# eduardburlacu/DiTSep

Measured on AMD Instinct MI355X. Metric: separated utterances/sec @ N=30, 2-spk 4 s mixtures, higher is better.
Workload: dtype fp16 (fp16 MFMA operands, fp32 accumulate)

## Files before the change

ditsep_amd/csrc/engine.hip:

```cpp
#include <math.h>
#include <stdarg.h>
#include <stdio.h>
#include <stdlib.h>
#include <string.h>

#include <algorithm>
#include <map>
#include <numeric>
#include <set>
#include <stdexcept>
#include <string>
#include <vector>

#include "../../include/ditsep_hip.h"
#include "igemm.h"
#include "kernels.h"

namespace {

struct Err : std::runtime_error {
  int code;
  Err(int c, const std::string& m) : std::runtime_error(m), code(c) {}
};

[[noreturn]] void fail(int code, const char* fmt, ...) {
  char buf[512];
  va_list ap;
  va_start(ap, fmt);
  vsnprintf(buf, sizeof buf, fmt, ap);
  va_end(ap);
  throw Err(code, buf);
}

#define HIPCHK(expr)                                                                       \
  do {                                                                                     \
    hipError_t e_ = (expr);                                                                \
    if (e_ != hipSuccess) fail(DSN_EHIP, "%s -> %s (%s:%d)", #expr, hipGetErrorString(e_), \
                               __FILE__, __LINE__);                                        \
  } while (0)

struct DevTensor {
  float* p = nullptr;
  std::vector<long> shape;
  long numel = 0;
};

struct Packed {
  op16_t* w = nullptr;
  long ps = 0;
  int N = 0, K = 0, Cin = 0, taps = 0;
  float* bias = nullptr;
  int bias_mod = 1;
};

struct ActP {
  int kind = DSN_ACT_NONE;
  float* a = nullptr;
  float* ib = nullptr;
  int mod = 1;
};

struct Packed8 {
  unsigned char* w = nullptr;
  unsigned char* s = nullptr;
  int N = 0, K = 0;
  float* bias = nullptr;
};

struct DitLayer {
  float *g1 = nullptr, *be1 = nullptr, *g2 = nullptr, *be2 = nullptr;
  Packed qkv, out, ff1, ff2;
  Packed8 qkv8, out8, ff1_8, ff2_8;
  Packed ff1f;
  float* ff1_colsum = nullptr;
  Packed8 ff1f8;
  float* ff1_colsum8 = nullptr;
};

struct ResUnit {
  ActP act0, act2;
  Packed conv7, conv1;
  int dil = 1;
};

struct VaeBlock {
  ActP act;
  Packed conv;
  ResUnit ru[3];
  int cin = 0, cout = 0, stride = 1;
};

struct Graph {
  hipGraphExec_t exec = nullptr;
  uint64_t epoch = ~0ull;
  bool warmed = false;
};

struct ProfRec {
  hipEvent_t a, b;
  double flops;
  double hbm_bytes = 0;
  const char* tag = "";
  bool gemm = true;
  bool hbm_bound = false;
};

struct ProfRow {
  std::string name;
  double ms = 0, flops = 0, bytes = 0;
  int64_t launches = 0;
};

}

struct dsn_ctx {
  dsn_config cfg;
  std::string err;
  int P = 2;
  int PL = 2;
  bool fp8 = false;
  bool fold_ln8 = false;
  bool fold_ln = false;
  bool finalized = false;
  bool use_graphs = false;
  int* fin_err_host = nullptr;
  int* fin_err_dev = nullptr;
  std::map<int, std::pair<unsigned*, long>> gnf_sync;
  unsigned* gnf_counters(int nper, long count, hipStream_t st) {
    if (!fin_err_host) {
      HIPCHK(hipHostMalloc((void**)&fin_err_host, sizeof(int), hipHostMallocMapped));
      *fin_err_host = 0;
      HIPCHK(hipHostGetDevicePointer((void**)&fin_err_dev, fin_err_host, 0));
    }
    auto& c = gnf_sync[nper];
    if (!c.first || c.second < count) {
      if (c.first) {
        HIPCHK(hipDeviceSynchronize());
        HIPCHK(hipFree(c.first));
      }
      c.second = std::max(count, 1024L);
      HIPCHK(hipMalloc((void**)&c.first, c.second * sizeof(unsigned)));
      HIPCHK(hipMemsetAsync(c.first, 0, c.second * sizeof(unsigned), st));
      ++ws_epoch;
    }
    return c.first;
  }
  double hbm_ms = 0, hbm_bytes = 0;
  int64_t hbm_launches = 0;
  std::map<std::string, DevTensor> raw;
  std::vector<void*> allocs;
  std::map<std::string, std::pair<void*, size_t>> ws;
  uint64_t ws_epoch = 0;
  struct StoiFilter {
    double* taps = nullptr;
    int ntaps = 0, up = 1, down = 1, n_pre_pad = 0, n_pre_remove = 0;
  };
  std::map<int, StoiFilter> stoi_filters;
  OdeCtl* ode_host = nullptr;

  float* tf_w = nullptr;
  Packed t1, t2, pin, pout;
  std::vector<DitLayer> layers;
  Packed dec_in;
  std::vector<VaeBlock> dec_blocks;
  ActP dec_final_act;
  float* dec_out_w = nullptr;
  int dec_out_taps = 7;
  float *enc_in_w = nullptr, *enc_in_b = nullptr;
  std::vector<VaeBlock> enc_blocks;
  ActP enc_final_act;
  Packed enc_out;

  std::map<std::string, Graph> graphs;
  hipStream_t own[2] = {nullptr, nullptr};
  hipEvent_t ev_in[2] = {nullptr, nullptr}, ev_out[2] = {nullptr, nullptr};
  bool profiling = false;
  std::vector<ProfRec> prof;
  std::vector<ProfRow> prof_rows;
  const char* cur_tag = "";
  struct Tag {
    dsn_ctx* c;
    const char* prev;
    Tag(dsn_ctx* ctx, const char* t) : c(ctx), prev(ctx->cur_tag) { c->cur_tag = t; }
    ~Tag() { c->cur_tag = prev; }
  };
  template <class F>
  void prof_launch(const char* tag, double bytes, hipStream_t st, F&& f) {
    if (!profiling) {
      f();
      return;
    }
    ProfRec pr;
    HIPCHK(hipEventCreate(&pr.a));
    HIPCHK(hipEventCreate(&pr.b));
    pr.flops = 0;
    pr.hbm_bytes = bytes;
    pr.tag = tag;
    pr.gemm = false;
    HIPCHK(hipEventRecord(pr.a, st));
    f();
    HIPCHK(hipEventRecord(pr.b, st));
    prof.push_back(pr);
  }
  std::vector<float> tv_host;
  int tv_B = -1;

  template <class F>
  void run_graphed(const std::string& key, hipStream_t st, F&& body) {
    if (!use_graphs || profiling) {
      body(st);
      return;
    }
    Graph& g = graphs[key];
    if (g.exec && g.epoch == ws_epoch) {
      HIPCHK(hipGraphLaunch(g.exec, st));
      return;
    }
    if (g.exec) {
      (void)hipGraphExecDestroy(g.exec);
      g.exec = nullptr;
    }
    if (!g.warmed || g.epoch != ws_epoch) {
      body(st);
      g.warmed = true;
      g.epoch = ws_epoch;
      return;
    }
    hipGraph_t graph = nullptr;
// ... 260 lines not shown
      raw.erase(name);
    }
  }

  void finalize(hipStream_t st, bool strict = true) {
    used.clear();
    if (!allocs.empty()) {
      HIPCHK(hipDeviceSynchronize());
      for (void* q : allocs) (void)hipFree(q);
      allocs.clear();
      ++ws_epoch;
    }
    const int D = cfg.dit_embed_dim;
    fold_ln = P == 1 && !fp8 && D % 64 == 0 && getenv("DSN_NO_LN_FOLD") == nullptr;
    fold_ln8 = fp8 && D % 128 == 0 && getenv("DSN_NO_LN_FOLD") == nullptr;
    if (cfg.score_kind == DSN_SCORE_DIT) {
      const std::string sp = "score_model.";
      if (D % 64 != 0 || cfg.dit_heads <= 0 || D / cfg.dit_heads != 64 || D % cfg.dit_heads != 0)
        fail(DSN_EINVAL, "DiT: embed_dim must be heads x 64 (got %d / %d heads)", D, cfg.dit_heads);
      tf_w = get(sp + "timestep_features.weight").p;
      t1 = pack_linear(sp + "to_timestep_embed.0.weight", sp + "to_timestep_embed.0.bias", false, st);
      t2 = pack_linear(sp + "to_timestep_embed.2.weight", sp + "to_timestep_embed.2.bias", false, st);
      fold_dit_io(sp);
      pin = pack_linear(sp + "__project_in_folded", "", false, st);
      pout = pack_linear(sp + "__project_out_folded", "", false, st);
      layers.resize(cfg.dit_depth);
      for (int i = 0; i < cfg.dit_depth; ++i) {
        const std::string lp = sp + "transformer.layers." + std::to_string(i) + ".";
        DitLayer& L = layers[i];
        L.g1 = get(lp + "pre_norm.gamma").p;
        L.be1 = maybe(lp + "pre_norm.beta");
        L.g2 = get(lp + "ff_norm.gamma").p;
        L.be2 = maybe(lp + "ff_norm.beta");
        if (fp8) {
          L.qkv8 = pack_linear_fp8(lp + "self_attn.to_qkv.weight", "", false, st);
          L.qkv = pack_linear(lp + "self_attn.to_qkv.weight", "", false, st);
          L.out8 = pack_linear_fp8(lp + "self_attn.to_out.weight", "", false, st);
          L.ff1_8 = pack_linear_fp8(lp + "ff.ff.0.proj.weight", lp + "ff.ff.0.proj.bias", true, st);
          L.ff2_8 = pack_linear_fp8(lp + "ff.ff.2.weight", lp + "ff.ff.2.bias", false, st);
          if (fold_ln8) {
            const DevTensor& w = get(lp + "ff.ff.0.proj.weight");
            Packed8& p = L.ff1f8;
            p.N = L.ff1_8.N;
            p.K = L.ff1_8.K;
            p.w = (unsigned char*)dmalloc((size_t)p.N * p.K);
            p.s = (unsigned char*)dmalloc((size_t)p.N * (p.K / 32));
            launch_pack_weight_fp8(w.p, p.w, p.s, p.N, p.K, 1, st, L.g2);
            L.ff1_colsum8 = (float*)dmalloc(sizeof(float) * p.N);
            launch_fp8_row_sum(p.w, p.s, p.N, p.K, L.ff1_colsum8, st);
            p.bias = L.ff1_8.bias;
            if (L.be2) {
              float* tmp = (float*)dmalloc(sizeof(float) * p.N);
              launch_bias_plus_wbeta(w.p, L.be2, maybe(lp + "ff.ff.0.proj.bias"), p.N, p.K, tmp, st);
              p.bias = (float*)dmalloc(sizeof(float) * p.N);
              launch_pack_bias_swiglu(tmp, p.bias, p.N, st);
            }
          }
          continue;
        }
        L.qkv = pack_linear(lp + "self_attn.to_qkv.weight", "", false, st);
        L.out = pack_linear(lp + "self_attn.to_out.weight", "", false, st);
        L.ff1 = pack_linear(lp + "ff.ff.0.proj.weight", lp + "ff.ff.0.proj.bias", true, st);
        L.ff2 = pack_linear(lp + "ff.ff.2.weight", lp + "ff.ff.2.bias", false, st);
        if (fold_ln) {
          const DevTensor& w = get(lp + "ff.ff.0.proj.weight");
          Packed& p = L.ff1f;
          p.N = (int)w.shape[0];
          p.K = p.Cin = (int)(w.numel / w.shape[0]);
          p.taps = 1;
          p.ps = (long)p.N * p.K;
          p.w = (op16_t*)dmalloc(sizeof(op16_t) * p.ps * P);
          launch_pack_weight(w.p, nullptr, p.w, p.ps, PL, PACK_LINEAR_SWIGLU, p.N, p.K, p.K, p.N, 1, 1, st, L.g2);
          L.ff1_colsum = (float*)dmalloc(sizeof(float) * p.N);
          launch_packed_row_sum(p.w, p.ps, PL, p.N, p.K, L.ff1_colsum, st);
          const float* b1 = maybe(lp + "ff.ff.0.proj.bias");
          p.bias = L.ff1.bias;
          if (L.be2) {
            float* tmp = (float*)dmalloc(sizeof(float) * p.N);
            launch_bias_plus_wbeta(w.p, L.be2, b1, p.N, p.K, tmp, st);
            p.bias = (float*)dmalloc(sizeof(float) * p.N);
            launch_pack_bias_swiglu(tmp, p.bias, p.N, st);
          }
          p.bias_mod = p.N;
        }
      }
    }
    if (cfg.score_kind == DSN_SCORE_NCSNPP) finalize_ncsnpp(st);
    const int nb = cfg.vae_n_blocks;
    const int ch = cfg.vae_channels;
    std::vector<int> mult(nb + 1, 1);
    for (int i = 0; i < nb; ++i) mult[i + 1] = cfg.vae_c_mults[i];
    if (cfg.vae_has_decoder) {
      const std::string dp = "vae.decoder.";
      dec_in = pack_conv(dp + "layers.0.", st);
      dec_blocks.resize(nb);
      int li = 1;
      for (int i = nb; i >= 1; --i, ++li) {
        VaeBlock& b = dec_blocks[li - 1];
        const std::string bp = dp + "layers." + std::to_string(li) + ".";
        b.cin = mult[i] * ch;
        b.cout = mult[i - 1] * ch;
        b.stride = cfg.vae_strides[i - 1];
        b.act = make_act(bp + "layers.0.", b.cin, st);
        b.conv = pack_convT(bp + "layers.1.", b.stride, st);
        const int dils[3] = {1, 3, 9};
        for (int j = 0; j < 3; ++j)
          b.ru[j] = make_ru(bp + "layers." + std::to_string(2 + j) + ".", b.cout, dils[j], st);
      }
      dec_final_act = make_act(dp + "layers." + std::to_string(li) + ".", mult[0] * ch, st);
      {
        const std::string fp = dp + "layers." + std::to_string(li + 1) + ".";
        const bool wn = has(fp + "weight_v");
        const DevTensor& v = get(fp + (wn ? "weight_v" : "weight"));
        if (v.shape[0] != 1) fail(DSN_EINVAL, "decoder io_channels must be 1 (got %ld)", v.shape[0]);
        const int C = (int)v.shape[1], kw = (int)v.shape[2];
        dec_out_taps = kw;
        std::vector<float> hv(v.numel), hg(1, 1.f);
        HIPCHK(hipStreamSynchronize(st));
        HIPCHK(hipMemcpy(hv.data(), v.p, sizeof(float) * v.numel, hipMemcpyDeviceToHost));
        double nrm = 1.0, g = 1.0;
        if (wn) {
          HIPCHK(hipMemcpy(hg.data(), get(fp + "weight_g").p, sizeof(float), hipMemcpyDeviceToHost));
          double ss = 0;
          for (float x : hv) ss += (double)x * x;
          nrm = sqrt(ss);
          g = hg[0];
        }
        std::vector<float> w(kw * C);
        for (int c = 0; c < C; ++c)
          for (int k = 0; k < kw; ++k) w[k * C + c] = (float)(hv[c * kw + k] * ((float)g / (float)nrm));
        dec_out_w = (float*)dmalloc(sizeof(float) * w.size());
        HIPCHK(hipMemcpy(dec_out_w, w.data(), sizeof(float) * w.size(), hipMemcpyHostToDevice));
      }
    }
    if (cfg.vae_has_encoder) {
      const std::string ep = "vae.encoder.";
      {
        const std::string fp = ep + "layers.0.";
        const bool wn = has(fp + "weight_v");
        const DevTensor& v = get(fp + (wn ? "weight_v" : "weight"));
        if (v.shape[1] != 1) fail(DSN_EINVAL, "encoder in_channels must be 1");
        const int Cout = (int)v.shape[0], kw = (int)v.shape[2];
        std::vector<float> hv(v.numel), hg(Cout, 1.f);
        HIPCHK(hipStreamSynchronize(st));
        HIPCHK(hipMemcpy(hv.data(), v.p, sizeof(float) * v.numel, hipMemcpyDeviceToHost));
        if (wn) HIPCHK(hipMemcpy(hg.data(), get(fp + "weight_g").p, sizeof(float) * Cout, hipMemcpyDeviceToHost));
        for (int co = 0; co < Cout; ++co) {
          float s = 1.f;
          if (wn) {
            float ss = 0;
            for (int k = 0; k < kw; ++k) ss += hv[co * kw + k] * hv[co * kw + k];
            s = hg[co] / sqrtf(ss);
          }
          for (int k = 0; k < kw; ++k) hv[co * kw + k] *= s;
        }
        enc_in_w = (float*)dmalloc(sizeof(float) * hv.size());
        HIPCHK(hipMemcpy(enc_in_w, hv.data(), sizeof(float) * hv.size(), hipMemcpyHostToDevice));
        enc_in_b = maybe(fp + "bias");
      }
      enc_blocks.resize(nb);
      int li = 1;
      for (int i = 0; i < nb; ++i, ++li) {
        VaeBlock& b = enc_blocks[i];
        const std::string bp = ep + "layers." + std::to_string(li) + ".";
        b.cin = mult[i] * ch;
        b.cout = mult[i + 1] * ch;
// ... 31 lines not shown
    d.in_row_elems = w.Cin;
    d.out_bstride = (long)rows_per_b * w.N;
    d.out_row_elems = w.N;
    d.out_off = 0;
    d.out_limit = d.out_bstride;
    d.resid_bstride = d.out_bstride;
    d.resid_row_elems = d.out_row_elems;
    d.resid_off = d.out_off;
    d.bias = w.bias;
    d.bias_mod = w.bias_mod;
    d.out_scale = 1.f;
    d.act_mod = 1;
    return d;
  }
  void set_act(GemmDesc& d, const ActP& a) {
    d.act = a.kind;
    d.act_a = a.a;
    d.act_b = a.ib;
    d.act_mod = a.mod;
  }
  int pick_ksplit(const GemmDesc& d) const {
    const int nkt = d.taps * (d.Cin / 32);
    const int tiles = cdiv(d.M, 128) * cdiv(d.N, 128);
    int k = (400 + tiles / 2) / tiles;
    k = std::min(k, std::min(8, nkt / 8));
    return std::max(k, 1);
  }
  void audit_span(const char* what, const void* p, long lo_bytes, long hi_bytes, const GemmDesc& d) const {
    if (!p || hi_bytes <= lo_bytes) return;
    hipDeviceptr_t base = nullptr;
    size_t size = 0;
    if (hipMemGetAddressRange(&base, &size, (hipDeviceptr_t)p) != hipSuccess)
      fail(DSN_EINVAL, "audit: %s = %p is not inside a device allocation (M=%d N=%d Cin=%d taps=%d)", what, p, d.M, d.N,
           d.Cin, d.taps);
    const char* b0 = (const char*)base;
    const char* q = (const char*)p;
    if (q + lo_bytes < b0 || q + hi_bytes > b0 + size)
      fail(DSN_EINVAL, "audit: %s spans [%ld, %ld) bytes from its pointer but the allocation holds [%ld, %ld) "
           "(M=%d N=%d Cin=%d taps=%d rows_per_b=%d)", what, lo_bytes, hi_bytes, (long)(b0 - q), (long)(b0 + size - q),
           d.M, d.N, d.Cin, d.taps, d.rows_per_b);
  }
  void audit_desc(const GemmDesc& d, bool engine_gn_slots = true) const {
    if (d.a_scale) return;
    const long nb = cdiv(d.M, d.rows_per_b), rows_last = d.M - (nb - 1) * (long)d.rows_per_b;
    const long rows_max = nb > 1 ? d.rows_per_b : rows_last;
    const long e16 = sizeof(op16_t), e32 = sizeof(float);
    if (d.M <= 0 || d.N <= 0 || d.rows_per_b <= 0) fail(DSN_EINVAL, "audit: empty GEMM");
    audit_span("A", d.A, 0, ((nb - 1) * d.in_bstride + (long)(d.Lin - 1) * d.in_row_elems + d.Cin + (P - 1) * d.a_ps) * e16, d);
    audit_span("W", d.W, 0, ((long)d.N * d.taps * d.Cin + (P - 1) * d.w_ps) * e16, d);
    const long n_out = d.swiglu ? d.N / 2 : d.N;
    const long rel_hi = std::min<long>(d.out_limit, (rows_max - 1) * (long)d.out_row_elems + d.out_off + n_out);
    const long out_hi = (nb - 1) * d.out_bstride + rel_hi;
    const long ks = std::max(d.ksplit, 1);
    if (d.stat_out) {
      audit_span("out_f32", d.out_f32, 0, (long)d.M * d.N * e32, d);
      audit_span("out_planes", d.out_planes, 0, ((long)d.M * d.N + (P - 1) * d.out_ps) * e16, d);
      audit_span("stat_out", d.stat_out, 0, (long)d.M * d.stat_np * 2 * e32, d);
    } else {
      audit_span("out_f32", d.out_f32, 0, (out_hi + (ks - 1) * d.slab_stride) * e32, d);
      audit_span("out_planes", d.out_planes, 0, (out_hi + (P - 1) * d.out_ps) * e16, d);
    }
    audit_span("resid", d.resid, 0, ((nb - 1) * d.resid_bstride + (rows_max - 1) * (long)d.resid_row_elems + d.resid_off + d.N) * e32, d);
    if (d.resid && d.resid_off < 0) fail(DSN_EINVAL, "audit: negative residual offset");
    audit_span("bias", d.bias, 0, (long)d.bias_mod * e32, d);
    audit_span("bbias", d.bbias, 0, ((nb - 1) * (long)d.bbias_stride + d.N) * e32, d);
    if (d.act == DSN_ACT_SNAKE) {
      audit_span("act_a", d.act_a, 0, (long)d.act_mod * e32, d);
      audit_span("act_b", d.act_b, 0, (long)d.act_mod * e32, d);
    }
    if (d.gn_stats) {
      if (d.rows_per_b % 64 != 0 || d.N % 4 != 0 || d.M % d.rows_per_b != 0 || d.ksplit > 1)
        fail(DSN_EINVAL, "audit: GroupNorm partials need whole 64-row slices (rows_per_b=%d M=%d N=%d ksplit=%d)",
             d.rows_per_b, d.M, d.N, d.ksplit);
      audit_span("gn_stats", d.gn_stats, 0, nb * (d.rows_per_b / 64) * (long)(d.N / 4) * 2 * e32, d);
      if (engine_gn_slots && nb * (d.rows_per_b / 64) * (long)(d.N / 4) * 2 > ncs_slot_floats)
        fail(DSN_EINVAL, "audit: GroupNorm partials overflow their statistics slot");
      if (d.gn_stats2) {
        if (d.gn_qoff2 < 0 || d.gn_qoff2 + d.N / 4 > d.gn_nq2 ||
            (engine_gn_slots && nb * (d.rows_per_b / 64) * (long)d.gn_nq2 * 2 > ncs_slot_floats))
          fail(DSN_EINVAL, "audit: concat GroupNorm partials outside their slot (nq2=%d qoff2=%d N=%d)", d.gn_nq2,
               d.gn_qoff2, d.N);
        audit_span("gn_stats2", d.gn_stats2, 0, nb * (d.rows_per_b / 64) * (long)d.gn_nq2 * 2 * e32, d);
      }
    }
    if (d.ln_stats) {
      audit_span("ln_stats", d.ln_stats, 0, (long)d.M * d.ln_np * 2 * e32, d);
      audit_span("ln_colsum", d.ln_colsum, 0, (long)d.N * e32, d);
    }
    if (d.rope_cos) {
      audit_span("rope_cos", d.rope_cos, 0, (long)d.rope_S * 32 * e32, d);
      audit_span("rope_sin", d.rope_sin, 0, (long)d.rope_S * 32 * e32, d);
    }
    if (d.sc_A) {
      audit_span("sc_A", d.sc_A, 0, ((nb - 1) * d.sc_bstride + (rows_max - 1) * (long)d.sc_row_elems + d.sc_Cin) * e16, d);
      audit_span("sc_W", d.sc_W, 0, (long)d.N * d.sc_Cin * e16, d);
      audit_span("sc_bias", d.sc_bias, 0, (long)d.N * e32, d);
    }
    if (d.img_w > 0 && (d.rows_per_b != d.img_w * d.img_h || d.taps != 9))
      fail(DSN_EINVAL, "audit: 2-D conv descriptor with rows_per_b != H*W");
  }
  void run(const GemmDesc& d, hipStream_t st, int panel_bn = 0, bool skinny = false) {
    static const bool audit = getenv("DSN_AUDIT") != nullptr;
    if (audit) audit_desc(d);
    ProfRec pr;
    if (profiling) {
      HIPCHK(hipEventCreate(&pr.a));
      HIPCHK(hipEventCreate(&pr.b));
      pr.flops = 2.0 * (double)d.M * (double)d.N * ((double)d.taps * (double)d.Cin + (d.sc_A ? (double)d.sc_Cin : 0.0));
      pr.tag = cur_tag;
      HIPCHK(hipEventRecord(pr.a, st));
    }
    const long ctiles = (long)cdiv(d.M, 128) * cdiv(d.N, 128);
    if (P == 1 && cfg.score_kind == DSN_SCORE_NCSNPP && !skinny && panel_bn == 0 && d.ksplit <= 1 &&
        d.Cin % 32 == 0 && d.N % 64 == 0 && ctiles <= 32 && d.taps * d.Cin >= 512 && !d.swiglu && !d.rope_cos &&
        (d.out_f32 || d.out_planes) && d.out_off >= 0 && d.tap_dil >= 0 && d.in_stride == 1 &&
        (d.img_w > 0 || (d.taps == 1 && d.in_pad == 0))) {
      const int nkt = d.taps * d.Cin / 32;
      const int ks = (int)std::max(2L, std::min<long>(std::min<long>(8, nkt / 4), 64 / ctiles));
      const long span = (long)cdiv(d.M, d.rows_per_b) * d.out_bstride;
      float* slabs = wsbuf<float>("conv_slabs", span * 8);
      GemmDesc g = d;
      g.ksplit = ks;
      g.slab_stride = span;
      g.out_f32 = slabs;
      g.out_planes = nullptr;
      g.gn_stats = nullptr;
      g.gn_stats2 = nullptr;
      g.cfg_bm = 128;
      g.cfg_bn = 128;
      g.cfg_nst = 3;
      g.cfg_bk = 32;
      hipError_t e1 = igemm2_launch(g, PL, st);
      if (e1 == hipSuccess) e1 = igemm_slab_epilogue_launch(d, PL, slabs, ks, span, st);
      if (profiling) {
        HIPCHK(hipEventRecord(pr.b, st));
        prof.push_back(pr);
      }
      if (e1 != hipSuccess) fail(DSN_EHIP, "split conv launch failed: %s", hipGetErrorString(e1));
      return;
    }
    hipError_t e = skinny ? igemm_skinny_launch(d, PL, st)
                          : (panel_bn > 0 ? igemm_panel_launch(d, PL, panel_bn, st) : igemm2_launch(d, PL, st));
    if (profiling) {
      HIPCHK(hipEventRecord(pr.b, st));
      prof.push_back(pr);
    }
    if (e != hipSuccess) fail(DSN_EHIP, "igemm launch failed: %s (M=%d N=%d Cin=%d taps=%d)", hipGetErrorString(e),
                              d.M, d.N, d.Cin, d.taps);
  }

  GemmDesc fp8_desc(const unsigned char* A8, const unsigned char* SA, const Packed8& w, int M) {
    Packed pk;
    pk.w = reinterpret_cast<op16_t*>(w.w);
    pk.ps = 0;
    pk.N = w.N;
    pk.Cin = w.K / 2;
    pk.K = w.K / 2;
    pk.taps = 1;
    pk.bias = w.bias;
    pk.bias_mod = w.N;
    GemmDesc d = base_desc(reinterpret_cast<const op16_t*>(A8), 0, pk, 1, M, M);
    d.a_scale = SA;
    d.w_scale = w.s;
    d.mx_kblocks = w.K / 32;
    return d;
  }
// ... 83 lines not shown
    float* data = nullptr;
    int width = 0;
    const float* find(const float* t, int B) const {
      if (!data || t < t0 || t + B > t0 + rows) return nullptr;
      return data + (long)(t - t0) * width;
    }
  } time_cache;

  float* dit_forward(const float* xt, const float* t, const float* mix, int B, int T, hipStream_t st) {
    const int n = cfg.n_src, Dl = cfg.latent_dim, D = cfg.dit_embed_dim, H = cfg.dit_heads;
    const int io = n * Dl, din = io + Dl, S = T + 1;
    const long Mt = (long)B * T, M = (long)B * S;
    op16_t* Up = wsbuf<op16_t>("dit_Up", Mt * din * P);
    float* X = wsbuf<float>("dit_X", M * D);
    op16_t* Ap = wsbuf<op16_t>("dit_Ap", M * D * P);
    op16_t* QKVp = wsbuf<op16_t>("dit_QKVp", M * 3 * D * P);
    op16_t* FF = wsbuf<op16_t>("dit_FF", M * 4 * D * P);
    float* SC = wsbuf<float>("sc", Mt * io);
    unsigned char* A8 = fp8 ? wsbuf<unsigned char>("dit_A8", M * D) : nullptr;
    unsigned char* SA8 = fp8 ? wsbuf<unsigned char>("dit_SA8", M * D / 32) : nullptr;
    unsigned char* H8 = fp8 ? wsbuf<unsigned char>("dit_H8", M * 4 * D) : nullptr;
    unsigned char* SH8 = fp8 ? wsbuf<unsigned char>("dit_SH8", M * 4 * D / 32) : nullptr;
    op16_t* lnout = fp8 ? reinterpret_cast<op16_t*>(A8) : Ap;
    const char* skx = getenv("DSN_SKINNY_MAX");
    const int skinny_max = skx ? std::min(atoi(skx), 128) : 80;
    const bool skinny = P == 1 && !fp8 && M <= skinny_max && D % 256 == 0;
    const int skinny_ks = 8;
    const bool use_panel = D % 64 == 0;
    int fold_rows = 0;
    if ((fold_ln || fold_ln8) && use_panel && !skinny) {
      for (int rounds = 1; rounds <= 4 && !fold_rows; ++rounds) {
        const int np = 256 * rounds / std::max(1, cdiv(D, 128));
        if (np >= 1 && cdiv(M, np) <= 80) fold_rows = cdiv(M, np);
      }
    }
    op16_t* Xp = (fold_rows && !fp8) ? wsbuf<op16_t>("dit_Xp", M * D) : nullptr;
    unsigned char* X8 = (fold_rows && fp8) ? wsbuf<unsigned char>("dit_X8", M * D) : nullptr;
    unsigned char* SX8 = (fold_rows && fp8) ? wsbuf<unsigned char>("dit_SX8", M * D / 32) : nullptr;
    float* ST = fold_rows ? wsbuf<float>("dit_ST", M * (D / 64) * 2) : nullptr;
    const int rot = 32;
    const bool new_rope = !ws.count("rope_cos_" + std::to_string(S));
    float* rc = wsbuf<float>("rope_cos_" + std::to_string(S), (long)S * rot);
    float* rs = wsbuf<float>("rope_sin_" + std::to_string(S), (long)S * rot);
    if (new_rope) launch_rope_tables(rc, rs, S, rot, st);

    launch_pack_tokens(xt, io, mix, Dl, B, T, nullptr, Up, Mt * din, PL, st);
    {
      Tag tg(this, "dit.project_in");
      GemmDesc d = base_desc(Up, Mt * din, pin, B, T, T);
      d.out_f32 = X;
      d.out_bstride = (long)S * D;
      d.out_off = D;
      d.out_limit = (long)S * D;
      run(d, st);
    }
    {
      const float* te = time_cache.find(t, B);
      if (!te) {
        float* tmp = wsbuf<float>("dit_te1", (long)B * D);
        Tag tg(this, "dit.time_embed");
        dit_time_embed(t, B, tmp, st);
        te = tmp;
      }
      launch_copy_rows(te, X, B, D, (long)S * D, st);
    }
    const bool short_panel = use_panel && P == 1;
    auto panel_rows_for = [&](int wg_per_panel, int max_rows = 272) {
      for (int rounds = 1;; ++rounds) {
        const int np = std::max(1, 256 * rounds / std::max(1, wg_per_panel));
        const int rows = (cdiv(M, np) + 7) / 8 * 8;
        if (rows <= max_rows) return rows;
      }
    };
    const int qkv_panel = short_panel ? 256 : 0;
    int qa_ipp = 0;
    if (P == 1 && !skinny && D == H * 64 && S <= qkv_attention_max_rows()) {
      int ipp = std::min(B, std::max(1, 144 / S));
      while (ipp > 1 && cdiv(B, ipp) * H < 256) --ipp;
      if (cdiv(B, ipp) * H >= 128) qa_ipp = ipp;
      const char* force = getenv("DSN_QA_IPP");
      if (force && atoi(force) >= 1 && atoi(force) * S <= qkv_attention_max_rows()) qa_ipp = atoi(force);
    }
    op16_t* AOp = qa_ipp ? wsbuf<op16_t>("dit_AOp", M * D) : nullptr;
    float* slabs = nullptr;
    int pend_n = 0;
    const float* pend_bias = nullptr;
    const long slab_stride = M * D;
    for (int i = 0; i < cfg.dit_depth; ++i) {
      const DitLayer& L = layers[i];
      auto ln_bytes = [&](int np) { return (double)M * D * (4.0 * (np ? 2 : 1) + 4.0 * np + 2.0 * P); };
      prof_launch("dit.residual_norm", ln_bytes(pend_n), st, [&] {
        launch_residual_norm(X, slabs, pend_n, slab_stride, pend_bias, L.g1, L.be1, qa_ipp ? Ap : lnout, M * D, PL,
                             (int)M, D, 1e-5f, 1, st, qa_ipp ? nullptr : SA8);
      });
      if (qa_ipp) {
        QkvAttnDesc q;
        memset(&q, 0, sizeof q);
        q.A = Ap;
        q.W = L.qkv.w;
        q.bias = L.qkv.bias;
        q.rope_cos = rc;
        q.rope_sin = rs;
        q.out = fp8 ? nullptr : AOp;
        q.out8 = fp8 ? A8 : nullptr;
        q.out8_scale = fp8 ? SA8 : nullptr;
        q.M = (int)M;
        q.D = D;
        q.H = H;
        q.S = S;
        q.ipp = qa_ipp;
        q.q_scale = 0.125f;
        ProfRec pr;
        if (profiling) {
          HIPCHK(hipEventCreate(&pr.a));
          HIPCHK(hipEventCreate(&pr.b));
          pr.flops = 2.0 * (double)M * 3.0 * D * D + 4.0 * (double)B * H * (double)S * S * 64.0;
          pr.tag = "dit.qkv_attention";
          HIPCHK(hipEventRecord(pr.a, st));
        }
        const hipError_t e = qkv_attention_launch(q, PL, st);
        if (profiling) {
          HIPCHK(hipEventRecord(pr.b, st));
          prof.push_back(pr);
        }
        if (e != hipSuccess) fail(DSN_EHIP, "qkv_attention launch failed: %s", hipGetErrorString(e));
      } else {
      {
        Tag tg(this, "dit.qkv");
        GemmDesc d = fp8 ? fp8_desc(A8, SA8, L.qkv8, (int)M) : base_desc(Ap, M * D, L.qkv, 1, (int)M, (int)M);
        d.out_planes = QKVp;
        d.out_ps = M * 3 * D;
        d.rope_cos = rc;
        d.rope_sin = rs;
        d.rope_S = S;
        d.qkv_D = D;
        d.q_scale = 0.125f;
        d.m_fast = 1;
        if (qkv_panel) d.panel_rows = panel_rows_for(cdiv(3 * D, qkv_panel));
        if (fp8) {
          d.panel_rows = panel_rows_for(cdiv(3 * D, 256), 208);
          run_fp8(d, st, 256);
        } else if (skinny) {
          run(d, st, 0, true);
        } else {
          run(d, st, qkv_panel);
        }
      }
      prof_launch("dit.attention", (double)M * D * 2.0 * P * 4.0, st,
                  [&] { launch_attention_mfma(QKVp, M * 3 * D, lnout, M * D, PL, B, S, H, 64, st, SA8); });
      }
      {
        Tag tg(this, "dit.attn_out");
        GemmDesc d = fp8 ? fp8_desc(A8, SA8, L.out8, (int)M)
                         : base_desc(qa_ipp ? AOp : Ap, M * D, L.out, 1, (int)M, (int)M);
        if (fold_rows) {
          d.panel_rows = fold_rows;
          d.resid = X;
          d.out_f32 = X;
          d.out_planes = Xp;
          d.out_fp8 = X8;
          d.out_fp8_scale = SX8;
          d.out_ps = M * D;
          d.stat_out = ST;
          d.stat_np = D / 64;
          d.m_fast = 0;
          if (fp8) run_fp8(d, st, 128);
          else run(d, st, 128);
          pend_n = 0;
          pend_bias = nullptr;
        } else {
        const int obn = 128, oks = 2;
        d.ksplit = skinny ? skinny_ks : ((short_panel || fp8) ? oks : pick_ksplit(d));
        if (short_panel || fp8) d.panel_rows = panel_rows_for(cdiv(D, obn) * oks);
        if (d.ksplit > 1) {
          slabs = wsbuf<float>("dit_slabs", slab_stride * 8);
          d.out_f32 = slabs;
          d.slab_stride = slab_stride;
          d.bias = nullptr;
        } else {
          d.resid = X;
          d.out_f32 = X;
        }
        if (fp8) run_fp8(d, st, obn);
        else if (skinny) run(d, st, 0, true);
        else run(d, st, short_panel ? obn : 0);
        pend_n = d.ksplit > 1 ? d.ksplit : 0;
        pend_bias = nullptr;
        }
      }
      if (!fold_rows)
        prof_launch("dit.residual_norm", ln_bytes(pend_n), st, [&] {
          launch_residual_norm(X, slabs, pend_n, slab_stride, pend_bias, L.g2, L.be2, lnout, M * D, PL, (int)M, D,
                               1e-5f, 1, st, SA8);
        });
      {
        Tag tg(this, "dit.ff_in");
        GemmDesc d = fp8 ? (fold_rows ? fp8_desc(X8, SX8, L.ff1f8, (int)M) : fp8_desc(A8, SA8, L.ff1_8, (int)M))
                         : (fold_rows ? base_desc(Xp, M * D, L.ff1f, 1, (int)M, (int)M)
                                      : base_desc(Ap, M * D, L.ff1, 1, (int)M, (int)M));
        d.swiglu = 1;
        if (fold_rows) {
          d.ln_stats = ST;
          d.ln_np = D / 64;
          d.ln_colsum = fp8 ? L.ff1_colsum8 : L.ff1_colsum;
          d.ln_eps = 1e-5f;
        }
        if (fp8) {
          d.out_fp8 = H8;
          d.out_fp8_scale = SH8;
        } else {
          d.out_planes = FF;
        }
        d.out_ps = M * 4 * D;
        d.out_bstride = M * 4L * D;
        d.out_row_elems = 4 * D;
        d.out_limit = d.out_bstride;
        d.m_fast = 1;
        if (use_panel) {
          const int np = cdiv(M, 272);
          d.panel_rows = short_panel ? panel_rows_for(cdiv(4 * D * 2, 256)) : (cdiv(M, np) + 7) / 8 * 8;
        }
        if (fp8) {
          d.panel_rows = panel_rows_for(cdiv(4 * D * 2, 256));
          run_fp8(d, st, 256);
        } else if (skinny) {
          run(d, st, 0, true);
        } else {
          run(d, st, use_panel ? 256 : 0);
        }
      }
      {
        Tag tg(this, "dit.ff_out");
        GemmDesc d = fp8 ? fp8_desc(H8, SH8, L.ff2_8, (int)M) : base_desc(FF, M * 4 * D, L.ff2, 1, (int)M, (int)M);
        const int fbn = 256, fks = 4;
        d.ksplit = skinny ? skinny_ks : ((short_panel || fp8) ? fks : pick_ksplit(d));
        if (short_panel || fp8) d.panel_rows = panel_rows_for(cdiv(D, fbn) * fks, fp8 ? 208 : 272);
        if (d.ksplit > 1) {
          slabs = wsbuf<float>("dit_slabs", slab_stride * 8);
          d.out_f32 = slabs;
          d.slab_stride = slab_stride;
          pend_bias = d.bias;
          d.bias = nullptr;
        } else {
          d.resid = X;
          d.out_f32 = X;
          pend_bias = nullptr;
        }
        if (fp8) run_fp8(d, st, fbn);
        else if (skinny) run(d, st, 0, true);
        else run(d, st, short_panel ? fbn : 0);
        pend_n = d.ksplit > 1 ? d.ksplit : 0;
      }
    }
    prof_launch("dit.residual_norm", (double)M * D * (8.0 + 4.0 * pend_n + 2.0 * P), st, [&] {
      launch_residual_norm(X, slabs, pend_n, slab_stride, pend_bias, nullptr, nullptr, Ap, M * D, PL, (int)M, D, 1e-5f,
                           0, st);
    });
    {
      Tag tg(this, "dit.project_out");
      GemmDesc d = base_desc(Ap, M * D, pout, B, T, S);
      d.in_pad = -1;
      d.in_bstride = (long)S * D;
      d.out_f32 = SC;
      if (use_panel && P == 1 && d.N <= 128 && d.M >= 1024) {
        d.panel_rows = 64;
        run(d, st, 128);
      } else {
        run(d, st);
      }
    }
    return SC;
  }

#include "engine_ncsnpp.inc"

  float* score_tokens(const float* xt, const float* t, const float* mix, int B, int T, hipStream_t st) {
    if (!finalized) fail(DSN_ESTATE, "weights not finalized");
    if (cfg.score_kind == DSN_SCORE_DIT) return dit_forward(xt, t, mix, B, T, st);
    if (cfg.score_kind == DSN_SCORE_NCSNPP) {
      Tag tg(this, "ncsnpp.conv");
      return ncsnpp_forward(xt, t, mix, B, T, st);
    }
    fail(DSN_ESTATE, "no score network configured (score_kind=%d)", cfg.score_kind);
  }

  struct Sched {
    std::vector<float> t, std, step, gain, G, g;
    float stdT;
  };
  float ouve_std(float t) const {
    const double th = cfg.sde_theta, smin = cfg.sde_sigma_min, ls = log((double)cfg.sde_sigma_max / smin);
    const float a = expf((float)(-2.0 * th) * t);
    const float b = expf((float)(2.0 * (th + ls)) * t) - 1.f;
    const float num = (float)(smin * smin) * a * b * (float)ls;
    return sqrtf(num / (float)(th + ls));
  }
  std::vector<float> t_override;
  Sched schedule(int N, float t_eps, float snr) const {
    Sched s;
    const double smin = cfg.sde_sigma_min, smax = cfg.sde_sigma_max, ls = log(smax / smin);
    s.t.resize(N);
    s.std.resize(N);
    s.step.resize(N);
    s.gain.resize(N);
    s.G.resize(N);
    s.g.resize(N);
    const float start = 1.f, end = t_eps;
    const float stp = N > 1 ? (end - start) / (float)(N - 1) : 0.f;
    const int halfway = N / 2;
    for (int i = 0; i < N; ++i) s.t[i] = i < halfway ? start + stp * (float)i : end - stp * (float)(N - 1 - i);
    if ((int)t_override.size() >= N)
      for (int i = 0; i < N; ++i) s.t[i] = t_override[i];
    const float sqdt = sqrtf((float)(1.0 / N));
    for (int i = 0; i < N; ++i) {
      const float t = s.t[i];
      s.std[i] = ouve_std(t);
      const float q = snr * s.std[i];
      s.step[i] = q * q * 2.f;
      s.gain[i] = sqrtf(s.step[i] * 2.f);
      const float sigma = (float)smin * powf((float)(smax / smin), t);
      s.g[i] = sigma * (float)sqrt(2.0 * ls);
      s.G[i] = s.g[i] * sqdt;
    }
    s.stdT = ouve_std(1.f);
    return s;
  }

  void upload_timesteps(int B, int N, float t_eps, float snr, hipStream_t st) {
    const Sched s = schedule(N, t_eps, snr);
    std::vector<float> ht((size_t)B * N);
    for (int i = 0; i < N; ++i)
      for (int b = 0; b < B; ++b) ht[(size_t)i * B + b] = s.t[i];
    float* tv = wsbuf<float>("pc_t", (long)B * N);
    if (ht == tv_host && tv_B == B) return;
    HIPCHK(hipMemcpyAsync(tv, ht.data(), sizeof(float) * ht.size(), hipMemcpyHostToDevice, st));
    HIPCHK(hipStreamSynchronize(st));
    tv_host = ht;
    tv_B = B;
  }
  struct PcOpts {
    int pred = DSN_PRED_REVERSE_DIFFUSION, corr = DSN_CORR_ALD, c = 1, denoise = 1;
    float snr = 0.5f, t_eps = 0.03f;
    const float* prior_mean = nullptr;
// ... 421 lines not shown
      HIPCHK(hipMemcpy2DAsync(wc, sizeof(float) * Lc, wav + (long)c.src * h, sizeof(float) * Lt, sizeof(float) * Lc, S,
                              hipMemcpyDeviceToDevice, st));
      float* e = encode_body(wc, S, (int)Lc, st);
      HIPCHK(hipMemcpy2DAsync(out + (long)c.t0 * E, sizeof(float) * (size_t)T * E, e + (long)c.c0 * E,
                              sizeof(float) * (size_t)chunk * E, sizeof(float) * (size_t)(c.t1 - c.t0) * E, S,
                              hipMemcpyDeviceToDevice, st));
    }
    return out;
  }
};

namespace {
thread_local std::string g_create_err;

template <class F>
int guarded(dsn_ctx* ctx, F&& f) {
  if (!ctx) return DSN_EINVAL;
  try {
    HIPCHK(hipSetDevice(ctx->cfg.device));
    if (ctx->fin_err_host && *ctx->fin_err_host) {
      *ctx->fin_err_host = 0;
      fail(DSN_EHIP, "a GroupNorm hand-off wait of an earlier call gave up (the workgroups of one conv were not resident "
                     "together): that call's results are invalid; DSN_NO_GN_FIN=1 selects the separate GroupNorm pass");
    }
    f();
    return DSN_OK;
  } catch (const Err& e) {
    ctx->err = e.what();
    return e.code;
  } catch (const std::exception& e) {
    ctx->err = e.what();
    return DSN_EINVAL;
  }
}
}

extern "C" {

dsn_ctx* dsn_create(const dsn_config* cfg) {
  try {
    if (!cfg) fail(DSN_EINVAL, "null config");
    if (cfg->precision < DSN_PREC_BF16 || cfg->precision > DSN_PREC_FP8)
      fail(DSN_EINVAL, "precision must be one of DSN_PREC_{BF16,BF16X3,FP16,FP16X3,FP8}");
    if (cfg->vae_n_blocks < 0 || cfg->vae_n_blocks > DSN_MAX_VAE_BLOCKS) fail(DSN_EINVAL, "bad vae_n_blocks");
    if (cfg->n_src < 1 || cfg->latent_dim % 32 != 0) fail(DSN_EINVAL, "bad n_src / latent_dim");
    if (cfg->score_kind == DSN_SCORE_DIT &&
        (cfg->dit_heads <= 0 || cfg->dit_embed_dim <= 0 || cfg->dit_embed_dim % cfg->dit_heads != 0 ||
         cfg->dit_embed_dim / cfg->dit_heads != 64))
      fail(DSN_EINVAL, "DiT: only 64-wide attention heads are implemented (embed_dim %d / %d heads = %d)",
           cfg->dit_embed_dim, cfg->dit_heads, cfg->dit_heads > 0 ? cfg->dit_embed_dim / cfg->dit_heads : 0);
    int ndev = 0;
    HIPCHK(hipGetDeviceCount(&ndev));
    if (cfg->device < 0 || cfg->device >= ndev) fail(DSN_EINVAL, "device %d out of range (%d GPUs)", cfg->device, ndev);
    HIPCHK(hipSetDevice(cfg->device));
    dsn_ctx* c = new dsn_ctx();
    c->cfg = *cfg;
    c->P = (cfg->precision == DSN_PREC_BF16X3 || cfg->precision == DSN_PREC_FP16X3) ? 2 : 1;
    c->PL = DSN_PL(c->P, cfg->precision >= DSN_PREC_FP16 ? 1 : 0);
    c->fp8 = cfg->precision == DSN_PREC_FP8;
    if (c->fp8 && cfg->score_kind == DSN_SCORE_DIT && cfg->dit_embed_dim % 128 != 0)
      fail(DSN_EINVAL, "DSN_PREC_FP8: embed_dim must be a multiple of 128 (got %d)", cfg->dit_embed_dim);
    return c;
  } catch (const std::exception& e) {
    g_create_err = e.what();
    return nullptr;
  }
}

void dsn_destroy(dsn_ctx* ctx) {
  if (!ctx) return;
  (void)hipSetDevice(ctx->cfg.device);
  (void)hipDeviceSynchronize();
  for (auto& g : ctx->graphs)
    if (g.second.exec) (void)hipGraphExecDestroy(g.second.exec);
  for (int k = 0; k < 2; ++k) {
    if (ctx->own[k]) (void)hipStreamDestroy(ctx->own[k]);
    if (ctx->ev_in[k]) (void)hipEventDestroy(ctx->ev_in[k]);
    if (ctx->ev_out[k]) (void)hipEventDestroy(ctx->ev_out[k]);
  }
  for (auto& kv : ctx->raw) (void)hipFree(kv.second.p);
  for (void* p : ctx->allocs) (void)hipFree(p);
  for (auto& kv : ctx->ws) (void)hipFree(kv.second.first);
  for (auto& kv : ctx->gnf_sync) (void)hipFree(kv.second.first);
  if (ctx->fin_err_host) (void)hipHostFree(ctx->fin_err_host);
  if (ctx->ode_host) (void)hipHostFree(ctx->ode_host);
  delete ctx;
}

const char* dsn_last_error(const dsn_ctx* ctx) { return ctx ? ctx->err.c_str() : g_create_err.c_str(); }

int dsn_load_tensor(dsn_ctx* ctx, const char* name, const float* data, const int64_t* shape, int ndim,
                    int is_device) {
  return guarded(ctx, [&] {
    if (!name || !data || ndim < 0 || ndim > 8) fail(DSN_EINVAL, "dsn_load_tensor: bad arguments");
    DevTensor t;
    t.numel = 1;
    for (int i = 0; i < ndim; ++i) {
      t.shape.push_back(shape[i]);
      t.numel *= shape[i];
    }
    if (t.numel <= 0) fail(DSN_EINVAL, "%s: empty tensor", name);
    auto it = ctx->raw.find(name);
    if (it != ctx->raw.end()) {
      HIPCHK(hipFree(it->second.p));
      ctx->raw.erase(it);
    }
    HIPCHK(hipMalloc((void**)&t.p, sizeof(float) * t.numel));
    HIPCHK(hipMemcpy(t.p, data, sizeof(float) * t.numel, is_device ? hipMemcpyDeviceToDevice : hipMemcpyHostToDevice));
    ctx->raw[name] = t;
    ctx->finalized = false;
  });
}

int dsn_finalize_weights(dsn_ctx* ctx) { return dsn_finalize_weights_ex(ctx, 1); }

int dsn_finalize_weights_ex(dsn_ctx* ctx, int strict) {
  return guarded(ctx, [&] { ctx->finalize(nullptr, strict != 0); });
}

int dsn_score(dsn_ctx* ctx, const float* xt, const float* t, const float* mix, float* out, int B, int T,
              void* stream) {
  return guarded(ctx, [&] {
    if (!xt || !t || !mix || !out || B <= 0 || T <= 0) fail(DSN_EINVAL, "dsn_score: bad arguments");
    hipStream_t st = (hipStream_t)stream;
    float* sc = ctx->score_tokens(xt, t, mix, B, T, st);
    launch_unpack_tokens(sc, out, B, ctx->cfg.n_src * ctx->cfg.latent_dim, T, st);
    HIPCHK(hipGetLastError());
  });
}

int dsn_ouve_schedule(const dsn_ctx* ctx, int N, float t_eps, float snr, float* timesteps, float* std_,
                      float* corr_step, float* corr_gain, float* G, float* std_T) {
  if (!ctx || N <= 0) return DSN_EINVAL;
  const dsn_ctx::Sched s = ctx->schedule(N, t_eps, snr);
  for (int i = 0; i < N; ++i) {
    if (timesteps) timesteps[i] = s.t[i];
    if (std_) std_[i] = s.std[i];
    if (corr_step) corr_step[i] = s.step[i];
    if (corr_gain) corr_gain[i] = s.gain[i];
    if (G) G[i] = s.G[i];
  }
  if (std_T) *std_T = s.stdT;
  return DSN_OK;
}

int dsn_pc_sample_ex(dsn_ctx* ctx, const float* y, const float* noise, uint64_t seed, float* x_out, int B, int T,
                     int N, const dsn_sampler_opts* opts, int* nfe_out, void* stream) {
  return guarded(ctx, [&] {
    if (!y || !x_out || !opts || B <= 0 || T <= 0 || N <= 0 || opts->corrector_steps < 0)
      fail(DSN_EINVAL, "dsn_pc_sample: bad arguments");
    if (opts->predictor < 0 || opts->predictor > DSN_PRED_NONE || opts->corrector < 0 ||
        opts->corrector > DSN_CORR_LANGEVIN)
      fail(DSN_EINVAL, "dsn_pc_sample: unknown predictor %d / corrector %d", opts->predictor, opts->corrector);
    dsn_ctx::PcOpts o;
    o.pred = opts->predictor;
    o.corr = opts->corrector;
    o.c = opts->corrector_steps;
    o.denoise = opts->denoise;
    o.snr = opts->snr;
    o.t_eps = opts->timesteps ? opts->timesteps[N - 1] : opts->t_eps;
    o.inter = opts->intermediates;
    hipStream_t caller = (hipStream_t)stream;
    const int n = ctx->cfg.n_src, Dl = ctx->cfg.latent_dim;
    const long ysz = (long)B * Dl * T, sz = ysz * n;
    const long draws = o.draws(N);
    const bool graphs = ctx->use_graphs;
// ... 931 lines not shown
    op16_t* ap = ctx->wsbuf<op16_t>("tg_a", t->a_numel * P);
    op16_t* wp = ctx->wsbuf<op16_t>("tg_w", wn * P);
    launch_to_planes(t->a, ap, t->a_numel, PL, t->a_numel, st);
    launch_to_planes(t->w, wp, wn, PL, wn, st);
    Packed pk;
    pk.w = wp;
    pk.ps = wn;
    pk.N = t->N;
    pk.Cin = t->Cin;
    pk.taps = t->taps;
    pk.K = t->taps * t->Cin;
    pk.bias = const_cast<float*>(t->bias);
    pk.bias_mod = t->bias ? (t->bias_mod > 0 ? t->bias_mod : t->N) : 1;
    GemmDesc d = ctx->base_desc(ap + t->a_off, t->a_numel, pk, t->B, t->rows_per_b, t->Lin);
    if (t->M > 0) d.M = t->M;
    d.in_stride = t->in_stride;
    d.tap_dil = t->tap_dil;
    d.in_pad = t->in_pad;
    if (t->in_row_elems > 0) d.in_row_elems = t->in_row_elems;
    d.in_bstride = t->in_bstride > 0 ? t->in_bstride : (long)t->Lin * d.in_row_elems;
    d.img_h = t->img_h;
    d.img_w = t->img_w;
    const int n_out = t->swiglu ? t->N / 2 : t->N;
    d.out_row_elems = t->out_row_elems > 0 ? t->out_row_elems : n_out;
    d.out_bstride = t->out_bstride > 0 ? t->out_bstride : (long)t->rows_per_b * d.out_row_elems;
    d.out_off = t->out_off;
    d.out_limit = t->out_limit > 0 ? t->out_limit : d.out_bstride;
    d.bbias = t->bbias;
    d.bbias_stride = t->bbias_stride > 0 ? t->bbias_stride : t->N;
    d.resid = t->resid;
    d.resid_row_elems = t->resid_row_elems > 0 ? t->resid_row_elems : d.out_row_elems;
    d.resid_bstride = t->resid_bstride > 0 ? t->resid_bstride : (long)t->rows_per_b * d.resid_row_elems;
    d.resid_off = t->resid_off;
    d.out_scale = t->out_scale != 0.f ? t->out_scale : 1.f;
    d.f32_op = t->f32_op;
    d.act = t->act;
    d.act_a = t->act_a;
    d.act_b = t->act_b;
    d.act_mod = t->act_mod > 0 ? t->act_mod : t->N;
    d.swiglu = t->swiglu;
    d.gn_stats = t->gn_stats;
    d.gn_stats2 = t->gn_stats2;
    d.gn_nq2 = t->gn_nq2;
    d.gn_qoff2 = t->gn_qoff2;
    d.out_f32 = t->out_f32;
    d.out_planes = reinterpret_cast<op16_t*>(t->out_planes);
    d.out_ps = t->out_ps;
    if (t->sc_a) {
      if (!t->sc_w || t->sc_a_numel % 4 != 0) fail(DSN_EINVAL, "test_gemm: shortcut weight missing or sc_a_numel %% 4 != 0");
      const long sw = (long)t->N * t->sc_Cin;
      op16_t* sap = ctx->wsbuf<op16_t>("tg_sa", t->sc_a_numel * P);
      op16_t* swp = ctx->wsbuf<op16_t>("tg_sw", sw * P);
      launch_to_planes(t->sc_a, sap, t->sc_a_numel, PL, t->sc_a_numel, st);
      launch_to_planes(t->sc_w, swp, sw, PL, sw, st);
      d.sc_A = sap;
      d.sc_W = swp;
      d.sc_bias = t->sc_bias;
      d.sc_Cin = t->sc_Cin;
      d.sc_row_elems = t->sc_row_elems > 0 ? t->sc_row_elems : t->sc_Cin;
      d.sc_bstride = (long)t->rows_per_b * d.sc_row_elems;
    }
    static const bool audit = getenv("DSN_AUDIT") != nullptr;
    auto check = [&](hipError_t e, const char* what) {
      if (e != hipSuccess) fail(DSN_EHIP, "test_gemm: %s refused or failed: %s (M=%d N=%d Cin=%d taps=%d)", what,
                                hipGetErrorString(e), d.M, d.N, d.Cin, d.taps);
    };
    switch (t->kernel) {
      case DSN_TG_AUTO:
        ctx->run(d, st);
        break;
      case DSN_TG_TILE:
        if (audit) ctx->audit_desc(d, false);
        check(igemm2_launch_cfg(d, PL, t->bm, t->bn, t->nst, t->bk, st), "igemm2 tile");
        break;
      case DSN_TG_V1:
        if (audit) ctx->audit_desc(d, false);
        check(igemm_launch(d, PL, st), "igemm v1");
        break;
      case DSN_TG_PANEL:
        d.panel_rows = t->panel_rows;
        d.panel_wm = t->panel_wm;
        d.cfg_nst = t->nst;
        d.cfg_bk = t->bk;
        if (audit) ctx->audit_desc(d, false);
        check(igemm_panel_launch(d, PL, t->panel_bn, st), "row-panel kernel");
        break;
      case DSN_TG_SKINNY:
        d.ksplit = std::max(t->ksplit, 1);
        d.slab_stride = t->slab_stride;
        if (audit) ctx->audit_desc(d, false);
        check(igemm_skinny_launch(d, PL, st), "skinny kernel");
        break;
      case DSN_TG_HALO:
        if (audit) ctx->audit_desc(d, false);
        check(igemm_halo3x3_launch(d, PL, st), "halo 3x3 kernel");
        break;
      case DSN_TG_SPLITK: {
        if (!t->slabs || t->ksplit < 2 || t->slab_stride <= 0) fail(DSN_EINVAL, "test_gemm: split-K needs slabs, ksplit >= 2");
        GemmDesc g = d;
        g.ksplit = t->ksplit;
        g.slab_stride = t->slab_stride;
        g.out_f32 = t->slabs;
        g.out_planes = nullptr;
        g.gn_stats = g.gn_stats2 = nullptr;
        if (audit) {
          ctx->audit_desc(g, false);
          ctx->audit_desc(d, false);
        }
        check(igemm2_launch_cfg(g, PL, t->bm, t->bn, t->nst, t->bk, st), "igemm2 split-K tile");
        check(igemm_slab_epilogue_launch(d, PL, t->slabs, t->ksplit, t->slab_stride, st), "slab epilogue");
        break;
      }
      default:
        fail(DSN_EINVAL, "test_gemm: unknown kernel %d", t->kernel);
    }
    HIPCHK(hipGetLastError());
  });
}

int dsn_bench_igemm(dsn_ctx* ctx, int B, int Lin, int Cin, int N, int taps, int tap_dil, int in_pad, int ksplit,
                    int variant, int iters, double* ms_out) {
  return guarded(ctx, [&] {
    const int P = ctx->P, PL = ctx->PL;
    const long an = (long)B * Lin * Cin, wn = (long)N * taps * Cin, on = (long)B * Lin * N;
    float* af = ctx->wsbuf<float>("b_af", an);
    float* wf = ctx->wsbuf<float>("b_wf", wn);
    op16_t* ap = ctx->wsbuf<op16_t>("b_a", an * P);
    op16_t* wp = ctx->wsbuf<op16_t>("b_w", wn * P);
    float* out = ctx->wsbuf<float>("b_o", on * (ksplit > 1 ? ksplit : 1));
    launch_randn(af, an, 1, 0, nullptr);
    launch_randn(wf, wn, 2, 0, nullptr);
    launch_to_planes(af, ap, an, PL, an, nullptr);
    launch_to_planes(wf, wp, wn, PL, wn, nullptr);
    Packed pk;
    pk.w = wp;
    pk.ps = wn;
    pk.N = N;
    pk.Cin = Cin;
    pk.taps = taps;
    pk.K = taps * Cin;
    GemmDesc d = ctx->base_desc(ap, an, pk, B, Lin, Lin);
    d.tap_dil = tap_dil;
    d.in_pad = in_pad;
    d.out_f32 = out;
    d.ksplit = ksplit;
    d.slab_stride = on;
    hipEvent_t e0, e1;
    HIPCHK(hipEventCreate(&e0));
    HIPCHK(hipEventCreate(&e1));
    auto launch = [&] {
      d.m_fast = (variant & 0x40) ? 1 : 0;
      if (variant & 0x20) {
        d.panel_rows = (variant >> 8) & 0xfff;
        d.panel_wm = (variant & 0x80) ? 2 : 0;
        if (variant & 0x80) {
          d.cfg_nst = variant & 0xf;
          d.cfg_bk = (variant & 0x10) ? 64 : 32;
        }
        hipError_t e2 = igemm_panel_launch(d, PL, (variant >> 20) & 0x3ff, nullptr);
        if (e2 != hipSuccess) fail(DSN_EHIP, "bench panel launch: %s", hipGetErrorString(e2));
        return;
      }
      hipError_t e = variant == 1 ? igemm_launch(d, PL, nullptr)
                                  : igemm2_launch_cfg(d, PL, (variant >> 8) & 0xfff, (variant >> 20) & 0x3ff,
                                                      variant & 0xf, (variant & 0x10) ? 64 : 32, nullptr);
      if (e != hipSuccess) fail(DSN_EHIP, "bench launch: %s", hipGetErrorString(e));
    };
    launch();
    launch();
    HIPCHK(hipEventRecord(e0, nullptr));
    for (int i = 0; i < iters; ++i) launch();
    HIPCHK(hipEventRecord(e1, nullptr));
    HIPCHK(hipEventSynchronize(e1));
    float ms = 0;
    HIPCHK(hipEventElapsedTime(&ms, e0, e1));
    if (ms_out) *ms_out = ms / iters;
    (void)hipEventDestroy(e0);
    (void)hipEventDestroy(e1);
  });
}

}
```

ditsep_amd/csrc/igemm.h:

```cpp
#pragma once
#include "common.h"

struct GemmDesc {
  const op16_t* A;
  long a_ps;
  const op16_t* W;
  long w_ps;
  int M, N, Cin, taps;
  int rows_per_b, Lin, in_stride, tap_dil, in_pad;
  long in_bstride;
  int in_row_elems;
  int img_h, img_w;
  long out_bstride;
  int out_row_elems, out_off;
  long out_limit;
  const float* bias;
  int bias_mod;
  const float* resid;
  long resid_bstride;
  int resid_row_elems, resid_off;
  const float* bbias;
  int bbias_stride;
  float* gn_stats;
  float* gn_stats2;
  int gn_nq2, gn_qoff2;
  float* out_f32;
  float out_scale;
  int f32_op;
  op16_t* out_planes;
  long out_ps;
  int act;
  const float* act_a;
  const float* act_b;
  int act_mod;
  int swiglu;
  int tiles_m, tiles_n;
  int ksplit;
  long slab_stride;
  const float* rope_cos;
  const float* rope_sin;
  int rope_S, qkv_D;
  float q_scale;
  const unsigned char* a_scale;
  const unsigned char* w_scale;
  int mx_kblocks;
  unsigned char* out_fp8;
  unsigned char* out_fp8_scale;
  float* stat_out;
  int stat_np;
  const float* ln_stats;
  int ln_np;
  const float* ln_colsum;
  float ln_eps;
  int panel_rows;
  int panel_wm;
  const op16_t* sc_A;
  const op16_t* sc_W;
  const float* sc_bias;
  int sc_Cin, sc_row_elems;
  long sc_bstride;
  op16_t* gnf_out;
  const float* gnf_gamma;
  const float* gnf_beta;
  unsigned* gnf_sync;
  int* gnf_err;
  float gnf_eps;
  int gnf_silu;
  int cfg_bm, cfg_bn, cfg_nst, cfg_bk;
  int dbg;
  int m_fast;
};

hipError_t igemm_launch(const GemmDesc& d, int pl, hipStream_t stream);
hipError_t igemm2_launch(const GemmDesc& d, int pl, hipStream_t stream);
hipError_t igemm2_launch_cfg(const GemmDesc& d, int pl, int bm, int bn, int nstage, int bk, hipStream_t stream);
hipError_t igemm_slab_epilogue_launch(const GemmDesc& d, int pl, const float* slabs, int nslab, long slab_stride,
                                      hipStream_t stream);
hipError_t igemm_halo3x3_launch(const GemmDesc& d, int pl, hipStream_t stream);
int igemm_halo3x3_tile(const GemmDesc& d, int pl);
bool igemm_halo3x3_gnfin_ok(const GemmDesc& d, int pl);
bool igemm2_gnfin_ok(const GemmDesc& d, int pl);
bool igemm_halo3x3_eligible(const GemmDesc& d, int pl);
hipError_t igemm_panel_launch(const GemmDesc& d, int pl, int bn, hipStream_t stream);
hipError_t igemm_skinny_launch(const GemmDesc& d, int pl, hipStream_t stream);
hipError_t igemm_panel_fp8_launch(const GemmDesc& d, int bn, hipStream_t stream);

struct QkvAttnDesc {
  const op16_t* A;
  const op16_t* W;
  const float* bias;
  const float* rope_cos;
  const float* rope_sin;
  op16_t* out;
  unsigned char* out8;
  unsigned char* out8_scale;
  int M, D, H, S;
  int ipp;
  int panels;
  float q_scale;
};
hipError_t qkv_attention_launch(const QkvAttnDesc& d, int pl, hipStream_t stream);
int qkv_attention_max_rows();
int qkv_attention_panel_rows(int rows);

struct RuDesc {
  const op16_t* A;
  long a_ps;
  const float* X;
  const op16_t* W7;
  long w7_ps;
  const float* b7;
  const op16_t* W1;
  long w1_ps;
  const float* b1;
  float* out_f32;
  op16_t* out_planes;
  long out_ps;
  int act_mid, act_out;
  const float *mid_a, *mid_b, *out_a, *out_b;
  int S, L, dil;
};
hipError_t ru_fused_launch(const RuDesc& d, int pl, hipStream_t stream);
```

ditsep_amd/csrc/igemm.hip:

```cpp
#include "igemm.h"

#ifndef DSN_SETPRIO
#define DSN_SETPRIO 0
#endif

namespace {

constexpr int BM = 128, BN = 128, BK = 32;
constexpr int TILE_ELEMS = 128 * BK;

__device__ __forceinline__ int swz(int row, int chunk) { return chunk ^ ((-(row >> 2)) & 3); }

enum { EPI_STATS = 1, EPI_LNFOLD = 2, EPI_FP8OUT = 4 };
enum { LEAN_NO_DIT = 1, LEAN_NO_NCSN = 2, LEAN_SEEDED = 4 };

template <int NT, int MT>
__device__ __forceinline__ void seed_acc(const GemmDesc& d, f32x4 (&acc)[NT][MT], int mw0, int m_end, int nw0, int lane) {
  const int nq = (lane >> 4) * 4;
#pragma unroll
  for (int tm = 0; tm < MT; ++tm) {
    const int m = mw0 + tm * 16 + (lane & 15);
    const bool mok = m < m_end;
    const int b = mok ? m / d.rows_per_b : 0;
    const int j = mok ? m - b * d.rows_per_b : 0;
    const long roff = (long)b * d.resid_bstride + (long)j * d.resid_row_elems + d.resid_off;
#pragma unroll
    for (int tn = 0; tn < NT; ++tn) {
      const int n = nw0 + tn * 16 + nq;
      f32x4 v = {0.f, 0.f, 0.f, 0.f};
      if (mok && n < d.N) {
        if (d.bias) v = *reinterpret_cast<const f32x4*>(d.bias + (n % d.bias_mod));
        if (d.sc_bias) v += *reinterpret_cast<const f32x4*>(d.sc_bias + n);
        if (d.bbias) v += *reinterpret_cast<const f32x4*>(d.bbias + (long)b * d.bbias_stride + n);
        if (d.resid) v += *reinterpret_cast<const f32x4*>(d.resid + roff + n);
      }
      acc[tn][tm] = v;
    }
  }
}
__device__ __forceinline__ void dsn_touch(const f32x4& v) { asm volatile("" ::"v"(v)); }

#ifndef DSN_DRAIN_NOPS
#define DSN_DRAIN_NOPS 4
#endif
__device__ __forceinline__ void dsn_mfma_drain() {
#if DSN_DRAIN_NOPS > 0
  __builtin_amdgcn_sched_barrier(0);
#pragma unroll
  for (int i = 0; i < DSN_DRAIN_NOPS; ++i) asm volatile("s_nop 15" ::: "memory");
  __builtin_amdgcn_sched_barrier(0);
#endif
}

template <int ROT>
__device__ __forceinline__ float dsn_row_ror(float v) {
  const int i = __builtin_bit_cast(int, v);
  return __builtin_bit_cast(float, __builtin_amdgcn_update_dpp(i, i, 0x120 + ROT, 0xf, 0xf, false));
}

template <int P, int F16, int NT, int MT, int EPI = 0, int LEAN = 0>
__device__ __forceinline__ void epilogue_gen(const GemmDesc& d_arg, f32x4 (&acc)[NT][MT], int mw0, int m_end, int nw0,
                                             int lane, int z, const float* ln_rows = nullptr, int ln_m0 = 0) {
  dsn_mfma_drain();
  const GemmDesc d = d_arg;
  const bool f_rope = !(LEAN & LEAN_NO_DIT) && d.rope_cos != nullptr;
  const bool f_qkv = !(LEAN & LEAN_NO_DIT) && d.qkv_D > 0;
  const bool f_swiglu = !(LEAN & LEAN_NO_DIT) && d.swiglu;
  const bool f_gn = !(LEAN & LEAN_NO_NCSN) && d.gn_stats != nullptr;
  const bool f_bbias = !(LEAN & LEAN_NO_NCSN) && d.bbias != nullptr;
  const bool f_tanh = !(LEAN & LEAN_NO_NCSN) && d.f32_op == DSN_F32_TANH;
  const int nq = (lane >> 4) * 4;
  if (d.ksplit > 1) {
    float* slab = d.out_f32 + (long)z * d.slab_stride;
#pragma unroll
    for (int tm = 0; tm < MT; ++tm) {
      const int m = mw0 + tm * 16 + (lane & 15);
      if (m >= m_end) continue;
      const int b = m / d.rows_per_b;
      const int j = m - b * d.rows_per_b;
      const long row_rel = (long)j * d.out_row_elems + d.out_off;
      const long row_abs = (long)b * d.out_bstride + row_rel;
#pragma unroll
      for (int tn = 0; tn < NT; ++tn) {
        const int n = nw0 + tn * 16 + nq;
        if (n >= d.N) continue;
        const long rel = row_rel + n;
        if (rel < 0 || rel >= d.out_limit) continue;
        *reinterpret_cast<f32x4*>(slab + row_abs + n) = acc[tn][tm];
      }
    }
    return;
  }
  if constexpr ((EPI & EPI_STATS) != 0) {
    f32x4 bvec[NT];
#pragma unroll
    for (int tn = 0; tn < NT; ++tn) {
      const int n = nw0 + tn * 16 + nq;
      bvec[tn] = d.bias ? *reinterpret_cast<const f32x4*>(d.bias + (n % d.bias_mod)) : f32x4{0.f, 0.f, 0.f, 0.f};
    }
#pragma unroll
    for (int tn = 0; tn < NT; ++tn) dsn_touch(bvec[tn]);
#pragma unroll
    for (int tm = 0; tm < MT; ++tm) {
      const int m = mw0 + tm * 16 + (lane & 15);
      if (m >= m_end) continue;
      float s1 = 0.f;
#pragma unroll
      for (int tn = 0; tn < NT; ++tn) {
        const int n = nw0 + tn * 16 + nq;
        f32x4 v = acc[tn][tm] + bvec[tn];
        acc[tn][tm] = v;
        s1 += (v[0] + v[1]) + (v[2] + v[3]);
        if (n < d.N) {
          *reinterpret_cast<f32x4*>(d.out_f32 + (long)m * d.N + n) = v;
          if constexpr ((EPI & EPI_FP8OUT) == 0) {
            op16x4 hi, lo;
#pragma unroll
            for (int r = 0; r < 4; ++r) {
              op16_t h, l;
              dsn_split(v[r], h, l, F16);
              hi[r] = h;
              lo[r] = l;
            }
            *reinterpret_cast<op16x4*>(d.out_planes + (long)m * d.N + n) = hi;
            if (P == 2) *reinterpret_cast<op16x4*>(d.out_planes + d.out_ps + (long)m * d.N + n) = lo;
          }
        }
      }
      if constexpr ((EPI & EPI_FP8OUT) != 0) {
#pragma unroll
        for (int tp = 0; tp < NT / 2; ++tp) {
          float amax = 0.f;
#pragma unroll
          for (int u = 0; u < 2; ++u)
#pragma unroll
            for (int r = 0; r < 4; ++r) amax = fmaxf(amax, fabsf(acc[2 * tp + u][tm][r]));
          amax = fmaxf(amax, __shfl_xor(amax, 16, 64));
          amax = fmaxf(amax, __shfl_xor(amax, 32, 64));
          const int k = dsn_mx_exp(amax);
          const float inv = dsn_pow2(-k);
          const int nb = nw0 + tp * 32;
          if (nb < d.N) {
#pragma unroll
            for (int u = 0; u < 2; ++u)
              *reinterpret_cast<unsigned*>(d.out_fp8 + (long)m * d.N + nb + u * 16 + nq) = dsn_fp8x4(acc[2 * tp + u][tm] * inv);
            if ((lane >> 4) == 0) d.out_fp8_scale[(long)m * (d.N >> 5) + (nb >> 5)] = (unsigned char)(k + 127);
          }
        }
      }
      s1 += __shfl_xor(s1, 16, 64);
      s1 += __shfl_xor(s1, 32, 64);
      const float mean = s1 * (1.f / (NT * 16));
      float m2 = 0.f;
#pragma unroll
      for (int tn = 0; tn < NT; ++tn)
#pragma unroll
        for (int r = 0; r < 4; ++r) {
          const float dl = acc[tn][tm][r] - mean;
          m2 += dl * dl;
        }
      m2 += __shfl_xor(m2, 16, 64);
      m2 += __shfl_xor(m2, 32, 64);
      if ((lane >> 4) == 0)
        *reinterpret_cast<float2*>(d.stat_out + ((long)m * d.stat_np + nw0 / (NT * 16)) * 2) = float2{mean, m2};
    }
    return;
  }
  if constexpr ((EPI & EPI_LNFOLD) != 0 && (EPI & EPI_FP8OUT) != 0) {
    static_assert(NT == 4, "fp8 SwiGLU epilogue expects 64 packed columns per wave");
    if (nw0 >= d.N) return;
    f32x4 cv[2], cg[2], bv[2], bg[2];
#pragma unroll
    for (int tp = 0; tp < 2; ++tp) {
      const int np = nw0 + tp * 32;
      cv[tp] = *reinterpret_cast<const f32x4*>(d.ln_colsum + np + nq);
      cg[tp] = *reinterpret_cast<const f32x4*>(d.ln_colsum + np + 16 + nq);
      bv[tp] = d.bias ? *reinterpret_cast<const f32x4*>(d.bias + np + nq) : f32x4{0.f, 0.f, 0.f, 0.f};
      bg[tp] = d.bias ? *reinterpret_cast<const f32x4*>(d.bias + np + 16 + nq) : f32x4{0.f, 0.f, 0.f, 0.f};
    }
#pragma unroll
    for (int tp = 0; tp < 2; ++tp) {
      dsn_touch(cv[tp]);
      dsn_touch(cg[tp]);
      dsn_touch(bv[tp]);
      dsn_touch(bg[tp]);
    }
#pragma unroll
    for (int tm = 0; tm < MT; ++tm) {
      const int m = mw0 + tm * 16 + (lane & 15);
      if (m >= m_end) continue;
      const float mu = ln_rows[2 * (m - ln_m0)], rs = ln_rows[2 * (m - ln_m0) + 1];
      f32x4 h[2];
      float amax = 0.f;
#pragma unroll
      for (int tp = 0; tp < 2; ++tp) {
        const f32x4 val = (acc[2 * tp][tm] - cv[tp] * mu) * rs + bv[tp];
        const f32x4 gate = (acc[2 * tp + 1][tm] - cg[tp] * mu) * rs + bg[tp];
#pragma unroll
        for (int r = 0; r < 4; ++r) {
          h[tp][r] = val[r] * dsn_silu(gate[r]);
          amax = fmaxf(amax, fabsf(h[tp][r]));
        }
      }
      amax = fmaxf(amax, __shfl_xor(amax, 16, 64));
      amax = fmaxf(amax, __shfl_xor(amax, 32, 64));
      const int k = dsn_mx_exp(amax);
      const float inv = dsn_pow2(-k);
      const long orow = (long)m * (d.N >> 1);
#pragma unroll
      for (int tp = 0; tp < 2; ++tp)
        *reinterpret_cast<unsigned*>(d.out_fp8 + orow + (nw0 >> 1) + tp * 16 + nq) = dsn_fp8x4(h[tp] * inv);
      if ((lane >> 4) == 0) d.out_fp8_scale[(long)m * (d.N >> 6) + (nw0 >> 6)] = (unsigned char)(k + 127);
    }
    return;
  }
  if constexpr ((EPI & EPI_LNFOLD) != 0 && (EPI & EPI_FP8OUT) == 0) {
#pragma unroll
    for (int tp = 0; tp < NT / 2; ++tp) {
      const int np = nw0 + tp * 32;
      if (np >= d.N) continue;
      const f32x4 cv = *reinterpret_cast<const f32x4*>(d.ln_colsum + np + nq);
      const f32x4 cg = *reinterpret_cast<const f32x4*>(d.ln_colsum + np + 16 + nq);
      const f32x4 bv = d.bias ? *reinterpret_cast<const f32x4*>(d.bias + np + nq) : f32x4{0.f, 0.f, 0.f, 0.f};
      const f32x4 bg = d.bias ? *reinterpret_cast<const f32x4*>(d.bias + np + 16 + nq) : f32x4{0.f, 0.f, 0.f, 0.f};
      dsn_touch(cv);
      dsn_touch(cg);
      dsn_touch(bv);
      dsn_touch(bg);
#pragma unroll
      for (int tm = 0; tm < MT; ++tm) {
        const int m = mw0 + tm * 16 + (lane & 15);
        if (m >= m_end) continue;
        const float mu = ln_rows[2 * (m - ln_m0)], rs = ln_rows[2 * (m - ln_m0) + 1];
        const f32x4 val = (acc[2 * tp][tm] - cv * mu) * rs + bv;
        const f32x4 gate = (acc[2 * tp + 1][tm] - cg * mu) * rs + bg;
        op16x4 hi, lo;
#pragma unroll
        for (int r = 0; r < 4; ++r) {
          op16_t h, l;
          dsn_split(val[r] * dsn_silu(gate[r]), h, l, F16);
          hi[r] = h;
          lo[r] = l;
        }
        const long off = (long)m * (d.N >> 1) + (np >> 1) + nq;
        *reinterpret_cast<op16x4*>(d.out_planes + off) = hi;
        if (P == 2) *reinterpret_cast<op16x4*>(d.out_planes + d.out_ps + off) = lo;
// ... 867 lines not shown
  constexpr int REM = GROUPS % NWAVES;
  constexpr int KS = TBK / 32;

  const int tid = threadIdx.x;
  const int lane = tid & 63;
  const int wave = __builtin_amdgcn_readfirstlane(tid >> 6);
  const int wave_m = wave / WN_, wave_n = wave - wave_m * WN_;
  constexpr int MBASE = MT / WM_, MREM = MT % WM_;
  const int my_mt = MBASE + (wave_m < MREM ? 1 : 0);
  const int my_row0 = 16 * (wave_m * MBASE + min(wave_m, MREM));
  const int my_groups = (REM == 0 || wave < REM) ? GPW : GPW - 1;

  const int nwg = gridDim.x, bid = blockIdx.x;
  const int q = nwg >> 3, rr = nwg & 7, xcd = bid & 7, loc = bid >> 3;
  const int t = (xcd < rr ? xcd * (q + 1) : rr * (q + 1) + (xcd - rr) * q) + loc;
  const int ntiles = d.tiles_m * d.tiles_n;
  const int z = t / ntiles;
  const int tile = t - z * ntiles;
  const int tile_m = d.m_fast ? tile % d.tiles_m : tile / d.tiles_n;
  const int tile_n = d.m_fast ? tile / d.tiles_m : tile - tile_m * d.tiles_n;
  const int m0 = tile_m * d.panel_rows, n0 = tile_n * TBN;
  const int m_end = min(m0 + d.panel_rows, d.M);

  const int Ktot = d.taps * d.Cin;
  const int kc_per_tap = d.Cin / TBK;
  const int nkt_all = d.taps * kc_per_tap;
  const int kt_begin = (int)((long)nkt_all * z / d.ksplit);
  const int kt_end = (int)((long)nkt_all * (z + 1) / d.ksplit);
  const int nkt = kt_end - kt_begin;

  const int rsub = lane / CPR, cpos = lane % CPR;
  RowLoad rl[GPW];
#pragma unroll
  for (int gi = 0; gi < GPW; ++gi) {
    const int g = wave + gi * NWAVES;
    const bool is_a = g < AROWS / RPG;
    const int row = (is_a ? g : g - AROWS / RPG) * RPG + rsub;
    const int gchunk = cpos ^ swzk<TBK>(row);
    const int idx = (is_a ? m0 : n0) + row;
    rl[gi] = make_row(d, is_a, idx, g < GROUPS && (is_a ? idx < m_end : idx < d.N), gchunk, Ktot);
  }
  const op16_t* zsrc = zero_page + cpos * 8;
  int itap = kt_begin / kc_per_tap, ikc = kt_begin - itap * kc_per_tap;

  auto issue = [&](int stage) {
    op16_t* sbase = lds + stage * STAGE_ELEMS;
    const long offa = a_tile_off(d, itap, ikc, TBK), offw = w_tile_off(d, itap, ikc, TBK);
#pragma unroll
    for (int gi = 0; gi < GPW; ++gi) {
      if (gi < my_groups) {
        const int g = wave + gi * NWAVES;
        const bool ok = (rl[gi].mask >> itap) & 1u;
        const op16_t* g0 = rl[gi].ptr + (rl[gi].is_a ? offa : offw);
#pragma unroll
        for (int p = 0; p < P; ++p) {
          const op16_t* gp = ok ? g0 + p * rl[gi].ps : zsrc;
          __builtin_amdgcn_global_load_lds((const __attribute__((address_space(1))) void*)gp,
                                           (__attribute__((address_space(3))) void*)(sbase + p * PLANE_ELEMS + g * RPG * TBK),
                                           16, 0, 0);
        }
      }
    }
    if (++ikc == kc_per_tap) {
      ikc = 0;
      ++itap;
    }
  };

  f32x4 acc[4][MTW];
#pragma unroll
  for (int a = 0; a < 4; ++a)
#pragma unroll
    for (int b = 0; b < MTW; ++b) acc[a][b] = f32x4{0.f, 0.f, 0.f, 0.f};

  const int frow = lane & 15, fchunk = lane >> 4;
  const int fsw = swzk<TBK>(frow);
  const int a_row_off = (my_row0 + frow) * TBK;
  const int w_row_off = (AROWS + wave_n * 64 + frow) * TBK;

#pragma unroll
  for (int s2 = 0; s2 < NST - 1; ++s2)
    if (s2 < nkt) issue(s2);

  if constexpr ((EPI & EPI_STATS) != 0) {
#pragma unroll
    for (int tm = 0; tm < MTW; ++tm) {
      const int m = m0 + my_row0 + tm * 16 + (lane & 15);
#pragma unroll
      for (int tn = 0; tn < 4; ++tn) {
        const int n = n0 + wave_n * 64 + tn * 16 + (lane >> 4) * 4;
        if (tm < my_mt && m < m_end && n < d.N) acc[tn][tm] = *reinterpret_cast<const f32x4*>(d.resid + (long)m * d.N + n);
      }
    }
  }

  float* const ln_rows = reinterpret_cast<float*>(lds + NST * STAGE_ELEMS);
  if ((EPI & EPI_LNFOLD) && d.ln_stats) {
    for (int r = tid; r < m_end - m0; r += NWAVES * 64) {
      const f32x4* ps = reinterpret_cast<const f32x4*>(d.ln_stats + (long)(m0 + r) * d.ln_np * 2);
      float msum = 0.f, m2 = 0.f, q = 0.f;
      for (int p2 = 0; p2 < d.ln_np / 2; ++p2) {
        const f32x4 v = ps[p2];
        msum += v[0] + v[2];
        m2 += v[1] + v[3];
        q += v[0] * v[0] + v[2] * v[2];
      }
      const float mean = msum / (float)d.ln_np;
      const float cnt = (float)(d.Cin * d.taps) / (float)d.ln_np;
      m2 += cnt * fmaxf(q - (float)d.ln_np * mean * mean, 0.f);
      ln_rows[2 * r] = mean;
      ln_rows[2 * r + 1] = rsqrtf(m2 / (float)(d.Cin * d.taps) + d.ln_eps);
    }
  }

  for (int i = 0; i < nkt; ++i) {
    const int younger = min(NST - 2, nkt - 1 - i);
    if (NST >= 4 && younger >= 2) {
      if (REM == 0 || wave < REM)
        asm volatile("s_waitcnt vmcnt(%0) lgkmcnt(0)" ::"n"(2 * GPW * P) : "memory");
      else
        asm volatile("s_waitcnt vmcnt(%0) lgkmcnt(0)" ::"n"(2 * (GPW - 1) * P) : "memory");
    } else if (NST >= 3 && younger >= 1) {
      if (REM == 0 || wave < REM)
        asm volatile("s_waitcnt vmcnt(%0) lgkmcnt(0)" ::"n"(GPW * P) : "memory");
      else
        asm volatile("s_waitcnt vmcnt(%0) lgkmcnt(0)" ::"n"((GPW - 1) * P) : "memory");
    } else {
      asm volatile("s_waitcnt vmcnt(0) lgkmcnt(0)" ::: "memory");
    }
    __builtin_amdgcn_s_barrier();
    if (i + NST - 1 < nkt) issue((i + NST - 1) % NST);

    const op16_t* base = lds + (i % NST) * STAGE_ELEMS;
#pragma unroll
    for (int ks = 0; ks < KS; ++ks) {
      const int coff = ((ks * 4 + fchunk) ^ fsw) * 8;
      op16x8 fw[P][4];
#pragma unroll
      for (int p = 0; p < P; ++p)
#pragma unroll
        for (int k = 0; k < 4; ++k)
          fw[p][k] = *reinterpret_cast<const op16x8*>(base + p * PLANE_ELEMS + w_row_off + k * 16 * TBK + coff);
#pragma unroll
      for (int tm = 0; tm < MTW; ++tm) {
        if (tm < my_mt) {
          op16x8 fa[P];
#pragma unroll
          for (int p = 0; p < P; ++p)
            fa[p] = *reinterpret_cast<const op16x8*>(base + p * PLANE_ELEMS + a_row_off + tm * 16 * TBK + coff);
#pragma unroll
          for (int tn = 0; tn < 4; ++tn) {
            if (P == 2) {
              acc[tn][tm] = mfma16<F16>(fw[P - 1][tn], fa[0], acc[tn][tm]);
              acc[tn][tm] = mfma16<F16>(fw[0][tn], fa[P - 1], acc[tn][tm]);
            }
            acc[tn][tm] = mfma16<F16>(fw[0][tn], fa[0], acc[tn][tm]);
          }
        }
      }
    }
  }
  epilogue_gen<P, F16, 4, MTW, EPI, LEAN_NO_NCSN>(d, acc, m0 + my_row0, min(m_end, m0 + my_row0 + my_mt * 16), n0 + wave_n * 64, lane,
                                    z, ((EPI & EPI_LNFOLD) && d.ln_stats) ? ln_rows : nullptr, m0);
}


template <int WM_, int WN_, int NST, int MT, int EPI = EPI_FP8OUT>
__global__ __launch_bounds__(WM_ * WN_ * 64, 1) void igemm_panel_fp8_kernel(const GemmDesc d,
                                                                             const op16_t* __restrict__ zero_page) {
  extern __shared__ __attribute__((aligned(16))) op16_t lds[];
  constexpr int TBK = 64;
  constexpr int NWAVES = WM_ * WN_;
  constexpr int MTW = (MT + WM_ - 1) / WM_;
  constexpr int TBN = WN_ * 64;
  constexpr int AROWS = MT * 16;
  constexpr int ROWS = AROWS + TBN;
  constexpr int STAGE_ELEMS = ROWS * TBK;
  constexpr int CPR = TBK / 8;
  constexpr int RPG = 64 / CPR;
  constexpr int GROUPS = ROWS / RPG;
  constexpr int GPW = (GROUPS + NWAVES - 1) / NWAVES;
  constexpr int REM = GROUPS % NWAVES;
  constexpr int SG = (ROWS + 63) / 64;
  constexpr int SGW = (SG + NWAVES - 1) / NWAVES;
  constexpr int SROWS = (SG + 1) * 64;
  constexpr bool PF = MTW < 8;
  unsigned* const slds = reinterpret_cast<unsigned*>(lds + NST * STAGE_ELEMS);

  const int tid = threadIdx.x;
  const int lane = tid & 63;
  const int wave = __builtin_amdgcn_readfirstlane(tid >> 6);
  const int wave_m = wave / WN_, wave_n = wave - wave_m * WN_;
  constexpr int MBASE = MT / WM_, MREM = MT % WM_;
  const int my_mt = MBASE + (wave_m < MREM ? 1 : 0);
  const int my_row0 = 16 * (wave_m * MBASE + min(wave_m, MREM));
  const int my_groups = (REM == 0 || wave < REM) ? GPW : GPW - 1;

  const int nwg = gridDim.x, bid = blockIdx.x;
  const int q = nwg >> 3, rr = nwg & 7, xcd = bid & 7, loc = bid >> 3;
  const int t = (xcd < rr ? xcd * (q + 1) : rr * (q + 1) + (xcd - rr) * q) + loc;
  const int ntiles = d.tiles_m * d.tiles_n;
  const int z = t / ntiles;
  const int tile = t - z * ntiles;
  const int tile_m = d.m_fast ? tile % d.tiles_m : tile / d.tiles_n;
  const int tile_n = d.m_fast ? tile / d.tiles_m : tile - tile_m * d.tiles_n;
  const int m0 = tile_m * d.panel_rows, n0 = tile_n * TBN;
  const int m_end = min(m0 + d.panel_rows, d.M);

  const int Ktot = d.Cin;
  const int nkt_all = d.Cin / TBK;
  const int kt_begin = (int)((long)nkt_all * z / d.ksplit);
  const int kt_end = (int)((long)nkt_all * (z + 1) / d.ksplit);
  const int nkt = kt_end - kt_begin;

  const int rsub = lane / CPR, cpos = lane % CPR;
  unsigned roff[GPW];
#pragma unroll
  for (int gi = 0; gi < GPW; ++gi) {
    const int g = wave + gi * NWAVES;
    const bool is_a = g < AROWS / RPG;
    const int row = (is_a ? g : g - AROWS / RPG) * RPG + rsub;
    const int gchunk = cpos ^ swzk<TBK>(row);
    const int idx = min((is_a ? m0 : n0) + row, (is_a ? m_end : d.N) - 1);
    roff[gi] = (unsigned)(idx * Ktot + gchunk * 8) * 2u;
  }
  unsigned soff[SGW];
  bool s_a[SGW];
#pragma unroll
  for (int j = 0; j < SGW; ++j) {
    const int srow = (wave + j * NWAVES) * 64 + lane;
    const bool s_is_a = srow < AROWS;
    s_a[j] = s_is_a;
    const int sidx = s_is_a ? min(m0 + srow, m_end - 1) : min(n0 + min(srow - AROWS, TBN - 1), d.N - 1);
    soff[j] = (unsigned)(sidx * d.mx_kblocks);
  }
  int kt_abs = kt_begin;

  auto issue = [&](int stage) {
    op16_t* sbase = lds + stage * STAGE_ELEMS;
    const unsigned off = (unsigned)(kt_abs * TBK) * 2u;
#pragma unroll
    for (int gi = 0; gi < GPW; ++gi) {
      if (gi < my_groups) {
        const int g = wave + gi * NWAVES;
        const char* gp = reinterpret_cast<const char*>(g < AROWS / RPG ? d.A : d.W) + (off + roff[gi]);
        __builtin_amdgcn_global_load_lds((const __attribute__((address_space(1))) void*)gp,
// ... 441 lines not shown
static hipError_t launch_panel_fp8_t(GemmDesc d, const op16_t* zp, hipStream_t stream) {
  constexpr int TBN = WN_ * 64;
  d.tiles_m = cdiv(d.M, d.panel_rows);
  d.tiles_n = cdiv(d.N, TBN);
  static std::atomic<unsigned long long> attr{0};
  if (dsn_first_use_on_device(attr)) {
    (void)hipFuncSetAttribute(reinterpret_cast<const void*>(igemm_panel_fp8_kernel<WM_, WN_, NST, MT, EPI>),
                              hipFuncAttributeMaxDynamicSharedMemorySize, 160 * 1024);
  }
  const int grid = d.tiles_m * d.tiles_n * d.ksplit;
  const size_t smem = (size_t)NST * ((MT * 16 + TBN) * 64 * sizeof(op16_t) + ((MT * 16 + TBN + 63) / 64 + 1) * 64 * sizeof(unsigned)) +
                      ((EPI & EPI_LNFOLD) ? MT * 16 * 2 * sizeof(float) : 0);
  if (smem > 160 * 1024) return hipErrorInvalidValue;
  hipLaunchKernelGGL((igemm_panel_fp8_kernel<WM_, WN_, NST, MT, EPI>), dim3(grid), dim3(WM_ * WN_ * 64), smem, stream, d, zp);
  return hipGetLastError();
}

hipError_t igemm_panel_fp8_launch(const GemmDesc& din, int bn, hipStream_t stream) {
  GemmDesc d = din;
  if (d.ksplit < 1) d.ksplit = 1;
  if (!d.a_scale || !d.w_scale || d.taps != 1 || d.in_stride != 1 || d.in_pad != 0 || d.rows_per_b != d.M ||
      d.img_w > 0 || d.Cin % 64 != 0 || d.mx_kblocks != d.Cin / 16 || d.M <= 0 || d.N <= 0 || d.panel_rows <= 0 ||
      d.panel_rows > 17 * 16 || (long)std::max(d.M, d.N) * d.Cin * 2 >= (1L << 32))
    return hipErrorInvalidValue;
  if (d.swiglu && (d.N % 64 != 0)) return hipErrorInvalidValue;
  if (d.ksplit > 1 && (!d.out_f32 || d.swiglu)) return hipErrorInvalidValue;
  if (d.stat_out && (d.N % 64 != 0 || d.stat_np != d.N / 64 || d.swiglu || d.ksplit > 1 || !d.resid || !d.out_f32 ||
                     !d.out_fp8 || !d.out_fp8_scale))
    return hipErrorInvalidValue;
  if (d.ln_stats && (!d.swiglu || !d.ln_colsum || d.ln_np <= 0 || (d.ln_np & 1) || !d.out_fp8 || !d.out_fp8_scale))
    return hipErrorInvalidValue;
  const op16_t* zp = zero_page();
  if (!zp) return hipErrorOutOfMemory;
#define FCFGE(MT_, WM_, W_, NS_, E_) \
  if (d.panel_rows <= MT_ * 16 && bn == W_ * 64) return launch_panel_fp8_t<WM_, W_, NS_, MT_, E_>(d, zp, stream);
#define FCFG(MT_, WM_, W_, NS_) FCFGE(MT_, WM_, W_, NS_, EPI_FP8OUT)
  if (d.stat_out) {
    FCFGE(5, 4, 2, 4, EPI_STATS | EPI_FP8OUT)
    return hipErrorInvalidValue;
  }
  if (d.ln_stats) {
    FCFGE(7, 4, 4, 3, EPI_LNFOLD | EPI_FP8OUT) FCFGE(9, 2, 4, 3, EPI_LNFOLD | EPI_FP8OUT)
    FCFGE(17, 2, 4, 2, EPI_LNFOLD | EPI_FP8OUT)
    return hipErrorInvalidValue;
  }
  FCFG(7, 4, 4, 3) FCFG(9, 2, 4, 3) FCFG(9, 4, 2, 3) FCFG(13, 2, 4, 2) FCFG(13, 4, 2, 3) FCFG(17, 4, 2, 3)
  FCFG(17, 2, 4, 2)
#undef FCFG
#undef FCFGE
  return hipErrorInvalidValue;
}

hipError_t igemm_skinny_launch(const GemmDesc& din, int pl, hipStream_t stream) {
  GemmDesc d = din;
  if (d.ksplit < 1) d.ksplit = 1;
  if (PL_COUNT(pl) != 1 || d.taps != 1 || d.in_stride != 1 || d.in_pad != 0 || d.rows_per_b != d.M || d.img_w > 0 ||
      d.M <= 0 || d.M > 128 || d.N <= 0 || d.Cin % 32 != 0 || d.N % 4 != 0 || d.gn_stats || d.stat_out || d.ln_stats ||
      d.out_fp8)
    return hipErrorInvalidValue;
  if (d.swiglu && d.N % 32 != 0) return hipErrorInvalidValue;
  if (d.ksplit > 1 && (!d.out_f32 || d.swiglu || d.ksplit > d.Cin / 32)) return hipErrorInvalidValue;
  const int grid = ((d.N + 31) / 32) * d.ksplit;
  const int mt = std::max((d.M + 15) / 16, 3);
#define SK(MT_)                                                                                     \
  if (mt == MT_) {                                                                                  \
    if (PL_F16(pl)) hipLaunchKernelGGL((igemm_skinny_kernel<1, MT_>), dim3(grid), dim3(256), 0, stream, d); \
    else hipLaunchKernelGGL((igemm_skinny_kernel<0, MT_>), dim3(grid), dim3(256), 0, stream, d);     \
    return hipGetLastError();                                                                       \
  }
  SK(3) SK(4) SK(5) SK(6) SK(7) SK(8)
#undef SK
  return hipErrorInvalidValue;
}

hipError_t igemm_panel_launch(const GemmDesc& din, int pl, int bn, hipStream_t stream) {
  const int planes = PL_COUNT(pl), f16 = PL_F16(pl);
  GemmDesc d = din;
  if (d.ksplit < 1) d.ksplit = 1;
  if (d.Cin % 64 != 0 || d.M <= 0 || d.N <= 0 || d.panel_rows <= 0 || d.panel_rows > 17 * 16) return hipErrorInvalidValue;
  if (d.panel_wm == 2 && d.cfg_bk == 32 && d.Cin % 32 != 0) return hipErrorInvalidValue;
  if (d.swiglu && (d.N % 32 != 0)) return hipErrorInvalidValue;
  if (d.ksplit > 1 && (!d.out_f32 || d.swiglu)) return hipErrorInvalidValue;
  if (d.img_w > 0) return hipErrorInvalidValue;
  if (d.stat_out && (d.N % 64 != 0 || d.stat_np != d.N / 64 || d.swiglu || d.ksplit > 1)) return hipErrorInvalidValue;
  if (d.ln_stats && (!d.swiglu || !d.ln_colsum || d.ln_np <= 0 || d.taps != 1 || planes != 1)) return hipErrorInvalidValue;
  const op16_t* zp = zero_page();
  if (!zp) return hipErrorOutOfMemory;
  const int epi = (d.stat_out ? EPI_STATS : 0) | (d.ln_stats ? EPI_LNFOLD : 0);
#define PCFGE(MT_, P_, W_, NS_, BK_, E_)                                                             \
  if (planes == P_ && bn == W_ * 64 && epi == E_)                                                     \
    return f16 ? launch_panel_t<P_, 1, W_, NS_, BK_, MT_, E_>(d, zp, stream)                          \
               : launch_panel_t<P_, 0, W_, NS_, BK_, MT_, E_>(d, zp, stream);
#define PCFGS(MT_, P_, W_, NS_, BK_) PCFGE(MT_, P_, W_, NS_, BK_, 0)
#define PCFG2(MT_, NS_, BK_, E_)                                                                                \
  if (planes == 1 && bn == 256 && epi == E_ && d.panel_rows <= MT_ * 16 && (d.cfg_nst == 0 || d.cfg_nst == NS_) && \
      (d.cfg_bk == 0 || d.cfg_bk == BK_))                                                                       \
    return f16 ? launch_panel_t<1, 1, 4, NS_, BK_, MT_, E_, 2>(d, zp, stream)                                   \
               : launch_panel_t<1, 0, 4, NS_, BK_, MT_, E_, 2>(d, zp, stream);
  if (d.panel_wm == 2) {
    PCFG2(9, 3, 64, 0) PCFG2(17, 2, 64, 0) PCFG2(17, 4, 32, 0) PCFG2(17, 2, 64, EPI_LNFOLD) PCFG2(17, 4, 32, EPI_LNFOLD)
  }
#undef PCFG2
  if (d.panel_rows <= 5 * 16) {
    PCFGE(5, 1, 2, 4, 64, EPI_STATS) PCFGS(5, 1, 2, 4, 64)
  }
  if (d.panel_rows <= 7 * 16) {
    PCFGS(7, 1, 4, 3, 64) PCFGE(7, 1, 4, 3, 64, EPI_LNFOLD)
  }
  if (d.panel_rows <= 9 * 16) {
    PCFGS(9, 1, 4, 3, 64) PCFGS(9, 1, 2, 3, 64) PCFGS(9, 2, 4, 2, 32) PCFGS(9, 2, 2, 2, 32)
    PCFGE(9, 1, 4, 3, 64, EPI_LNFOLD)
  }
  if (d.panel_rows <= 13 * 16) {
    PCFGS(13, 1, 4, 2, 64) PCFGS(13, 1, 2, 2, 64) PCFGE(13, 1, 4, 2, 64, EPI_LNFOLD)
  }
  PCFGS(17, 1, 4, 2, 64) PCFGS(17, 1, 2, 2, 64) PCFGS(17, 2, 4, 2, 32) PCFGS(17, 2, 2, 2, 32)
  PCFGE(17, 1, 4, 2, 64, EPI_LNFOLD)
#undef PCFGS
#undef PCFGE
  return hipErrorInvalidValue;
}
```

ditsep_amd/csrc/kernels.h:

```cpp
#pragma once
#include "common.h"

void launch_pack_tokens(const float* src0, int C0, const float* src1, int C1, int B, int T,
                        float* dst_f32, op16_t* dst_planes, long ps, int planes, hipStream_t s);
void launch_copy_rows(const float* src, float* dst, int rows, int width, long dst_stride, hipStream_t s);
void launch_unpack_tokens(const float* src, float* dst, int B, int C, int T, hipStream_t s);
void launch_to_planes(const float* src, op16_t* dst, long ps, int planes, long n, hipStream_t s);

void launch_pc_prior(const float* mean, int mean_full, const float* z, float* x, float stdT, int B, int n, int D,
                     int T, hipStream_t s);
void launch_pc_corrector(float* x, float* x_mean , const float* score_tok, const float* z, float step,
                         float noise_gain, const float* norms, float snr, int B, int n, int D, int T, hipStream_t s);
void launch_pc_item_norms(const float* a, long per_item, int B, float* out, hipStream_t s);
void launch_pc_predictor(float* x, float* x_mean, const float* y, const float* score_tok, const float* z,
                         float theta, float dt, float G, float g, int em, int B, int n, int D, int T, hipStream_t s);

void launch_sigma_mix(const float* y, float* smix, int B, int L, int avg_len, hipStream_t s);
void launch_mix_prior(const float* y, const float* z, float* x, const float* smix, float s1, float s2, int B, int n, int D,
                      int T, hipStream_t s);
void launch_mix_corrector(float* x, float* x_mean, const float* score_tok, const float* z, const float* smix, float sq1,
                          float sq2, float snr, int B, int n, int D, int T, hipStream_t s);
void launch_mix_predictor(float* x, float* x_mean, const float* score_tok, const float* z, const float* smix,
                          float lambda, float dt, float g, float sqdt, int em, int B, int n, int D, int T, hipStream_t s);
void launch_sb_update(float* x, const float* est_tok, const float* third, float w_prev, float w_est, float w3,
                      int third_is_y, int B, int n, int D, int T, hipStream_t s);
void launch_repeat_sources(const float* y, float* x, int B, int n, int D, int T, hipStream_t s);

void launch_residual_norm(float* x, const float* slabs, int nslab, long slab_stride, const float* bias,
                          const float* gamma, const float* beta, op16_t* out, long ps, int planes, int rows, int D,
                          float eps, int do_norm, hipStream_t s, unsigned char* out_fp8_scale = nullptr);
void launch_timestep_features(const float* t, const float* w, int B, int half, op16_t* out, long ps,
                              int planes, hipStream_t s);
int launch_attention_mfma(const op16_t* qkv, long ps, op16_t* out, long out_ps, int pl, int B, int S, int H, int dh,
                          hipStream_t s, unsigned char* out_fp8_scale = nullptr);
void launch_rope_tables(float* cos_t, float* sin_t, int S, int rot, hipStream_t s);

void launch_conv_out1(const op16_t* a, long ps, int planes, const float* w, float* out, int S, int L, int C,
                      int ktaps, int apply_tanh, hipStream_t s);
void launch_conv_in1(const float* wav, const float* w, const float* bias, int S, int L, int Cout, int ktaps,
                     float* out_f32, op16_t* out_planes, long ps, int planes, int act, const float* act_a,
                     const float* act_b, hipStream_t s);
void launch_vae_sample(const float* enc_tok, const float* noise, float* y, int S, int D, int T, hipStream_t s);

void launch_randn(float* out, long n, unsigned long long seed, unsigned long long offset, hipStream_t s);

enum { PACK_LINEAR = 0, PACK_LINEAR_SWIGLU = 1, PACK_CONV = 2, PACK_CONVT = 3, PACK_CONV2D = 4, PACK_NIN = 5 };
void launch_wn_scale(const float* v, const float* g, float* scale, int R, long inner, hipStream_t s);
void launch_pack_weight(const float* src, const float* scale, op16_t* dst, long ps, int planes, int mode,
                        int N, int K, int Cin, int Cout, int kw, int stride, hipStream_t s,
                        const float* colscale = nullptr);
void launch_packed_row_sum(const op16_t* w, long ps, int planes, int N, int K, float* out, hipStream_t s);
void launch_bias_plus_wbeta(const float* W, const float* beta, const float* bias, int N, int K, float* out,
                            hipStream_t s);
void launch_pack_bias_swiglu(const float* src, float* dst, int N, hipStream_t s);
void launch_pack_weight_fp8(const float* src, unsigned char* dst, unsigned char* scales, int N, int K, int swiglu,
                            hipStream_t s, const float* colscale = nullptr);
void launch_fp8_row_sum(const unsigned char* w, const unsigned char* scales, int N, int K, float* out, hipStream_t s);
void launch_snake_params(const float* alpha, const float* beta, float* a_out, float* ib_out, int C,
                         hipStream_t s);

void launch_ncsn_pack(const float* xt, const float* mix, int B, int n, int H, int T, int Wp, int Cp, float* of,
                      op16_t* op, long ps, int planes, hipStream_t s);
void launch_gn_stats(const float* x, long bstride, int rstride, int C, int B, int HW, float* stats,
                     hipStream_t s);
void launch_gn_apply(const float* x, long bstride, int rstride, int C, int B, int HW, const float* stats,
                     const float* gamma, const float* beta, float eps, int silu, float* of, op16_t* op, long ps,
                     int planes, hipStream_t s);
void launch_fir2d(const float* x, long bstride, int rstride, int C, int B, int H, int W, int up, const float* add,
                  float* of, op16_t* op, long ps, int planes, hipStream_t s);
void launch_ncsn_fourier(const float* t, const float* w, int B, int nf, op16_t* out, long ps, int planes,
                         hipStream_t s);
void launch_ncsn_output(const float* pyr, int Cp, const float* t, const float* w, const float* bias, int cin, int n,
                        int B, int H, int T, int Wp, float* score, hipStream_t s);

void launch_sisdr_dots(const float* ref, const float* est, int B, int n, int L, double* out, hipStream_t s);

struct StoiBands {
  int lo[15], hi[15];
};
void launch_stoi_resample(const float* ref, const float* est, const int* ymap, int items, int n_in,
                          const double* taps, int ntaps, int up, int down, int n_pre_pad, int n_pre_remove, int n_out,
                          float* out, hipStream_t s);
void launch_stoi_frames(const float* xs, const float* ys, long stride, const int* ymap, int items, int F,
                        StoiBands bands, int extended, double* en, int* idx, int* Kc, double* tob, double* part,
                        double* score, int* frames, hipStream_t s);

#define DSN_ODE_MAX_ROWS 7
struct OdeTableau {
  int stages;
  int err_order;
  double a[DSN_ODE_MAX_ROWS][DSN_ODE_MAX_ROWS];
  double b[DSN_ODE_MAX_ROWS];
  double c[DSN_ODE_MAX_ROWS];
  double e[DSN_ODE_MAX_ROWS];
};
struct OdeSde {
  double theta, sigma_min, ratio, logratio;
};
struct OdeCtl {
  double t, t_new, h, h_abs, min_step, t_bound, direction, max_step, first_step, rtol, atol, h0, d1;
  int step_rejected, accept_pending, done, status;
  int nfev, accepted, rejected, attempts, max_attempts;
};
int ode_grid(long total);
void launch_ode_prior(const float* ymix, const float* z, double* y, float* xs32, float* tv, float stdT, int B, int n,
                      int D, int T, hipStream_t s);
void launch_ode_init_f0(const OdeSde& q, const OdeCtl* ctl, const float* ymix, const float* sc, const double* y,
                        double* K0, double* part, int B, int n, int D, int T, hipStream_t s);
void launch_ode_init_h0(OdeCtl* ctl, const double* part, long total, hipStream_t s);
void launch_ode_init_y1(const OdeCtl* ctl, const double* y, const double* K0, double* xs64, float* xs32, float* tv,
                        int B, long total, hipStream_t s);
void launch_ode_init_f1(const OdeSde& q, const OdeCtl* ctl, const float* ymix, const float* sc, const double* y,
                        const double* K0, const double* xs64, double* part, int B, int n, int D, int T, hipStream_t s);
// ... 26 lines not shown
```

ditsep_amd/csrc/kernels.hip:

```cpp
#include "kernels.h"

namespace {

constexpr int TPB = 256;
inline int grid_for(long n, int per_block = TPB, int cap = 256 * 16) {
  long g = (n + per_block - 1) / per_block;
  return (int)(g < 1 ? 1 : (g > cap ? cap : g));
}

__device__ __forceinline__ void store_planes(op16_t* dst, long ps, int planes, long i, float v) {
  op16_t h, l;
  dsn_split(v, h, l, PL_F16(planes));
  dst[i] = h;
  if (PL_COUNT(planes) == 2) dst[ps + i] = l;
}

__global__ void pack_tokens_kernel(const float* __restrict__ s0, int C0, const float* __restrict__ s1, int C1,
                                   int B, int T, float* __restrict__ df, op16_t* __restrict__ dp, long ps,
                                   int planes) {
  const int C = C0 + C1;
  const long n = (long)B * T * C;
  for (long i = blockIdx.x * (long)blockDim.x + threadIdx.x; i < n; i += (long)gridDim.x * blockDim.x) {
    const int c = (int)(i % C);
    const long bt = i / C;
// ... 354 lines not shown
          dsn_split(o[r], h, l, PL_F16(planes));
          hi[r] = h;
          lo[r] = l;
        }
        const long oi = (rbase >> 2) + i;
        reinterpret_cast<op16x4*>(out)[oi] = hi;
        if (PL_COUNT(planes) == 2) reinterpret_cast<op16x4*>(out + ps)[oi] = lo;
      }
    }
  }
}

template <int NS>
__global__ __launch_bounds__(TPB) void residual_norm_row_kernel(float* __restrict__ x, const float* __restrict__ slabs,
                                                                long slab_stride, const float* __restrict__ bias,
                                                                const float* __restrict__ gamma,
                                                                const float* __restrict__ beta, op16_t* __restrict__ out,
                                                                long ps, int planes, int D, float eps, int do_norm,
                                                                unsigned char* __restrict__ o8s) {
  __shared__ float red[2][TPB / 64];
  const int i = threadIdx.x, lane = i & 63, wave = i >> 6;
  const long rbase = (long)blockIdx.x * D;
  f32x4 a = reinterpret_cast<const f32x4*>(x + rbase)[i];
  f32x4 part[NS > 0 ? NS : 1];
#pragma unroll
  for (int z = 0; z < NS; ++z) part[z] = reinterpret_cast<const f32x4*>(slabs + z * slab_stride + rbase)[i];
  f32x4 g = {1.f, 1.f, 1.f, 1.f}, be = {0.f, 0.f, 0.f, 0.f};
  if (do_norm) {
    g = reinterpret_cast<const f32x4*>(gamma)[i];
    if (beta) be = reinterpret_cast<const f32x4*>(beta)[i];
  }
  if (NS > 0) {
    if (bias) a += reinterpret_cast<const f32x4*>(bias)[i];
#pragma unroll
    for (int z = 0; z < NS; ++z) a += part[z];
    reinterpret_cast<f32x4*>(x + rbase)[i] = a;
  }
  f32x4 o = a;
  if (do_norm) {
    const float s = wave_sum((a[0] + a[1]) + (a[2] + a[3]));
    if (lane == 0) red[0][wave] = s;
    __syncthreads();
    float tot = 0.f;
#pragma unroll
    for (int w = 0; w < TPB / 64; ++w) tot += red[0][w];
    const float mean = tot / D;
    float q = 0.f;
#pragma unroll
    for (int r = 0; r < 4; ++r) {
      const float dlt = a[r] - mean;
      q += dlt * dlt;
    }
    q = wave_sum(q);
    if (lane == 0) red[1][wave] = q;
    __syncthreads();
    float qt = 0.f;
#pragma unroll
    for (int w = 0; w < TPB / 64; ++w) qt += red[1][w];
    const float rstd = rsqrtf(qt / D + eps);
#pragma unroll
    for (int r = 0; r < 4; ++r) o[r] = (a[r] - mean) * rstd * g[r] + be[r];
  }
  if (o8s) {
    float amax = fmaxf(fmaxf(fabsf(o[0]), fabsf(o[1])), fmaxf(fabsf(o[2]), fabsf(o[3])));
    amax = fmaxf(amax, __shfl_xor(amax, 1, 64));
    amax = fmaxf(amax, __shfl_xor(amax, 2, 64));
    amax = fmaxf(amax, __shfl_xor(amax, 4, 64));
    const int kx = dsn_mx_exp(amax);
    reinterpret_cast<unsigned*>(out)[(rbase >> 2) + i] = dsn_fp8x4(o * dsn_pow2(-kx));
    if ((lane & 7) == 0) o8s[(rbase >> 5) + (i >> 3)] = (unsigned char)(kx + 127);
    return;
  }
  op16x4 hi, lo;
#pragma unroll
  for (int r = 0; r < 4; ++r) {
    op16_t h, l;
    dsn_split(o[r], h, l, PL_F16(planes));
    hi[r] = h;
    lo[r] = l;
  }
  const long oi = (rbase >> 2) + i;
  reinterpret_cast<op16x4*>(out)[oi] = hi;
  if (PL_COUNT(planes) == 2) reinterpret_cast<op16x4*>(out + ps)[oi] = lo;
}

__global__ void timestep_features_kernel(const float* __restrict__ t, const float* __restrict__ w, int B, int half,
                                         op16_t* __restrict__ out, long ps, int planes) {
  const int n = B * half;
  for (int i = blockIdx.x * blockDim.x + threadIdx.x; i < n; i += gridDim.x * blockDim.x) {
    const int b = i / half, k = i - b * half;
    const float f = 2.f * 3.14159265358979323846f * t[b] * w[k];
    store_planes(out, ps, planes, (long)b * 2 * half + k, cosf(f));
    store_planes(out, ps, planes, (long)b * 2 * half + half + k, sinf(f));
  }
}

__global__ void rope_tables_kernel(float* __restrict__ ct, float* __restrict__ st, int S, int rot) {
  const int half = rot / 2;
  for (int i = blockIdx.x * blockDim.x + threadIdx.x; i < S * rot; i += gridDim.x * blockDim.x) {
    const int p = i / rot, d = i - p * rot;
    const int k = d % half;
    const float inv = 1.0f / powf(10000.0f, (float)(2 * k) / (float)rot);
    const float f = (float)p * inv;
    ct[i] = cosf(f);
    st[i] = sinf(f);
  }
}

__global__ __launch_bounds__(256) void conv_out1_kernel(const op16_t* __restrict__ a, long ps, int planes,
                                                        const float* __restrict__ w, float* __restrict__ out,
                                                        int L, int C, int ktaps, int apply_tanh) {
  extern __shared__ __attribute__((aligned(16))) float smem[];
  const int RS = C + 4;
  const int nrows = 64 + ktaps - 1;
  float* rows = smem;
  float* wl = rows + nrows * RS;
  float* part = wl + ktaps * C;
  const int blocks_per_seq = (L + 63) / 64;
  const int s = blockIdx.x / blocks_per_seq;
  const int l0 = (blockIdx.x - s * blocks_per_seq) * 64;
  const int pad = (ktaps - 1) / 2;
  const int c8 = C / 8;
  for (int i = threadIdx.x; i < nrows * c8; i += blockDim.x) {
    const int r = i / c8, ch = (i - r * c8) * 8;
    const int l = l0 - pad + r;
    float v[8];
    if (l >= 0 && l < L) {
      const long gi = ((long)s * L + l) * C + ch;
      const op16x8 hi = *reinterpret_cast<const op16x8*>(a + gi);
#pragma unroll
      for (int k = 0; k < 8; ++k) v[k] = from_op16(hi[k], PL_F16(planes));
      if (PL_COUNT(planes) == 2) {
        const op16x8 lo = *reinterpret_cast<const op16x8*>(a + ps + gi);
#pragma unroll
        for (int k = 0; k < 8; ++k) v[k] += from_op16(lo[k], PL_F16(planes));
      }
    } else {
#pragma unroll
      for (int k = 0; k < 8; ++k) v[k] = 0.f;
    }
#pragma unroll
    for (int k = 0; k < 8; ++k) rows[r * RS + ch + k] = v[k];
  }
  for (int i = threadIdx.x; i < ktaps * C; i += blockDim.x) wl[i] = w[i];
  __syncthreads();
  const int pos = threadIdx.x & 63, cq = threadIdx.x >> 6;
  const int cw = C / 4;
  float acc = 0.f;
  for (int t = 0; t < ktaps; ++t) {
    const float* rr = rows + (pos + t) * RS + cq * cw;
    const float* ww = wl + t * C + cq * cw;
    for (int c = 0; c < cw; c += 4) {
      const f32x4 x4 = *reinterpret_cast<const f32x4*>(rr + c);
      const f32x4 w4 = *reinterpret_cast<const f32x4*>(ww + c);
      acc += x4[0] * w4[0] + x4[1] * w4[1] + x4[2] * w4[2] + x4[3] * w4[3];
    }
  }
  part[cq * 64 + pos] = acc;
  __syncthreads();
  if (threadIdx.x < 64) {
    const int l = l0 + threadIdx.x;
    if (l < L) {
      float v = (part[threadIdx.x] + part[64 + threadIdx.x]) + (part[128 + threadIdx.x] + part[192 + threadIdx.x]);
      out[(long)s * L + l] = apply_tanh ? tanhf(v) : v;
    }
  }
// ... 336 lines not shown
    const int g = n >> 5, w = n & 31;
    dst[n] = src[w < 16 ? 16 * g + w : F + 16 * g + (w - 16)];
  }
}

__global__ void snake_params_kernel(const float* __restrict__ alpha, const float* __restrict__ beta,
                                    float* __restrict__ a, float* __restrict__ ib, int C) {
  for (int i = blockIdx.x * blockDim.x + threadIdx.x; i < C; i += gridDim.x * blockDim.x) {
    a[i] = expf(alpha[i]);
    ib[i] = 1.0f / (expf(beta[i]) + 1e-9f);
  }
}

}

void launch_pack_tokens(const float* s0, int C0, const float* s1, int C1, int B, int T, float* df, op16_t* dp,
                        long ps, int planes, hipStream_t st) {
  const long n = (long)B * T * (C0 + C1);
  hipLaunchKernelGGL(pack_tokens_kernel, dim3(grid_for(n)), dim3(TPB), 0, st, s0, C0, s1, C1, B, T, df, dp, ps,
                     planes);
}
void launch_copy_rows(const float* src, float* dst, int rows, int width, long dst_stride, hipStream_t st) {
  hipLaunchKernelGGL(copy_rows_kernel, dim3(grid_for((long)rows * (width / 4))), dim3(TPB), 0, st, src, dst, rows,
                     width / 4, dst_stride);
}
void launch_unpack_tokens(const float* src, float* dst, int B, int C, int T, hipStream_t st) {
  hipLaunchKernelGGL(unpack_tokens_kernel, dim3(grid_for((long)B * C * T)), dim3(TPB), 0, st, src, dst, B, C, T);
}
void launch_to_planes(const float* src, op16_t* dst, long ps, int planes, long n, hipStream_t st) {
  hipLaunchKernelGGL(to_planes_kernel, dim3(grid_for(n / 4)), dim3(TPB), 0, st, src, dst, ps, planes, n / 4);
}
void launch_pc_prior(const float* mean, int mean_full, const float* z, float* x, float stdT, int B, int n, int D,
                     int T, hipStream_t st) {
  const long total = (long)B * n * D * T;
  hipLaunchKernelGGL(pc_prior_kernel, dim3(grid_for(total)), dim3(TPB), 0, st, mean, z, x, stdT, n, D, T, total,
                     mean_full);
}
void launch_pc_corrector(float* x, float* xm, const float* sc, const float* z, float step, float gain,
                         const float* norms, float snr, int B, int n, int D, int T, hipStream_t st) {
  const long total = (long)B * n * D * T;
  hipLaunchKernelGGL(pc_corrector_kernel, dim3(grid_for(total)), dim3(TPB), 0, st, x, xm, sc, z, step, gain, norms,
                     B, snr, n, D, T, total);
}
void launch_pc_item_norms(const float* a, long per_item, int B, float* out, hipStream_t st) {
  hipLaunchKernelGGL(pc_item_norm_kernel, dim3(B), dim3(256), 0, st, a, per_item, out);
}
void launch_pc_predictor(float* x, float* xm, const float* y, const float* sc, const float* z, float theta,
                         float dt, float G, float g, int em, int B, int n, int D, int T, hipStream_t st) {
  const long total = (long)B * n * D * T;
  hipLaunchKernelGGL(pc_predictor_kernel, dim3(grid_for(total)), dim3(TPB), 0, st, x, xm, y, sc, z, theta, dt, G, g,
                     em, n, D, T, total);
}
void launch_sigma_mix(const float* y, float* smix, int B, int L, int avg_len, hipStream_t st) {
  const long total = (long)B * L;
  hipLaunchKernelGGL(sigma_mix_kernel, dim3(grid_for(total)), dim3(TPB), 0, st, y, smix, L, avg_len, total);
}
void launch_mix_prior(const float* y, const float* z, float* x, const float* smix, float s1, float s2, int B, int n, int D,
                      int T, hipStream_t st) {
  const long npos = (long)B * D * T;
  hipLaunchKernelGGL(mix_prior_kernel, dim3(grid_for(npos)), dim3(TPB), 0, st, y, z, x, smix, s1, s2, n, D, T, npos);
}
void launch_mix_corrector(float* x, float* xm, const float* sc, const float* z, const float* smix, float sq1, float sq2,
                          float snr, int B, int n, int D, int T, hipStream_t st) {
  const long npos = (long)B * D * T;
  hipLaunchKernelGGL(mix_corrector_kernel, dim3(grid_for(npos)), dim3(TPB), 0, st, x, xm, sc, z, smix, sq1, sq2, snr, n,
                     D, T, npos);
}
void launch_mix_predictor(float* x, float* xm, const float* sc, const float* z, const float* smix, float lambda, float dt,
                          float g, float sqdt, int em, int B, int n, int D, int T, hipStream_t st) {
  const long npos = (long)B * D * T;
  hipLaunchKernelGGL(mix_predictor_kernel, dim3(grid_for(npos)), dim3(TPB), 0, st, x, xm, sc, z, smix, lambda, dt, g,
                     sqdt, em, n, D, T, npos);
}
void launch_sb_update(float* x, const float* est, const float* third, float w_prev, float w_est, float w3, int third_is_y,
                      int B, int n, int D, int T, hipStream_t st) {
  const long total = (long)B * n * D * T;
  hipLaunchKernelGGL(sb_update_kernel, dim3(grid_for(total)), dim3(TPB), 0, st, x, est, third, w_prev, w_est, w3,
                     third_is_y, n, D, T, total);
}
void launch_repeat_sources(const float* y, float* x, int B, int n, int D, int T, hipStream_t st) {
  const long total = (long)B * n * D * T;
  hipLaunchKernelGGL(repeat_sources_kernel, dim3(grid_for(total)), dim3(TPB), 0, st, y, x, n, D, T, total);
}
void launch_residual_norm(float* x, const float* slabs, int nslab, long slab_stride, const float* bias,
                          const float* gamma, const float* beta, op16_t* out, long ps, int planes, int rows, int D,
                          float eps, int do_norm, hipStream_t st, unsigned char* o8s) {
#define RN_LAUNCH(MV, NS_, BT_)                                                                                       \
  hipLaunchKernelGGL((residual_norm_kernel<MV, NS_, BT_>), dim3(grid_for(rows, 4)), dim3(TPB), 0, st, x, slabs, nslab, \
                     slab_stride, bias, gamma, beta, out, ps, planes, rows, D, eps, do_norm, o8s)
#define RN_SWITCH(MV, BT_)                                                                 \
  switch (nslab) {                                                                         \
    case 0: RN_LAUNCH(MV, 0, BT_); break;                                                  \
    case 1: RN_LAUNCH(MV, 1, BT_); break;                                                  \
    case 2: RN_LAUNCH(MV, 2, BT_); break;                                                  \
    case 3: RN_LAUNCH(MV, 3, BT_); break;                                                  \
    case 4: RN_LAUNCH(MV, 4, BT_); break;                                                  \
    case 5: RN_LAUNCH(MV, 5, BT_); break;                                                  \
    case 6: RN_LAUNCH(MV, 6, BT_); break;                                                  \
    case 7: RN_LAUNCH(MV, 7, BT_); break;                                                  \
    default: RN_LAUNCH(MV, 8, BT_); break;            \
  }
  if (D == 4 * TPB && rows > 256 && nslab <= 4) {
#define RNR(NS_)                                                                                                     \
  hipLaunchKernelGGL((residual_norm_row_kernel<NS_>), dim3(rows), dim3(TPB), 0, st, x, slabs, slab_stride, bias, gamma, \
                     beta, out, ps, planes, D, eps, do_norm, o8s)
    switch (nslab) {
      case 0: RNR(0); break;
      case 1: RNR(1); break;
      case 2: RNR(2); break;
      case 3: RNR(3); break;
      default: RNR(4); break;
    }
#undef RNR
    return;
  }
  if (D <= 1024 && rows <= 256) {
    RN_SWITCH(4, true)
  } else if (D <= 1024) {
    RN_SWITCH(4, false)
  } else {
    RN_SWITCH(16, false)
  }
#undef RN_SWITCH
#undef RN_LAUNCH
}
void launch_timestep_features(const float* t, const float* w, int B, int half, op16_t* out, long ps, int planes,
                              hipStream_t st) {
  hipLaunchKernelGGL(timestep_features_kernel, dim3(grid_for((long)B * half)), dim3(TPB), 0, st, t, w, B, half,
                     out, ps, planes);
}
void launch_rope_tables(float* ct, float* stb, int S, int rot, hipStream_t st) {
  hipLaunchKernelGGL(rope_tables_kernel, dim3(grid_for((long)S * rot)), dim3(TPB), 0, st, ct, stb, S, rot);
}
void launch_conv_out1(const op16_t* a, long ps, int planes, const float* w, float* out, int S, int L, int C,
                      int ktaps, int apply_tanh, hipStream_t st) {
  if (ktaps == 7 && C % 32 == 0 && C <= 1024) {
    const size_t smr = ((size_t)7 * C + (size_t)(256 + 6) * 8) * sizeof(float);
    hipLaunchKernelGGL(conv_out1_rows_kernel<7>, dim3(S * ((L + 255) / 256)), dim3(256), smr, st, a, ps, planes, w,
                       out, L, C, apply_tanh);
    return;
  }
  const size_t sm = ((size_t)(64 + ktaps - 1) * (C + 4) + (size_t)ktaps * C + 256) * sizeof(float);
  static std::atomic<unsigned long long> attr_set{0};
  if (dsn_first_use_on_device(attr_set)) {
    (void)hipFuncSetAttribute(reinterpret_cast<const void*>(conv_out1_kernel),
                              hipFuncAttributeMaxDynamicSharedMemorySize, 160 * 1024);
  }
  const int blocks = S * ((L + 63) / 64);
  hipLaunchKernelGGL(conv_out1_kernel, dim3(blocks), dim3(TPB), sm, st, a, ps, planes, w, out, L, C, ktaps,
                     apply_tanh);
}
void launch_conv_in1(const float* wav, const float* w, const float* bias, int S, int L, int Cout, int ktaps,
                     float* of, op16_t* op, long ps, int planes, int act, const float* aa, const float* ab,
                     hipStream_t st) {
  if (Cout % 4 == 0 && TPB % (Cout / 4) == 0 && ktaps <= 8) {
    const long rows = (long)S * L;
    hipLaunchKernelGGL(conv_in1_vec_kernel, dim3(grid_for(rows * (Cout / 4))), dim3(TPB), 0, st, wav, w, bias, L, Cout,
                       ktaps, of, op, ps, planes, act, aa, ab, rows);
    return;
  }
  const long total = (long)S * L * Cout;
  hipLaunchKernelGGL(conv_in1_kernel, dim3(grid_for(total)), dim3(TPB), 0, st, wav, w, bias, L, Cout, ktaps, of, op,
                     ps, planes, act, aa, ab, total);
}
void launch_vae_sample(const float* enc, const float* noise, float* y, int S, int D, int T, hipStream_t st) {
  const long total = (long)S * D * T;
// ... 81 lines not shown
```

ditsep_amd/csrc/qkv_attn.hip:

```cpp
#include "igemm.h"
#include "kernels.h"

namespace {

typedef __attribute__((ext_vector_type(4))) short s16x4;

constexpr int QA_TN = 192, QA_BK = 64;
constexpr int QA_TM_MAX = 240;

__device__ __forceinline__ int qa_swz(int row) { return (row >> 1) & 7; }
__device__ __forceinline__ int qa_off(int row, int c) { return row * 64 + ((((c >> 3) ^ qa_swz(row))) << 3) + (c & 7); }

template <int F16, int NST, int NKT, int QA_TM = 144>
__global__ __launch_bounds__(512, 1) void qkv_attention_kernel(const QkvAttnDesc d, const op16_t* __restrict__ zero_page) {
  extern __shared__ __attribute__((aligned(16))) op16_t lds[];
  constexpr int QA_ROWS = QA_TM + QA_TN;
  constexpr int QA_STAGE = QA_ROWS * QA_BK;
  constexpr int QA_AG = QA_TM / 8, QA_WG = QA_TN / 8;
  constexpr int QA_GPW = (QA_AG + QA_WG + 7) / 8;
  constexpr int MT = QA_TM / 16;
  constexpr int MT0 = (MT + 1) / 2, MTW = MT0;
  static_assert(3 * QA_TM * 64 <= NST * QA_STAGE, "the q | k | v images must fit in the ring");
  const int tid = threadIdx.x;
  const int lane = tid & 63;
  const int wave = __builtin_amdgcn_readfirstlane(tid >> 6);
  const int wm = wave >> 2, wn = wave & 3;
  const int mtw = wm == 0 ? MT0 : MT - MT0;
  const int row0 = wm == 0 ? 0 : MT0 * 16;

  const int nwg = gridDim.x, bid = blockIdx.x;
  const int q8 = nwg >> 3, rr = nwg & 7, xcd = bid & 7, loc = bid >> 3;
  const int t = (xcd < rr ? xcd * (q8 + 1) : rr * (q8 + 1) + (xcd - rr) * q8) + loc;
  int head, panel;
  if ((d.H & 3) == 0) {
    const int per_group = d.panels * 4;
    const int hg = t / per_group, rem = t - hg * per_group;
    panel = rem >> 2;
    head = hg * 4 + (rem & 3);
  } else {
    panel = t / d.H;
    head = t - panel * d.H;
  }
  const int S = d.S, K = d.D;
  const int prow = d.ipp * S;
  const int m0 = panel * prow;
  const int rows_here = min(prow, d.M - m0);
  const int nkt = K / QA_BK;

  const int rsub = lane >> 3, cpos = lane & 7;
  const op16_t* src[QA_GPW];
  int step[QA_GPW], dsto[QA_GPW];
#pragma unroll
  for (int gi = 0; gi < QA_GPW; ++gi) {
    const int g = wave * QA_GPW + gi;
    const op16_t* z = zero_page + cpos * 8;
    if (g < QA_AG) {
      const int row = g * 8 + rsub;
      const bool ok = row < rows_here;
      src[gi] = ok ? d.A + (long)(m0 + row) * K + ((cpos ^ qa_swz(row)) << 3) : z;
      step[gi] = ok ? QA_BK : 0;
      dsto[gi] = g * 8 * QA_BK;
    } else if (g < QA_AG + QA_WG) {
      const int r = (g - QA_AG) * 8 + rsub;
      const long grow = (long)(r >> 6) * d.D + head * 64 + (r & 63);
      src[gi] = d.W + grow * K + ((cpos ^ qa_swz(r)) << 3);
      step[gi] = QA_BK;
      dsto[gi] = g * 8 * QA_BK;
    } else {
      src[gi] = z;
      step[gi] = 0;
      dsto[gi] = -1;
    }
  }
  auto issue = [&](int stage, int kt) {
#pragma unroll
    for (int gi = 0; gi < QA_GPW; ++gi) {
      const op16_t* g = src[gi] + (long)kt * step[gi];
      op16_t* dst = dsto[gi] < 0 ? lds + NST * QA_STAGE : lds + stage * QA_STAGE + dsto[gi];
      __builtin_amdgcn_global_load_lds((const __attribute__((address_space(1))) void*)g,
                                       (__attribute__((address_space(3))) void*)dst, 16, 0, 0);
    }
  };

  f32x4 acc[3][MTW];
#pragma unroll
  for (int a = 0; a < 3; ++a)
#pragma unroll
    for (int b = 0; b < MTW; ++b) acc[a][b] = f32x4{0.f, 0.f, 0.f, 0.f};

  const int r16 = lane & 15, g4 = lane >> 4;
  const int fsw = qa_swz(r16);
  const int a_row_off = (row0 + r16) * QA_BK;
  const int w_row_off = (QA_TM + wn * 48 + r16) * QA_BK;

#pragma unroll
  for (int s = 0; s < NST - 1; ++s)
    if (s < nkt) issue(s, s);

  for (int i = 0; i < nkt; ++i) {
    const int younger = min(NST - 2, nkt - 1 - i);
    if (NST >= 4 && younger >= 2)
      asm volatile("s_waitcnt vmcnt(%0) lgkmcnt(0)" ::"n"(2 * QA_GPW) : "memory");
    else if (NST >= 3 && younger >= 1)
      asm volatile("s_waitcnt vmcnt(%0) lgkmcnt(0)" ::"n"(QA_GPW) : "memory");
    else
      asm volatile("s_waitcnt vmcnt(0) lgkmcnt(0)" ::: "memory");
    __builtin_amdgcn_s_barrier();
    if (i + NST - 1 < nkt) issue((i + NST - 1) % NST, i + NST - 1);

    const op16_t* base = lds + (i % NST) * QA_STAGE;
#pragma unroll
    for (int ks = 0; ks < 2; ++ks) {
      const int coff = ((ks * 4 + g4) ^ fsw) << 3;
      op16x8 fa[MTW], fw[3];
#pragma unroll
      for (int k = 0; k < 3; ++k) fw[k] = *reinterpret_cast<const op16x8*>(base + w_row_off + k * 16 * QA_BK + coff);
#pragma unroll
      for (int k = 0; k < MTW; ++k)
        if (k < mtw) fa[k] = *reinterpret_cast<const op16x8*>(base + a_row_off + k * 16 * QA_BK + coff);
#pragma unroll
      for (int tm = 0; tm < MTW; ++tm)
        if (tm < mtw) {
#pragma unroll
          for (int tn = 0; tn < 3; ++tn) acc[tn][tm] = mfma16<F16>(fw[tn], fa[tm], acc[tn][tm]);
        }
    }
  }

  asm volatile("s_waitcnt vmcnt(0) lgkmcnt(0)" ::: "memory");
  __builtin_amdgcn_s_barrier();
  op16_t* const qkv_lds = lds;
  const int rope_first = wn == 0 ? 0 : (wn == 1 ? 1 : -1);
  const int nq = g4 * 4;
#pragma unroll
  for (int tm = 0; tm < MTW; ++tm) {
    if (tm >= mtw) continue;
    const int row = row0 + tm * 16 + r16;
    if (d.bias) {
#pragma unroll
      for (int tn = 0; tn < 3; ++tn) {
        const int col = wn * 48 + tn * 16 + nq;
        acc[tn][tm] += *reinterpret_cast<const f32x4*>(d.bias + (long)(col >> 6) * d.D + head * 64 + (col & 63));
      }
    }
    if (rope_first >= 0) {
      const int pos = row % S;
      const f32x4 c0 = *reinterpret_cast<const f32x4*>(d.rope_cos + pos * 32 + nq);
      const f32x4 s0 = *reinterpret_cast<const f32x4*>(d.rope_sin + pos * 32 + nq);
      const f32x4 c1 = *reinterpret_cast<const f32x4*>(d.rope_cos + pos * 32 + 16 + nq);
      const f32x4 s1 = *reinterpret_cast<const f32x4*>(d.rope_sin + pos * 32 + 16 + nq);
      if (rope_first == 0) {
        const f32x4 x0 = acc[0][tm], x1 = acc[1][tm];
        acc[0][tm] = x0 * c0 - x1 * s0;
        acc[1][tm] = x1 * c1 + x0 * s1;
      } else {
        const f32x4 x0 = acc[1][tm], x1 = acc[2][tm];
        acc[1][tm] = x0 * c0 - x1 * s0;
        acc[2][tm] = x1 * c1 + x0 * s1;
      }
    }
#pragma unroll
    for (int tn = 0; tn < 3; ++tn) {
      const int col = wn * 48 + tn * 16 + nq;
      const int sec = col >> 6, c = col & 63;
      f32x4 v = acc[tn][tm];
      if (sec == 0) v *= d.q_scale;
      op16x4 h;
#pragma unroll
      for (int r = 0; r < 4; ++r) h[r] = to_op16(v[r], F16);
      *reinterpret_cast<op16x4*>(qkv_lds + sec * (QA_TM * 64) + qa_off(row, c)) = h;
    }
  }
  __syncthreads();

  const op16_t* const ql = qkv_lds;
  const op16_t* const kl = qkv_lds + QA_TM * 64;
  const op16_t* const vl = qkv_lds + 2 * QA_TM * 64;
  const int nqt = (S + 15) >> 4;
  const int items = rows_here / S;
  const int tq = r16 >> 2, tp = r16 & 3;
  for (int job = wave; job < items * nqt; job += 8) {
    const int it = job / nqt, qt = job - it * nqt;
    const int base = it * S;
    const int qrow = base + min(qt * 16 + r16, S - 1);
    op16x8 fq[2];
#pragma unroll
    for (int ks = 0; ks < 2; ++ks) fq[ks] = *reinterpret_cast<const op16x8*>(ql + qa_off(qrow, (ks * 4 + g4) * 8));
    f32x4 sc[NKT];
#pragma unroll
    for (int kt = 0; kt < NKT; ++kt) {
      sc[kt] = f32x4{0.f, 0.f, 0.f, 0.f};
      if (kt < nqt) {
        const int krow = base + min(kt * 16 + r16, S - 1);
#pragma unroll
        for (int ks = 0; ks < 2; ++ks) {
          const op16x8 fk = *reinterpret_cast<const op16x8*>(kl + qa_off(krow, (ks * 4 + g4) * 8));
          sc[kt] = mfma16<F16>(fk, fq[ks], sc[kt]);
        }
      }
    }
    float mx = -INFINITY;
#pragma unroll
    for (int kt = 0; kt < NKT; ++kt) {
      if (kt < nqt) {
#pragma unroll
        for (int r = 0; r < 4; ++r) {
          if (kt * 16 + 4 * g4 + r >= S) sc[kt][r] = -INFINITY;
          mx = fmaxf(mx, sc[kt][r]);
        }
      }
    }
    mx = fmaxf(mx, __shfl_xor(mx, 16, 64));
    mx = fmaxf(mx, __shfl_xor(mx, 32, 64));
    float lsum = 0.f;
#pragma unroll
    for (int kt = 0; kt < NKT; ++kt) {
#pragma unroll
      for (int r = 0; r < 4; ++r) {
        const float pv = kt < nqt ? expf(sc[kt][r] - mx) : 0.f;
        sc[kt][r] = pv;
// ... 6 lines not shown
    f32x4 oacc[4];
#pragma unroll
    for (int dt = 0; dt < 4; ++dt) oacc[dt] = f32x4{0.f, 0.f, 0.f, 0.f};
#pragma unroll
    for (int u = 0; u < (NKT + 1) / 2; ++u) {
      if (2 * u < nqt) {
        op16x8 fp;
#pragma unroll
        for (int jj = 0; jj < 8; ++jj) {
          const float pv = jj < 4 ? sc[2 * u][jj] : (2 * u + 1 < NKT ? sc[(2 * u + 1 < NKT) ? 2 * u + 1 : 0][jj - 4] : 0.f);
          fp[jj] = to_op16(pv, F16);
        }
        const int v0 = min(base + (2 * u) * 16 + 4 * g4 + tq, QA_TM - 1);
        const int v1 = min(base + (2 * u + 1) * 16 + 4 * g4 + tq, QA_TM - 1);
#pragma unroll
        for (int dt = 0; dt < 4; ++dt) {
          const s16x4 lo4 = __builtin_amdgcn_ds_read_tr16_b64_v4i16(
              (__attribute__((address_space(3))) s16x4*)(vl + qa_off(v0, dt * 16 + 4 * tp)));
          const s16x4 hi4 = __builtin_amdgcn_ds_read_tr16_b64_v4i16(
              (__attribute__((address_space(3))) s16x4*)(vl + qa_off(v1, dt * 16 + 4 * tp)));
          op16x8 fv;
#pragma unroll
          for (int e = 0; e < 4; ++e) {
            fv[e] = (unsigned short)lo4[e];
            fv[4 + e] = (unsigned short)hi4[e];
          }
          oacc[dt] = mfma16<F16>(fv, fp, oacc[dt]);
        }
      }
    }
    const float inv = 1.f / lsum;
    const long orow = (long)(m0 + base + qt * 16 + r16);
    if (d.out8) {
#pragma unroll
      for (int dp = 0; dp < 2; ++dp) {
        f32x4 v[2];
        float amax = 0.f;
#pragma unroll
        for (int u = 0; u < 2; ++u) {
          v[u] = oacc[2 * dp + u] * inv;
#pragma unroll
          for (int r = 0; r < 4; ++r) amax = fmaxf(amax, fabsf(v[u][r]));
        }
        amax = fmaxf(amax, __shfl_xor(amax, 16, 64));
        amax = fmaxf(amax, __shfl_xor(amax, 32, 64));
        const int k = dsn_mx_exp(amax);
        const float sc = dsn_pow2(-k);
        if (qt * 16 + r16 < S) {
#pragma unroll
          for (int u = 0; u < 2; ++u)
            *reinterpret_cast<unsigned*>(d.out8 + orow * d.D + head * 64 + (2 * dp + u) * 16 + 4 * g4) = dsn_fp8x4(v[u] * sc);
          if (g4 == 0) d.out8_scale[orow * (d.D >> 5) + ((head * 64 + dp * 32) >> 5)] = (unsigned char)(k + 127);
        }
      }
    } else if (qt * 16 + r16 < S) {
      op16_t* o = d.out + orow * d.D + head * 64 + 4 * g4;
#pragma unroll
      for (int dt = 0; dt < 4; ++dt) {
        op16x4 h;
#pragma unroll
        for (int r = 0; r < 4; ++r) h[r] = to_op16(oacc[dt][r] * inv, F16);
        *reinterpret_cast<op16x4*>(o + dt * 16) = h;
      }
    }
  }
}

const op16_t* qa_zero_page() {
  static op16_t* zp[64] = {};
  op16_t*& z = zp[dsn_current_device()];
  if (!z) {
    if (hipMalloc((void**)&z, 4096) != hipSuccess) return nullptr;
    (void)hipMemset(z, 0, 4096);
  }
  return z;
}

template <int F16, int NST, int NKT, int TM>
hipError_t qa_launch_t(const QkvAttnDesc& d, const op16_t* zp, hipStream_t stream) {
  static std::atomic<unsigned long long> attr{0};
  if (dsn_first_use_on_device(attr))
    (void)hipFuncSetAttribute(reinterpret_cast<const void*>(qkv_attention_kernel<F16, NST, NKT, TM>),
                              hipFuncAttributeMaxDynamicSharedMemorySize, 160 * 1024);
  const size_t smem = (size_t)(NST * (TM + QA_TN) * QA_BK + 8 * QA_BK) * sizeof(op16_t);
  hipLaunchKernelGGL((qkv_attention_kernel<F16, NST, NKT, TM>), dim3(d.panels * d.H), dim3(512), smem, stream, d, zp);
  return hipGetLastError();
}

}

int qkv_attention_max_rows() { return QA_TM_MAX; }
int qkv_attention_panel_rows(int rows) { return rows <= 144 ? 144 : QA_TM_MAX; }

hipError_t qkv_attention_launch(const QkvAttnDesc& din, int pl, hipStream_t stream) {
  QkvAttnDesc d = din;
  if (PL_COUNT(pl) != 1 || d.D != d.H * 64 || d.D % QA_BK != 0 || d.S < 1 || d.ipp < 1 || d.ipp * d.S > QA_TM_MAX ||
      d.M <= 0 || d.M % d.S != 0 || !d.A || !d.W || (!d.out && !d.out8) || (d.out8 && !d.out8_scale) || !d.rope_cos ||
      !d.rope_sin || d.A == d.out)
    return hipErrorInvalidValue;
  d.panels = cdiv(d.M / d.S, d.ipp);
  const op16_t* zp = qa_zero_page();
  if (!zp) return hipErrorOutOfMemory;
  const int nqt = (d.S + 15) / 16;
  const int f16 = PL_F16(pl);
#define QA(NST_, NKT_, TM_) \
  return f16 ? qa_launch_t<1, NST_, NKT_, TM_>(d, zp, stream) : qa_launch_t<0, NST_, NKT_, TM_>(d, zp, stream);
  if (d.ipp * d.S <= 144) {
    if (nqt <= 3) { QA(3, 3, 144) }
    if (nqt <= 5) { QA(3, 5, 144) }
    QA(3, 9, 144)
  }
  if (nqt <= 9) { QA(2, 9, 240) }
  QA(2, 15, 240)
#undef QA
}
```

ditsep_amd/native.py:

```python
from __future__ import annotations

import ctypes as C
import math
import os
import warnings
from typing import Mapping, Optional

import torch

_HERE = os.path.dirname(os.path.abspath(__file__))
LIB_PATH = os.environ.get("DSN_LIB", os.path.join(_HERE, "libditsep_hip.so"))

PREC_BF16 = 1
PREC_BF16X3 = 2
PREC_FP16 = 3
PREC_FP16X3 = 4
PREC_FP8 = 5
SCORE_NONE, SCORE_DIT, SCORE_NCSNPP = 0, 1, 2
MAX_VAE_BLOCKS = 8

EXPORTS = [
    "dsn_create", "dsn_destroy", "dsn_last_error", "dsn_load_tensor", "dsn_finalize_weights", "dsn_finalize_weights_ex",
    "dsn_score", "dsn_ouve_schedule", "dsn_pc_sample", "dsn_pc_sample_sched", "dsn_pc_sample_ex", "dsn_pc_sample_mix", "dsn_sb_sample", "dsn_decode",
    "dsn_encode", "dsn_decode_chunked", "dsn_encode_chunked",
    "dsn_latent_frames", "dsn_hop_length", "dsn_separate", "dsn_enable_graphs",
    "dsn_workspace_bytes", "dsn_profile_begin", "dsn_profile_end", "dsn_profile_hbm", "dsn_profile_rows", "dsn_test_igemm",
    "dsn_test_gemm", "dsn_bench_igemm", "dsn_debug_read", "dsn_si_sdr_pit", "dsn_si_bss_eval",
    "dsn_stoi", "dsn_ode_sample", "dsn_score_loss",
]


PREDICTORS = {"reverse_diffusion": 0, "euler_maruyama": 1, "none": 2}
CORRECTORS = {"ald": 0, "langevin": 1}


class DsnSamplerOpts(C.Structure):
    _fields_ = [
        ("predictor", C.c_int), ("corrector", C.c_int), ("corrector_steps", C.c_int),
        ("snr", C.c_float), ("t_eps", C.c_float), ("denoise", C.c_int),
        ("timesteps", C.POINTER(C.c_float)), ("prior_mean", C.c_void_p), ("intermediates", C.c_void_p),
    ]


class DsnMixOpts(C.Structure):
    _fields_ = [
        ("prior_mix", C.c_int), ("d_lambda", C.c_float), ("sigma_min", C.c_float), ("sigma_max", C.c_float),
        ("avg_len", C.c_int), ("predictor", C.c_int), ("corrector", C.c_int), ("corrector_steps", C.c_int),
        ("snr", C.c_float), ("t_eps", C.c_float), ("denoise", C.c_int),
    ]


class DsnOdeOpts(C.Structure):
    _fields_ = [
        ("method", C.c_int), ("rtol", C.c_double), ("atol", C.c_double), ("t_eps", C.c_double), ("denoise", C.c_int),
        ("N", C.c_int), ("first_step", C.c_double), ("max_step", C.c_double), ("max_attempts", C.c_int),
    ]


class DsnOdeStats(C.Structure):
    _fields_ = [
        ("nfev", C.c_int), ("n_accepted", C.c_int), ("n_rejected", C.c_int), ("t_final", C.c_double),
        ("status", C.c_int),
    ]


class DsnLossOpts(C.Structure):
    _fields_ = [("mode", C.c_int), ("reduction", C.c_int), ("t_eps", C.c_float)]


LOSS_MODES = {"dsm": 0, "init_pit": 1}
LOSS_REDUCTIONS = {"none": 0, "mean": 1}
ODE_METHODS = {"RK45": 0, "RK23": 1}
ODE_STATUS = {-1: "running", 0: "finished", 1: "step size too small", 2: "max_attempts reached"}
MIX_CORRECTORS = {"ald2": 0, "none": 1}
SB_TYPES = {"sde": 0, "ode": 1}


class DsnConfig(C.Structure):
    _fields_ = [
        ("device", C.c_int32), ("precision", C.c_int32), ("n_src", C.c_int32), ("latent_dim", C.c_int32),
        ("score_kind", C.c_int32), ("dit_embed_dim", C.c_int32), ("dit_depth", C.c_int32),
        ("dit_heads", C.c_int32),
        ("ncsn_nf", C.c_int32), ("ncsn_n_levels", C.c_int32), ("ncsn_ch_mult", C.c_int32 * 4),
        ("ncsn_num_res_blocks", C.c_int32), ("ncsn_attn_resolution", C.c_int32), ("ncsn_image_size", C.c_int32),
        ("ncsn_max_latent_length", C.c_int32),
        ("vae_channels", C.c_int32), ("vae_n_blocks", C.c_int32),
        ("vae_c_mults", C.c_int32 * MAX_VAE_BLOCKS), ("vae_strides", C.c_int32 * MAX_VAE_BLOCKS),
        ("vae_enc_latent_dim", C.c_int32), ("vae_use_snake", C.c_int32), ("vae_final_tanh", C.c_int32),
        ("vae_has_encoder", C.c_int32), ("vae_has_decoder", C.c_int32),
        ("sde_theta", C.c_float), ("sde_sigma_min", C.c_float), ("sde_sigma_max", C.c_float),
    ]


TEST_GEMM_KERNELS = {"auto": 0, "tile": 1, "v1": 2, "panel": 3, "skinny": 4, "halo": 5, "splitk": 6}
ACT_NONE, ACT_ELU, ACT_SNAKE, ACT_SILU = 0, 1, 2, 3
F32_NONE, F32_TANH = 0, 1


class DsnTestGemm(C.Structure):
    _fields_ = [
        ("kernel", C.c_int), ("bm", C.c_int), ("bn", C.c_int), ("nst", C.c_int), ("bk", C.c_int),
        ("panel_rows", C.c_int), ("panel_bn", C.c_int), ("panel_wm", C.c_int), ("ksplit", C.c_int),
        ("B", C.c_int), ("Lin", C.c_int), ("Cin", C.c_int), ("N", C.c_int), ("taps", C.c_int), ("in_stride", C.c_int),
        ("tap_dil", C.c_int), ("in_pad", C.c_int), ("rows_per_b", C.c_int), ("M", C.c_int),
        ("in_row_elems", C.c_int), ("a_off", C.c_int), ("in_bstride", C.c_int64),
        ("img_h", C.c_int), ("img_w", C.c_int), ("out_bstride", C.c_int64),
        ("out_row_elems", C.c_int), ("out_off", C.c_int), ("out_limit", C.c_int64),
        ("a", C.c_void_p), ("a_numel", C.c_int64), ("w", C.c_void_p),
        ("bias", C.c_void_p), ("bias_mod", C.c_int), ("bbias", C.c_void_p), ("bbias_stride", C.c_int),
        ("resid", C.c_void_p), ("resid_bstride", C.c_int64), ("resid_row_elems", C.c_int), ("resid_off", C.c_int),
        ("out_scale", C.c_float), ("f32_op", C.c_int), ("act", C.c_int), ("act_a", C.c_void_p), ("act_b", C.c_void_p),
        ("act_mod", C.c_int), ("swiglu", C.c_int), ("gn_stats", C.c_void_p), ("gn_stats2", C.c_void_p),
        ("gn_nq2", C.c_int), ("gn_qoff2", C.c_int),
        ("sc_a", C.c_void_p), ("sc_a_numel", C.c_int64), ("sc_w", C.c_void_p), ("sc_bias", C.c_void_p),
        ("sc_Cin", C.c_int), ("sc_row_elems", C.c_int),
        ("out_f32", C.c_void_p), ("out_planes", C.c_void_p), ("out_ps", C.c_int64),
        ("slabs", C.c_void_p), ("slab_stride", C.c_int64),
    ]


_lib = None


def load_library() -> C.CDLL:
    global _lib
    if _lib is not None:
        return _lib
    if not os.path.exists(LIB_PATH):
        raise RuntimeError(
            f"{LIB_PATH} not found: the HIP extension is required (no CPU/PyTorch fallback). "
            "Build it with `python -c 'import __graft_entry__ as g; g.build()'` or `make -C ditsep_amd/csrc`.")
    lib = C.CDLL(LIB_PATH)
    vp, ci, cf, fp = C.c_void_p, C.c_int, C.c_float, C.POINTER(C.c_float)
    lib.dsn_create.restype = vp
    lib.dsn_create.argtypes = [C.POINTER(DsnConfig)]
    lib.dsn_destroy.restype = None
    lib.dsn_destroy.argtypes = [vp]
    lib.dsn_last_error.restype = C.c_char_p
    lib.dsn_last_error.argtypes = [vp]
    lib.dsn_load_tensor.argtypes = [vp, C.c_char_p, vp, C.POINTER(C.c_int64), ci, ci]
    lib.dsn_finalize_weights.argtypes = [vp]
    lib.dsn_finalize_weights_ex.argtypes = [vp, ci]
    lib.dsn_score.argtypes = [vp, vp, vp, vp, vp, ci, ci, vp]
    lib.dsn_ouve_schedule.argtypes = [vp, ci, cf, cf, fp, fp, fp, fp, fp, fp]
    lib.dsn_pc_sample.argtypes = [vp, vp, vp, C.c_uint64, vp, ci, ci, ci, ci, cf, cf, ci, C.POINTER(ci), vp]
    lib.dsn_pc_sample_sched.argtypes = [vp, vp, vp, C.c_uint64, vp, ci, ci, ci, fp, ci, cf, ci, C.POINTER(ci), vp]
    lib.dsn_pc_sample_ex.argtypes = [vp, vp, vp, C.c_uint64, vp, ci, ci, ci, C.POINTER(DsnSamplerOpts),
                                     C.POINTER(ci), vp]
    lib.dsn_pc_sample_mix.argtypes = [vp, vp, vp, C.c_uint64, vp, ci, ci, ci, C.POINTER(DsnMixOpts), C.POINTER(ci), vp]
    lib.dsn_sb_sample.argtypes = [vp, vp, vp, C.c_uint64, vp, ci, ci, ci, cf, cf, cf, cf, ci, vp]
    lib.dsn_ode_sample.argtypes = [vp, vp, vp, C.c_uint64, vp, ci, ci, C.POINTER(DsnOdeOpts), C.POINTER(DsnOdeStats),
                                   vp]
    lib.dsn_score_loss.argtypes = [vp, vp, vp, vp, vp, vp, C.c_uint64, vp, vp, vp, vp, vp, ci, ci,
                                   C.POINTER(DsnLossOpts), vp]
    lib.dsn_decode.argtypes = [vp, vp, vp, ci, ci, ci, vp]
    lib.dsn_encode.argtypes = [vp, vp, vp, C.c_uint64, vp, ci, ci, vp]
    lib.dsn_decode_chunked.argtypes = [vp, vp, vp, ci, ci, ci, ci, ci, vp]
    lib.dsn_encode_chunked.argtypes = [vp, vp, vp, C.c_uint64, vp, ci, ci, ci, ci, vp]
    lib.dsn_latent_frames.argtypes = [vp, ci]
    lib.dsn_hop_length.argtypes = [vp]
    lib.dsn_separate.argtypes = [vp, vp, vp, vp, C.c_uint64, vp, ci, ci, ci, ci, ci, cf, cf, ci,
                                 C.POINTER(ci), vp]
    lib.dsn_enable_graphs.argtypes = [vp, ci]
    lib.dsn_workspace_bytes.restype = C.c_int64
    lib.dsn_workspace_bytes.argtypes = [vp]
    lib.dsn_profile_begin.argtypes = [vp]
    lib.dsn_profile_end.argtypes = [vp, C.POINTER(C.c_double), C.POINTER(C.c_double), C.POINTER(C.c_int64)]
    lib.dsn_profile_hbm.argtypes = [vp, C.POINTER(C.c_double), C.POINTER(C.c_double), C.POINTER(C.c_int64)]
    lib.dsn_profile_rows.argtypes = [vp, ci, C.c_char_p, C.POINTER(C.c_double), C.POINTER(C.c_double),
                                     C.POINTER(C.c_double), C.POINTER(C.c_int64)]
    lib.dsn_test_igemm.argtypes = [vp, vp, vp, vp, ci, ci, ci, ci, ci, ci, ci, ci, ci, ci, ci, vp]
    lib.dsn_test_gemm.argtypes = [vp, C.POINTER(DsnTestGemm), vp]
    lib.dsn_si_sdr_pit.argtypes = [vp, vp, vp, ci, ci, ci, fp, C.POINTER(ci), vp]
    lib.dsn_si_bss_eval.argtypes = [vp, vp, vp, ci, ci, ci, ci, cf, fp, fp, fp, C.POINTER(ci), vp]
    lib.dsn_stoi.argtypes = [vp, vp, vp, ci, ci, ci, ci, ci, C.POINTER(ci), fp, C.POINTER(ci), vp]
    lib.dsn_debug_read.argtypes = [vp, C.c_char_p, vp, C.c_int64]
    lib.dsn_bench_igemm.argtypes = [vp] + [ci] * 10 + [C.POINTER(C.c_double)]
    for name in EXPORTS:
        getattr(lib, name)
    _lib = lib
    return lib


def _ptr(t: Optional[torch.Tensor]):
    return None if t is None else C.c_void_p(t.data_ptr())


def _dev32(t: torch.Tensor, device) -> torch.Tensor:
    return t.to(device=device, dtype=torch.float32).contiguous()


class Engine:

    def __init__(self, *, device: int = 0, precision: int = PREC_BF16X3, n_src: int = 2, latent_dim: int = 64,
                 score_kind: int = SCORE_DIT, dit_embed_dim: int = 1024, dit_depth: int = 24,
                 dit_heads: int = 16, ncsn_nf: int = 128, ncsn_ch_mult=(1, 2, 2), ncsn_num_res_blocks: int = 2,
                 ncsn_attn_resolution: int = 16, ncsn_image_size: int = 64, ncsn_max_latent_length: int = 4,
                 vae_channels: int = 128, vae_c_mults=(1, 2, 4, 8, 16),
                 vae_strides=(2, 4, 4, 8, 8), vae_enc_latent_dim: int = 128, vae_use_snake: bool = False,
                 vae_final_tanh: bool = True, vae_has_encoder: bool = True, vae_has_decoder: bool = True,
                 sde_theta: float = 1.5, sde_sigma_min: float = 0.96, sde_sigma_max: float = 10.0):
        self.lib = load_library()
        if not torch.cuda.is_available():
            raise RuntimeError("ditsep_amd needs a ROCm GPU (torch.cuda.is_available() is False)")
        cfg = DsnConfig()
        cfg.device, cfg.precision, cfg.n_src, cfg.latent_dim = device, precision, n_src, latent_dim
        cfg.score_kind = score_kind
        cfg.dit_embed_dim, cfg.dit_depth, cfg.dit_heads = dit_embed_dim, dit_depth, dit_heads
        cfg.ncsn_nf, cfg.ncsn_n_levels = ncsn_nf, len(ncsn_ch_mult)
        for i, m in enumerate(ncsn_ch_mult):
            cfg.ncsn_ch_mult[i] = int(m)
        cfg.ncsn_num_res_blocks, cfg.ncsn_attn_resolution = ncsn_num_res_blocks, ncsn_attn_resolution
        cfg.ncsn_image_size, cfg.ncsn_max_latent_length = ncsn_image_size, ncsn_max_latent_length
        cfg.vae_channels, cfg.vae_n_blocks = vae_channels, len(vae_c_mults)
        assert len(vae_c_mults) == len(vae_strides) <= MAX_VAE_BLOCKS
        for i, (m, s) in enumerate(zip(vae_c_mults, vae_strides)):
            cfg.vae_c_mults[i], cfg.vae_strides[i] = int(m), int(s)
        cfg.vae_enc_latent_dim = vae_enc_latent_dim
        cfg.vae_use_snake, cfg.vae_final_tanh = int(vae_use_snake), int(vae_final_tanh)
        cfg.vae_has_encoder, cfg.vae_has_decoder = int(vae_has_encoder), int(vae_has_decoder)
        cfg.sde_theta, cfg.sde_sigma_min, cfg.sde_sigma_max = sde_theta, sde_sigma_min, sde_sigma_max
        self.cfg = cfg
        self.device = torch.device("cuda", device)
        self.n_src, self.latent_dim = n_src, latent_dim
        self.ctx = self.lib.dsn_create(C.byref(cfg))
        if not self.ctx:
            raise RuntimeError("dsn_create failed: " + self.lib.dsn_last_error(None).decode())

    def close(self):
        if getattr(self, "ctx", None):
            self.lib.dsn_destroy(self.ctx)
            self.ctx = None

    def __del__(self):
        try:
            self.close()
        except Exception:
            pass

    def _check(self, rc: int, what: str):
        if rc != 0:
            raise RuntimeError(f"{what} failed ({rc}): {self.lib.dsn_last_error(self.ctx).decode()}")

    def _stream(self):
        return C.c_void_p(torch.cuda.current_stream(self.device).cuda_stream)

    def load_state_dict(self, sd: Mapping[str, torch.Tensor], prefix: str = ""):
        for k, v in sd.items():
            if not torch.is_floating_point(v):
                continue
            t = v.detach().to(torch.float32).contiguous()
            shape = (C.c_int64 * max(t.ndim, 1))(*t.shape)
            self._check(self.lib.dsn_load_tensor(self.ctx, (prefix + k).encode(), C.c_void_p(t.data_ptr()),
                                                 shape, t.ndim, int(t.is_cuda)), f"dsn_load_tensor({prefix + k})")

# ... 236 lines not shown
    def si_sdr_pit(self, ref, est):
        ref, est = _dev32(ref, self.device), _dev32(est, self.device)
        B, n, L = ref.shape
        sdr = (C.c_float * (B * n))()
        perm = (C.c_int * (B * n))()
        self._check(self.lib.dsn_si_sdr_pit(self.ctx, _ptr(ref), _ptr(est), B, n, L, sdr, perm, self._stream()),
                    "dsn_si_sdr_pit")
        return (torch.tensor(list(sdr), dtype=torch.float32).reshape(B, n),
                torch.tensor(list(perm), dtype=torch.long).reshape(B, n))

    def si_bss_eval(self, ref, est, perm_by: str = "sir", clamp_db: float = 100.0):
        ref, est = _dev32(ref, self.device), _dev32(est, self.device)
        B, n, L = ref.shape
        bufs = [(C.c_float * (B * n))() for _ in range(3)]
        perm = (C.c_int * (B * n))()
        self._check(self.lib.dsn_si_bss_eval(self.ctx, _ptr(ref), _ptr(est), B, n, L, {"sdr": 0, "sir": 1}[perm_by],
                                             float(clamp_db), *bufs, perm, self._stream()), "dsn_si_bss_eval")
        out = [torch.tensor(list(b), dtype=torch.float32).reshape(B, n) for b in bufs]
        return (*out, torch.tensor(list(perm), dtype=torch.long).reshape(B, n))

    def stoi(self, ref, est, fs: int, extended: bool = True, perm=None, return_frames: bool = False):
        ref, est = _dev32(ref, self.device), _dev32(est, self.device)
        if ref.dim() != 3 or est.shape != ref.shape:
            raise ValueError(f"ref and est must both be [B,n,L] (got {tuple(ref.shape)} and {tuple(est.shape)})")
        B, n, L = ref.shape
        out = (C.c_float * (B * n))()
        frames = (C.c_int * (B * n))()
        cperm = None
        if perm is not None:
            p = torch.as_tensor(perm, dtype=torch.int32).reshape(-1).tolist()
            if len(p) != B * n:
                raise ValueError(f"perm must hold B*n = {B * n} entries (got {len(p)})")
            cperm = (C.c_int * (B * n))(*p)
        self._check(self.lib.dsn_stoi(self.ctx, _ptr(ref), _ptr(est), B, n, L, int(fs), int(bool(extended)), cperm,
                                      out, frames, self._stream()), "dsn_stoi")
        score = torch.tensor(list(out), dtype=torch.float32).reshape(B, n)
        nfr = torch.tensor(list(frames), dtype=torch.long).reshape(B, n)
        short = (nfr < 30).nonzero().tolist()
        if short:
            warnings.warn(f"stoi: {len(short)} item(s) [b, i] {short[:8]} have fewer than 30 frames after silent-frame "
                          f"removal; their score is 1e-5", RuntimeWarning, stacklevel=2)
        return (score, nfr) if return_frames else score

    def debug_read(self, name: str, shape):
        out = torch.empty(shape, dtype=torch.float32)
        self._check(self.lib.dsn_debug_read(self.ctx, name.encode(), C.c_void_p(out.data_ptr()), out.numel()),
                    f"dsn_debug_read({name})")
        return out

    def bench_igemm(self, B, Lin, Cin, N, taps=1, tap_dil=1, in_pad=0, ksplit=1, variant=2, iters=10):
        ms = C.c_double()
        self._check(self.lib.dsn_bench_igemm(self.ctx, B, Lin, Cin, N, taps, tap_dil, in_pad, ksplit, variant,
                                             iters, C.byref(ms)), "dsn_bench_igemm")
        return ms.value

    def test_igemm(self, a, w, *, taps=1, in_stride=1, tap_dil=1, in_pad=0, rows_per_b=None, panel_rows=0,
                   panel_bn=256):
        a, w = _dev32(a, self.device), _dev32(w, self.device)
        B, Lin, Cin = a.shape
        N = w.shape[0]
        rpb = rows_per_b or Lin
        out = torch.empty((B, rpb, N), device=self.device, dtype=torch.float32)
        self._check(self.lib.dsn_test_igemm(self.ctx, _ptr(a), _ptr(w), _ptr(out), B, Lin, Cin, N, taps, in_stride,
                                            tap_dil, in_pad, rpb, panel_rows, panel_bn, self._stream()), "dsn_test_igemm")
        return out

    _PLANES = {PREC_BF16: (1, False), PREC_BF16X3: (2, False), PREC_FP16: (1, True), PREC_FP16X3: (2, True)}

    def test_gemm(self, a, w, *, kernel="auto", B, Lin, Cin, N, taps=1, rows_per_b=None, **kw):
        t = DsnTestGemm()
        t.kernel = TEST_GEMM_KERNELS[kernel]
        t.B, t.Lin, t.Cin, t.N, t.taps = B, Lin, Cin, N, taps
        t.rows_per_b = Lin if rows_per_b is None else rows_per_b
        t.in_stride, t.tap_dil, t.out_scale = 1, 1, 1.0
        keep = [a, w]
        for name, tensor_like in (("a", a), ("w", w)):
            assert tensor_like.is_cuda and tensor_like.dtype == torch.float32 and tensor_like.is_contiguous(), name
        t.a, t.a_numel, t.w = a.data_ptr(), a.numel(), w.data_ptr()
        if w.numel() != N * taps * Cin:
            raise ValueError(f"w has {w.numel()} elements, N*taps*Cin = {N * taps * Cin}")
        for k, v in kw.items():
            if isinstance(v, torch.Tensor):
                assert v.is_cuda and v.is_contiguous(), k
                assert v.dtype == (torch.int16 if k == "out_planes" else torch.float32), k
                keep.append(v)
                setattr(t, k, v.data_ptr())
                if k == "sc_a":
                    t.sc_a_numel = v.numel()
                if k == "out_planes" and "out_ps" not in kw:
                    t.out_ps = v.shape[-1] if v.dim() > 1 else v.numel()
            elif v is not None:
                setattr(t, k, v)
        self._check(self.lib.dsn_test_gemm(self.ctx, C.byref(t), self._stream()), f"dsn_test_gemm({kernel})")

    def decode_planes(self, raw):
        P, f16 = self._PLANES[self.cfg.precision]
        raw = raw.reshape(P, -1)
        planes = [(raw[p].view(torch.float16) if f16 else raw[p].view(torch.bfloat16)).double() for p in range(P)]
        return planes[0] if P == 1 else planes[0] + planes[1]
```

include/ditsep_hip.h:

```cpp
#ifndef DITSEP_HIP_H
#define DITSEP_HIP_H

#include <stdint.h>

#ifdef __cplusplus
extern "C" {
#endif

#define DSN_OK 0
#define DSN_EINVAL (-1)
#define DSN_EHIP (-2)
#define DSN_ESTATE (-3)
#define DSN_ENOMEM (-4)
#define DSN_ESOLVER (-5)

#define DSN_PREC_BF16 1
#define DSN_PREC_BF16X3 2
#define DSN_PREC_FP16 3
#define DSN_PREC_FP16X3 4
#define DSN_PREC_FP8 5

#define DSN_SCORE_NONE 0
#define DSN_SCORE_DIT 1
#define DSN_SCORE_NCSNPP 2
// ... 109 lines not shown

int dsn_decode_chunked(dsn_ctx* ctx, const float* est, float* wav, int B, int T, int target_len, int chunk_size,
                       int overlap, void* stream);

int dsn_encode_chunked(dsn_ctx* ctx, const float* mix, const float* vae_noise, uint64_t seed, float* y, int B, int L,
                       int chunk_size, int overlap, void* stream);

int dsn_encode(dsn_ctx* ctx, const float* mix, const float* vae_noise, uint64_t seed, float* y, int B, int L,
               void* stream);
int dsn_latent_frames(const dsn_ctx* ctx, int L);
int dsn_hop_length(const dsn_ctx* ctx);

int dsn_separate(dsn_ctx* ctx, const float* mix, const float* vae_noise, const float* noise, uint64_t seed,
                 float* wav, int B, int L, int target_len, int N, int corrector_steps, float snr, float t_eps,
                 int denoise, int* nfe_out, void* stream);

int dsn_si_sdr_pit(dsn_ctx* ctx, const float* ref, const float* est, int B, int n, int L, float* si_sdr_out,
                   int* perm_out, void* stream);

int dsn_si_bss_eval(dsn_ctx* ctx, const float* ref, const float* est, int B, int n, int L, int perm_by, float clamp_db,
                    float* si_sdr_out, float* si_sir_out, float* si_sar_out, int* perm_out, void* stream);

int dsn_stoi(dsn_ctx* ctx, const float* ref, const float* est, int B, int n, int L, int fs, int extended,
             const int* perm, float* out, int* frames_out, void* stream);

int dsn_enable_graphs(dsn_ctx* ctx, int enable);
int64_t dsn_workspace_bytes(const dsn_ctx* ctx);
int dsn_profile_begin(dsn_ctx* ctx);
int dsn_profile_end(dsn_ctx* ctx, double* gemm_ms, double* gemm_flops, int64_t* gemm_launches);
int dsn_profile_hbm(dsn_ctx* ctx, double* ms, double* bytes, int64_t* launches);
#define DSN_PROFILE_NAME_LEN 48
int dsn_profile_rows(dsn_ctx* ctx, int max_rows, char* names, double* ms, double* flops, double* bytes,
                     int64_t* launches);

int dsn_test_igemm(dsn_ctx* ctx, const float* a, const float* w, float* out, int B, int Lin, int Cin, int N,
                   int taps, int in_stride, int tap_dil, int in_pad, int rows_per_b, int panel_rows, int panel_bn,
                   void* stream);

enum { DSN_TG_AUTO = 0, DSN_TG_TILE = 1, DSN_TG_V1 = 2, DSN_TG_PANEL = 3, DSN_TG_SKINNY = 4, DSN_TG_HALO = 5,
       DSN_TG_SPLITK = 6 };
typedef struct DsnTestGemm {
  int kernel;
  int bm, bn, nst, bk;
  int panel_rows, panel_bn, panel_wm;
  int ksplit;
  int B, Lin, Cin, N, taps, in_stride, tap_dil, in_pad, rows_per_b;
  int M;
  int in_row_elems, a_off;
  int64_t in_bstride;
  int img_h, img_w;
  int64_t out_bstride;
  int out_row_elems, out_off;
  int64_t out_limit;
  const float* a;
  int64_t a_numel;
  const float* w;
  const float* bias;
  int bias_mod;
  const float* bbias;
  int bbias_stride;
  const float* resid;
  int64_t resid_bstride;
  int resid_row_elems, resid_off;
  float out_scale;
  int f32_op;
  int act;
  const float* act_a;
  const float* act_b;
  int act_mod;
  int swiglu;
  float* gn_stats;
  float* gn_stats2;
  int gn_nq2, gn_qoff2;
  const float* sc_a;
  int64_t sc_a_numel;
  const float* sc_w;
  const float* sc_bias;
  int sc_Cin, sc_row_elems;
  float* out_f32;
  int16_t* out_planes;
  int64_t out_ps;
  float* slabs;
  int64_t slab_stride;
} DsnTestGemm;
int dsn_test_gemm(dsn_ctx* ctx, const DsnTestGemm* t, void* stream);

int dsn_debug_read(dsn_ctx* ctx, const char* name, float* host, int64_t count);
int dsn_bench_igemm(dsn_ctx* ctx, int B, int Lin, int Cin, int N, int taps, int tap_dil, int in_pad, int ksplit,
                    int variant, int iters, double* ms_out);

#ifdef __cplusplus
}
#endif
#endif
```

Before: 287.7.

## Fold pre-attention LayerNorm into QKV GEMM and reduce FF2 split-K in-launch

The pre-attention LayerNorm is folded into the QKV-attention kernel. Gamma is baked into the packed weights, beta goes into a bias, and the kernel applies per-row mean/rstd from slice statistics using weight column sums. The FF2 split-K GEMM now does its reduction inside the launch: the last workgroup per tile, chosen by an atomic ticket, sums the slabs, adds bias and residual, and writes X, the fp16 planes and the row-slice stats. This removes the separate residual_norm kernels and their HBM round trips between layers. The cost is atomic counters, extra slab reads in the last workgroup, and some numerical risk from folded-LN variance recombination.

```diff
diff --git a/ditsep_amd/csrc/engine.hip b/ditsep_amd/csrc/engine.hip
--- a/ditsep_amd/csrc/engine.hip
+++ b/ditsep_amd/csrc/engine.hip
@@ -73,6 +73,8 @@
   Packed8 qkv8, out8, ff1_8, ff2_8;
   Packed ff1f;
   float* ff1_colsum = nullptr;
+  Packed qkvf;
+  float* qkv_colsum = nullptr;
   Packed8 ff1f8;
   float* ff1_colsum8 = nullptr;
 };
@@ -144,6 +146,21 @@
       ++ws_epoch;
     }
     return c.first;
+  }
+  unsigned* kr_count = nullptr;
+  long kr_count_n = 0;
+  unsigned* kr_counters(long count, hipStream_t st) {
+    if (!kr_count || kr_count_n < count) {
+      if (kr_count) {
+        HIPCHK(hipDeviceSynchronize());
+        HIPCHK(hipFree(kr_count));
+      }
+      kr_count_n = std::max(count, 1024L);
+      HIPCHK(hipMalloc((void**)&kr_count, kr_count_n * sizeof(unsigned)));
+      HIPCHK(hipMemsetAsync(kr_count, 0, kr_count_n * sizeof(unsigned), st));
+      ++ws_epoch;
+    }
+    return kr_count;
   }
   double hbm_ms = 0, hbm_bytes = 0;
   int64_t hbm_launches = 0;
@@ -570,6 +587,24 @@
             launch_pack_bias_swiglu(tmp, p.bias, p.N, st);
           }
           p.bias_mod = p.N;
+          if (D % 128 == 0) {
+            const DevTensor& wq = get(lp + "self_attn.to_qkv.weight");
+            Packed& pq = L.qkvf;
+            pq.N = (int)wq.shape[0];
+            pq.K = pq.Cin = (int)(wq.numel / wq.shape[0]);
+            pq.taps = 1;
+            pq.ps = (long)pq.N * pq.K;
+            pq.w = (op16_t*)dmalloc(sizeof(op16_t) * pq.ps * P);
+            launch_pack_weight(wq.p, nullptr, pq.w, pq.ps, PL, PACK_LINEAR, pq.N, pq.K, pq.K, pq.N, 1, 1, st, L.g1);
+            L.qkv_colsum = (float*)dmalloc(sizeof(float) * pq.N);
+            launch_packed_row_sum(pq.w, pq.ps, PL, pq.N, pq.K, L.qkv_colsum, st);
+            pq.bias = nullptr;
+            if (L.be1) {
+              pq.bias = (float*)dmalloc(sizeof(float) * pq.N);
+              launch_bias_plus_wbeta(wq.p, L.be1, nullptr, pq.N, pq.K, pq.bias, st);
+            }
+            pq.bias_mod = pq.N;
+          }
         }
       }
     }
@@ -767,6 +802,14 @@
                d.gn_qoff2, d.N);
         audit_span("gn_stats2", d.gn_stats2, 0, nb * (d.rows_per_b / 64) * (long)d.gn_nq2 * 2 * e32, d);
       }
+    }
+    if (d.kr_slabs) {
+      if (d.ksplit != 4 || d.panel_rows <= 0 || d.slab_stride < (long)d.M * d.N)
+        fail(DSN_EINVAL, "audit: in-launch split-K reduce with ksplit=%d panel_rows=%d slab_stride=%ld", d.ksplit,
+             d.panel_rows, d.slab_stride);
+      audit_span("kr_slabs", d.kr_slabs, 0, ((ks - 1) * d.slab_stride + (long)d.M * d.N) * e32, d);
+      audit_span("kr_count", d.kr_count, 0, (long)cdiv(d.M, d.panel_rows) * cdiv(d.N, 256) * (long)sizeof(unsigned), d);
+      audit_span("resid", d.resid, 0, (long)d.M * d.N * e32, d);
     }
     if (d.ln_stats) {
       audit_span("ln_stats", d.ln_stats, 0, (long)d.M * d.ln_np * 2 * e32, d);
@@ -1016,6 +1059,12 @@
       if (force && atoi(force) >= 1 && atoi(force) * S <= qkv_attention_max_rows()) qa_ipp = atoi(force);
     }
     op16_t* AOp = qa_ipp ? wsbuf<op16_t>("dit_AOp", M * D) : nullptr;
+    const int ffo_bn = 256, ffo_ks = 4;
+    const int ffo_rows = short_panel ? panel_rows_for(cdiv(D, ffo_bn) * ffo_ks, 272) : 0;
+    const bool tail = fold_rows && !fp8 && qa_ipp && D % 128 == 0 && ffo_rows > 0 && ffo_rows <= 144 &&
+                      !layers.empty() && layers[0].qkvf.w;
+    float* ST1 = tail ? wsbuf<float>("dit_ST1", M * (D / 64) * 2) : nullptr;
+    unsigned* krc = tail ? kr_counters((long)cdiv(M, ffo_rows) * cdiv(D, ffo_bn), st) : nullptr;
     float* slabs = nullptr;
     int pend_n = 0;
     const float* pend_bias = nullptr;
@@ -1023,6 +1072,11 @@
     for (int i = 0; i < cfg.dit_depth; ++i) {
       const DitLayer& L = layers[i];
       auto ln_bytes = [&](int np) { return (double)M * D * (4.0 * (np ? 2 : 1) + 4.0 * np + 2.0 * P); };
+      if (tail) {
+        if (i == 0)
+          prof_launch("dit.residual_norm", (double)M * D * (4.0 + 2.0) + (double)M * (D / 64) * 8.0, st,
+                      [&] { launch_row_slice_stats(X, Xp, ST1, (int)M, D, PL, st); });
+      } else
       prof_launch("dit.residual_norm", ln_bytes(pend_n), st, [&] {
         launch_residual_norm(X, slabs, pend_n, slab_stride, pend_bias, L.g1, L.be1, qa_ipp ? Ap : lnout, M * D, PL,
                              (int)M, D, 1e-5f, 1, st, qa_ipp ? nullptr : SA8);
@@ -1030,9 +1084,15 @@
       if (qa_ipp) {
         QkvAttnDesc q;
         memset(&q, 0, sizeof q);
-        q.A = Ap;
-        q.W = L.qkv.w;
-        q.bias = L.qkv.bias;
+        q.A = tail ? Xp : Ap;
+        q.W = tail ? L.qkvf.w : L.qkv.w;
+        q.bias = tail ? L.qkvf.bias : L.qkv.bias;
+        if (tail) {
+          q.ln_stats = ST1;
+          q.ln_np = D / 64;
+          q.ln_colsum = L.qkv_colsum;
+          q.ln_eps = 1e-5f;
+        }
         q.rope_cos = rc;
         q.rope_sin = rs;
         q.out = fp8 ? nullptr : AOp;
@@ -1169,7 +1229,21 @@
         const int fbn = 256, fks = 4;
         d.ksplit = skinny ? skinny_ks : ((short_panel || fp8) ? fks : pick_ksplit(d));
         if (short_panel || fp8) d.panel_rows = panel_rows_for(cdiv(D, fbn) * fks, fp8 ? 208 : 272);
-        if (d.ksplit > 1) {
+        if (tail) {
+          slabs = wsbuf<float>("dit_slabs", slab_stride * 8);
+          d.panel_rows = ffo_rows;
+          d.ksplit = ffo_ks;
+          d.kr_slabs = slabs;
+          d.kr_count = krc;
+          d.slab_stride = slab_stride;
+          d.resid = X;
+          d.out_f32 = X;
+          d.out_planes = Xp;
+          d.out_ps = M * D;
+          d.stat_out = ST1;
+          d.stat_np = D / 64;
+          pend_bias = nullptr;
+        } else if (d.ksplit > 1) {
           slabs = wsbuf<float>("dit_slabs", slab_stride * 8);
           d.out_f32 = slabs;
           d.slab_stride = slab_stride;
@@ -1183,16 +1257,17 @@
         if (fp8) run_fp8(d, st, fbn);
         else if (skinny) run(d, st, 0, true);
         else run(d, st, short_panel ? fbn : 0);
-        pend_n = d.ksplit > 1 ? d.ksplit : 0;
-      }
-    }
+        pend_n = (d.ksplit > 1 && !tail) ? d.ksplit : 0;
+      }
+    }
+    if (!tail)
     prof_launch("dit.residual_norm", (double)M * D * (8.0 + 4.0 * pend_n + 2.0 * P), st, [&] {
       launch_residual_norm(X, slabs, pend_n, slab_stride, pend_bias, nullptr, nullptr, Ap, M * D, PL, (int)M, D, 1e-5f,
                            0, st);
     });
     {
       Tag tg(this, "dit.project_out");
-      GemmDesc d = base_desc(Ap, M * D, pout, B, T, S);
+      GemmDesc d = base_desc(tail ? Xp : Ap, M * D, pout, B, T, S);
       d.in_pad = -1;
       d.in_bstride = (long)S * D;
       d.out_f32 = SC;
@@ -1780,6 +1855,7 @@
   for (void* p : ctx->allocs) (void)hipFree(p);
   for (auto& kv : ctx->ws) (void)hipFree(kv.second.first);
   for (auto& kv : ctx->gnf_sync) (void)hipFree(kv.second.first);
+  if (ctx->kr_count) (void)hipFree(ctx->kr_count);
   if (ctx->fin_err_host) (void)hipHostFree(ctx->fin_err_host);
   if (ctx->ode_host) (void)hipHostFree(ctx->ode_host);
   delete ctx;
@@ -2877,6 +2953,22 @@
         d.panel_wm = t->panel_wm;
         d.cfg_nst = t->nst;
         d.cfg_bk = t->bk;
+        if (t->ksplit > 1) {
+          if (!t->slabs || t->slab_stride <= 0) fail(DSN_EINVAL, "test_gemm: panel split-K needs slabs");
+          d.ksplit = t->ksplit;
+          d.slab_stride = t->slab_stride;
+          if (t->kr_count) {
+            d.kr_slabs = t->slabs;
+            d.kr_count = reinterpret_cast<unsigned*>(t->kr_count);
+            d.stat_out = t->stat_out;
+            d.stat_np = t->N / 64;
+          } else {
+            d.out_f32 = t->slabs;
+            d.out_planes = nullptr;
+            d.bias = nullptr;
+            d.resid = nullptr;
+          }
+        }
         if (audit) ctx->audit_desc(d, false);
         check(igemm_panel_launch(d, PL, t->panel_bn, st), "row-panel kernel");
         break;
@@ -2909,6 +3001,82 @@
       default:
         fail(DSN_EINVAL, "test_gemm: unknown kernel %d", t->kernel);
     }
+    HIPCHK(hipGetLastError());
+  });
+}
+
+int dsn_test_residual_norm(dsn_ctx* ctx, float* x, const float* slabs, int nslab, int64_t slab_stride, const float* bias,
+                           const float* gamma, const float* beta, int16_t* out_planes, int rows, int D, int do_norm,
+                           void* stream) {
+  return guarded(ctx, [&] {
+    if (!x || !out_planes || rows <= 0 || D <= 0 || D % 4 != 0 || nslab < 0 || nslab > 8 || (nslab > 0 && !slabs) ||
+        (do_norm && !gamma))
+      fail(DSN_EINVAL, "test_residual_norm: bad arguments");
+    launch_residual_norm(x, slabs, nslab, slab_stride, bias, gamma, beta, reinterpret_cast<op16_t*>(out_planes),
+                         (long)rows * D, ctx->PL, rows, D, 1e-5f, do_norm, (hipStream_t)stream);
+    HIPCHK(hipGetLastError());
+  });
+}
+
+int dsn_test_qkv_attention(dsn_ctx* ctx, const float* x, const float* wqkv, const float* gamma, const float* beta,
+                           int16_t* out, int M, int D, int H, int S, int ipp, int fold, void* stream) {
+  return guarded(ctx, [&] {
+    hipStream_t st = (hipStream_t)stream;
+    const int PL = ctx->PL;
+    if (ctx->P != 1) fail(DSN_EINVAL, "test_qkv_attention: single-plane precisions only");
+    if (!x || !wqkv || !gamma || !out || M <= 0 || D != H * 64 || S < 1 || M % S != 0 || (fold && D % 128 != 0))
+      fail(DSN_EINVAL, "test_qkv_attention: bad arguments");
+    const long wn = 3L * D * D;
+    op16_t* ap = ctx->wsbuf<op16_t>("tq_a", (long)M * D);
+    op16_t* wp = ctx->wsbuf<op16_t>("tq_w", wn);
+    float* stt = ctx->wsbuf<float>("tq_st", (long)M * (D / 64) * 2);
+    float* cs = ctx->wsbuf<float>("tq_cs", 3L * D);
+    float* bf = ctx->wsbuf<float>("tq_b", 3L * D);
+    float* rc = ctx->wsbuf<float>("tq_rc", (long)S * 32);
+    float* rs = ctx->wsbuf<float>("tq_rs", (long)S * 32);
+    launch_rope_tables(rc, rs, S, 32, st);
+    QkvAttnDesc q;
+    memset(&q, 0, sizeof q);
+    if (fold) {
+      launch_row_slice_stats(x, ap, stt, M, D, PL, st);
+      launch_pack_weight(wqkv, nullptr, wp, wn, PL, PACK_LINEAR, 3 * D, D, D, 3 * D, 1, 1, st, gamma);
+      launch_packed_row_sum(wp, wn, PL, 3 * D, D, cs, st);
+      if (beta) launch_bias_plus_wbeta(wqkv, beta, nullptr, 3 * D, D, bf, st);
+      q.bias = beta ? bf : nullptr;
+      q.ln_stats = stt;
+      q.ln_np = D / 64;
+      q.ln_colsum = cs;
+      q.ln_eps = 1e-5f;
+    } else {
+      launch_residual_norm(const_cast<float*>(x), nullptr, 0, 0, nullptr, gamma, beta, ap, (long)M * D, PL, M, D, 1e-5f,
+                           1, st);
+      launch_pack_weight(wqkv, nullptr, wp, wn, PL, PACK_LINEAR, 3 * D, D, D, 3 * D, 1, 1, st);
+    }
+    q.A = ap;
+    q.W = wp;
+    q.rope_cos = rc;
+    q.rope_sin = rs;
+    q.out = reinterpret_cast<op16_t*>(out);
+    q.M = M;
+    q.D = D;
+    q.H = H;
+    q.S = S;
+    q.ipp = ipp;
+    q.q_scale = 0.125f;
+    static const bool audit = getenv("DSN_AUDIT") != nullptr;
+    if (audit) {
+      GemmDesc g;
+      memset(&g, 0, sizeof g);
+      g.M = M;
+      g.N = D;
+      g.Cin = D;
+      g.taps = 1;
+      ctx->audit_span("qkv out", out, 0, (long)M * D * (long)sizeof(op16_t), g);
+      ctx->audit_span("qkv x", x, 0, (long)M * D * (long)sizeof(float), g);
+      ctx->audit_span("qkv w", wqkv, 0, wn * (long)sizeof(float), g);
+    }
+    const hipError_t e = qkv_attention_launch(q, PL, st);
+    if (e != hipSuccess) fail(DSN_EHIP, "test_qkv_attention: launch refused or failed: %s", hipGetErrorString(e));
     HIPCHK(hipGetLastError());
   });
 }
diff --git a/ditsep_amd/csrc/igemm.h b/ditsep_amd/csrc/igemm.h
--- a/ditsep_amd/csrc/igemm.h
+++ b/ditsep_amd/csrc/igemm.h
@@ -69,6 +69,8 @@
   int cfg_bm, cfg_bn, cfg_nst, cfg_bk;
   int dbg;
   int m_fast;
+  float* kr_slabs;
+  unsigned* kr_count;
 };
 
 hipError_t igemm_launch(const GemmDesc& d, int pl, hipStream_t stream);
@@ -98,6 +100,10 @@
   int ipp;
   int panels;
   float q_scale;
+  const float* ln_stats;
+  int ln_np;
+  const float* ln_colsum;
+  float ln_eps;
 };
 hipError_t qkv_attention_launch(const QkvAttnDesc& d, int pl, hipStream_t stream);
 int qkv_attention_max_rows();
diff --git a/ditsep_amd/csrc/igemm.hip b/ditsep_amd/csrc/igemm.hip
--- a/ditsep_amd/csrc/igemm.hip
+++ b/ditsep_amd/csrc/igemm.hip
@@ -11,7 +11,7 @@
 
 __device__ __forceinline__ int swz(int row, int chunk) { return chunk ^ ((-(row >> 2)) & 3); }
 
-enum { EPI_STATS = 1, EPI_LNFOLD = 2, EPI_FP8OUT = 4 };
+enum { EPI_STATS = 1, EPI_LNFOLD = 2, EPI_FP8OUT = 4, EPI_KREDUCE = 8 };
 enum { LEAN_NO_DIT = 1, LEAN_NO_NCSN = 2, LEAN_SEEDED = 4 };
 
 template <int NT, int MT>
@@ -60,7 +60,8 @@
 
 template <int P, int F16, int NT, int MT, int EPI = 0, int LEAN = 0>
 __device__ __forceinline__ void epilogue_gen(const GemmDesc& d_arg, f32x4 (&acc)[NT][MT], int mw0, int m_end, int nw0,
-                                             int lane, int z, const float* ln_rows = nullptr, int ln_m0 = 0) {
+                                             int lane, int z, const float* ln_rows = nullptr, int ln_m0 = 0,
+                                             unsigned* kr_flag = nullptr, int kr_tile = 0) {
   dsn_mfma_drain();
   const GemmDesc d = d_arg;
   const bool f_rope = !(LEAN & LEAN_NO_DIT) && d.rope_cos != nullptr;
@@ -70,6 +71,67 @@
   const bool f_bbias = !(LEAN & LEAN_NO_NCSN) && d.bbias != nullptr;
   const bool f_tanh = !(LEAN & LEAN_NO_NCSN) && d.f32_op == DSN_F32_TANH;
   const int nq = (lane >> 4) * 4;
+  if constexpr ((EPI & EPI_KREDUCE) != 0) {
+    static_assert((EPI & EPI_STATS) != 0 && (EPI & EPI_FP8OUT) == 0, "the in-launch reduce feeds the statistics epilogue");
+    constexpr int KR_KS = 4;
+    float* const slab = d.kr_slabs + (long)z * d.slab_stride;
+#pragma unroll
+    for (int tm = 0; tm < MT; ++tm) {
+      const int m = mw0 + tm * 16 + (lane & 15);
+      if (m >= m_end) continue;
+#pragma unroll
+      for (int tn = 0; tn < NT; ++tn) {
+        const int n = nw0 + tn * 16 + nq;
+        if (n < d.N) *reinterpret_cast<f32x4*>(slab + (long)m * d.N + n) = acc[tn][tm];
+      }
+    }
+    asm volatile("s_waitcnt vmcnt(0)" ::: "memory");
+    __syncthreads();
+    if (threadIdx.x == 0) {
+      __builtin_amdgcn_fence(__ATOMIC_RELEASE, "agent");
+      asm volatile("s_waitcnt vmcnt(0)" ::: "memory");
+      const unsigned ticket = __hip_atomic_fetch_add(d.kr_count + kr_tile, 1u, __ATOMIC_RELAXED, __HIP_MEMORY_SCOPE_AGENT);
+      const bool last = (ticket & (KR_KS - 1)) == KR_KS - 1;
+      if (last) {
+        __builtin_amdgcn_fence(__ATOMIC_ACQUIRE, "agent");
+        asm volatile("s_waitcnt vmcnt(0)" ::: "memory");
+      }
+      *kr_flag = last ? 1u : 0u;
+    }
+    __syncthreads();
+    if (*kr_flag == 0u) return;
+    f32x4 kb[NT];
+#pragma unroll
+    for (int tn = 0; tn < NT; ++tn) {
+      const int n = nw0 + tn * 16 + nq;
+      kb[tn] = (d.bias && n < d.N) ? *reinterpret_cast<const f32x4*>(d.bias + (n % d.bias_mod)) : f32x4{0.f, 0.f, 0.f, 0.f};
+    }
+    const float* const o0 = d.kr_slabs + (long)(z > 0 ? 0 : 1) * d.slab_stride;
+    const float* const o1 = d.kr_slabs + (long)(z > 1 ? 1 : 2) * d.slab_stride;
+    const float* const o2 = d.kr_slabs + (long)(z > 2 ? 2 : 3) * d.slab_stride;
+#pragma unroll
+    for (int tm = 0; tm < MT; ++tm) {
+      const int m = mw0 + tm * 16 + (lane & 15);
+      if (m >= m_end) continue;
+#pragma unroll
+      for (int tn = 0; tn < NT; ++tn) {
+        const int n = nw0 + tn * 16 + nq;
+        if (n >= d.N) continue;
+        const long off = (long)m * d.N + n;
+        f32x4 v = *reinterpret_cast<const f32x4*>(d.resid + off);
+        const f32x4 q0 = *reinterpret_cast<const f32x4*>(o0 + off);
+        const f32x4 q1 = *reinterpret_cast<const f32x4*>(o1 + off);
+        const f32x4 q2 = *reinterpret_cast<const f32x4*>(o2 + off);
+        const f32x4 own = acc[tn][tm];
+        if (d.bias) v += kb[tn];
+        v += z == 0 ? own : q0;
+        v += z == 1 ? own : (z == 0 ? q0 : q1);
+        v += z == 2 ? own : (z < 2 ? q1 : q2);
+        v += z == 3 ? own : q2;
+        acc[tn][tm] = v;
+      }
+    }
+  } else
   if (d.ksplit > 1) {
     float* slab = d.out_f32 + (long)z * d.slab_stride;
 #pragma unroll
@@ -96,7 +158,8 @@
 #pragma unroll
     for (int tn = 0; tn < NT; ++tn) {
       const int n = nw0 + tn * 16 + nq;
-      bvec[tn] = d.bias ? *reinterpret_cast<const f32x4*>(d.bias + (n % d.bias_mod)) : f32x4{0.f, 0.f, 0.f, 0.f};
+      bvec[tn] = (d.bias && !(EPI & EPI_KREDUCE)) ? *reinterpret_cast<const f32x4*>(d.bias + (n % d.bias_mod))
+                                                  : f32x4{0.f, 0.f, 0.f, 0.f};
     }
 #pragma unroll
     for (int tn = 0; tn < NT; ++tn) dsn_touch(bvec[tn]);
@@ -108,7 +171,8 @@
 #pragma unroll
       for (int tn = 0; tn < NT; ++tn) {
         const int n = nw0 + tn * 16 + nq;
-        f32x4 v = acc[tn][tm] + bvec[tn];
+        f32x4 v = acc[tn][tm];
+        if constexpr ((EPI & EPI_KREDUCE) == 0) v += bvec[tn];
         acc[tn][tm] = v;
         s1 += (v[0] + v[1]) + (v[2] + v[3]);
         if (n < d.N) {
@@ -161,7 +225,7 @@
         }
       m2 += __shfl_xor(m2, 16, 64);
       m2 += __shfl_xor(m2, 32, 64);
-      if ((lane >> 4) == 0)
+      if ((lane >> 4) == 0 && nw0 < d.N)
         *reinterpret_cast<float2*>(d.stat_out + ((long)m * d.stat_np + nw0 / (NT * 16)) * 2) = float2{mean, m2};
     }
     return;
@@ -1195,7 +1259,7 @@
   for (int s2 = 0; s2 < NST - 1; ++s2)
     if (s2 < nkt) issue(s2);
 
-  if constexpr ((EPI & EPI_STATS) != 0) {
+  if constexpr ((EPI & EPI_STATS) != 0 && (EPI & EPI_KREDUCE) == 0) {
 #pragma unroll
     for (int tm = 0; tm < MTW; ++tm) {
       const int m = m0 + my_row0 + tm * 16 + (lane & 15);
@@ -1274,7 +1338,8 @@
     }
   }
   epilogue_gen<P, F16, 4, MTW, EPI, LEAN_NO_NCSN>(d, acc, m0 + my_row0, min(m_end, m0 + my_row0 + my_mt * 16), n0 + wave_n * 64, lane,
-                                    z, ((EPI & EPI_LNFOLD) && d.ln_stats) ? ln_rows : nullptr, m0);
+                                    z, ((EPI & EPI_LNFOLD) && d.ln_stats) ? ln_rows : nullptr, m0,
+                                    reinterpret_cast<unsigned*>(lds), tile);
 }
 
 
@@ -1882,11 +1947,15 @@
   if (d.swiglu && (d.N % 32 != 0)) return hipErrorInvalidValue;
   if (d.ksplit > 1 && (!d.out_f32 || d.swiglu)) return hipErrorInvalidValue;
   if (d.img_w > 0) return hipErrorInvalidValue;
-  if (d.stat_out && (d.N % 64 != 0 || d.stat_np != d.N / 64 || d.swiglu || d.ksplit > 1)) return hipErrorInvalidValue;
+  const bool kred = d.kr_slabs != nullptr;
+  if (d.stat_out && (d.N % 64 != 0 || d.stat_np != d.N / 64 || d.swiglu || (d.ksplit > 1 && !kred))) return hipErrorInvalidValue;
+  if (kred && (!d.stat_out || !d.kr_count || d.ksplit != 4 || d.slab_stride < (long)d.M * d.N || !d.resid || !d.out_f32 ||
+               !d.out_planes || planes != 1 || bn != 256 || d.panel_rows > 9 * 16 || d.taps != 1 || d.rows_per_b != d.M))
+    return hipErrorInvalidValue;
   if (d.ln_stats && (!d.swiglu || !d.ln_colsum || d.ln_np <= 0 || d.taps != 1 || planes != 1)) return hipErrorInvalidValue;
   const op16_t* zp = zero_page();
   if (!zp) return hipErrorOutOfMemory;
-  const int epi = (d.stat_out ? EPI_STATS : 0) | (d.ln_stats ? EPI_LNFOLD : 0);
+  const int epi = (d.stat_out ? EPI_STATS : 0) | (d.ln_stats ? EPI_LNFOLD : 0) | (kred ? EPI_KREDUCE : 0);
 #define PCFGE(MT_, P_, W_, NS_, BK_, E_)                                                             \
   if (planes == P_ && bn == W_ * 64 && epi == E_)                                                     \
     return f16 ? launch_panel_t<P_, 1, W_, NS_, BK_, MT_, E_>(d, zp, stream)                          \
@@ -1909,7 +1978,7 @@
   }
   if (d.panel_rows <= 9 * 16) {
     PCFGS(9, 1, 4, 3, 64) PCFGS(9, 1, 2, 3, 64) PCFGS(9, 2, 4, 2, 32) PCFGS(9, 2, 2, 2, 32)
-    PCFGE(9, 1, 4, 3, 64, EPI_LNFOLD)
+    PCFGE(9, 1, 4, 3, 64, EPI_LNFOLD) PCFGE(9, 1, 4, 3, 64, (EPI_STATS | EPI_KREDUCE))
   }
   if (d.panel_rows <= 13 * 16) {
     PCFGS(13, 1, 4, 2, 64) PCFGS(13, 1, 2, 2, 64) PCFGE(13, 1, 4, 2, 64, EPI_LNFOLD)
diff --git a/ditsep_amd/csrc/kernels.h b/ditsep_amd/csrc/kernels.h
--- a/ditsep_amd/csrc/kernels.h
+++ b/ditsep_amd/csrc/kernels.h
@@ -29,6 +29,7 @@
 void launch_residual_norm(float* x, const float* slabs, int nslab, long slab_stride, const float* bias,
                           const float* gamma, const float* beta, op16_t* out, long ps, int planes, int rows, int D,
                           float eps, int do_norm, hipStream_t s, unsigned char* out_fp8_scale = nullptr);
+void launch_row_slice_stats(const float* x, op16_t* out, float* stats, int rows, int D, int planes, hipStream_t s);
 void launch_timestep_features(const float* t, const float* w, int B, int half, op16_t* out, long ps,
                               int planes, hipStream_t s);
 int launch_attention_mfma(const op16_t* qkv, long ps, op16_t* out, long out_ps, int pl, int B, int S, int H, int dh,
diff --git a/ditsep_amd/csrc/kernels.hip b/ditsep_amd/csrc/kernels.hip
--- a/ditsep_amd/csrc/kernels.hip
+++ b/ditsep_amd/csrc/kernels.hip
@@ -460,6 +460,19 @@
   const long oi = (rbase >> 2) + i;
   reinterpret_cast<op16x4*>(out)[oi] = hi;
   if (PL_COUNT(planes) == 2) reinterpret_cast<op16x4*>(out + ps)[oi] = lo;
+}
+
+__global__ __launch_bounds__(TPB) void row_slice_stats_kernel(const float* __restrict__ x, op16_t* __restrict__ out,
+                                                              float* __restrict__ stats, long nslices, int D, int f16) {
+  const int lane = threadIdx.x & 63;
+  const long sl = (long)blockIdx.x * (TPB / 64) + (threadIdx.x >> 6);
+  if (sl >= nslices) return;
+  const float v = x[sl * 64 + lane];
+  out[sl * 64 + lane] = to_op16(v, f16);
+  const float mean = wave_sum(v) * (1.f / 64.f);
+  const float dl = v - mean;
+  const float m2 = wave_sum(dl * dl);
+  if (lane == 0) *reinterpret_cast<float2*>(stats + sl * 2) = float2{mean, m2};
 }
 
 __global__ void timestep_features_kernel(const float* __restrict__ t, const float* __restrict__ w, int B, int half,
@@ -962,6 +975,11 @@
   const long total = (long)B * n * D * T;
   hipLaunchKernelGGL(repeat_sources_kernel, dim3(grid_for(total)), dim3(TPB), 0, st, y, x, n, D, T, total);
 }
+void launch_row_slice_stats(const float* x, op16_t* out, float* stats, int rows, int D, int planes, hipStream_t st) {
+  const long nslices = (long)rows * (D / 64);
+  hipLaunchKernelGGL(row_slice_stats_kernel, dim3((unsigned)cdiv(nslices, (long)(TPB / 64))), dim3(TPB), 0, st, x, out,
+                     stats, nslices, D, PL_F16(planes));
+}
 void launch_residual_norm(float* x, const float* slabs, int nslab, long slab_stride, const float* bias,
                           const float* gamma, const float* beta, op16_t* out, long ps, int planes, int rows, int D,
                           float eps, int do_norm, hipStream_t st, unsigned char* o8s) {
diff --git a/ditsep_amd/csrc/qkv_attn.hip b/ditsep_amd/csrc/qkv_attn.hip
--- a/ditsep_amd/csrc/qkv_attn.hip
+++ b/ditsep_amd/csrc/qkv_attn.hip
@@ -97,6 +97,29 @@
   for (int s = 0; s < NST - 1; ++s)
     if (s < nkt) issue(s, s);
 
+  float* const ln_rows = reinterpret_cast<float*>(lds + NST * QA_STAGE + 8 * QA_BK);
+  if (d.ln_stats) {
+    for (int r = tid; r < QA_TM; r += 512) {
+      float mean = 0.f, rstd = 0.f;
+      if (r < rows_here) {
+        const f32x4* ps = reinterpret_cast<const f32x4*>(d.ln_stats + (long)(m0 + r) * d.ln_np * 2);
+        float msum = 0.f, m2 = 0.f, q = 0.f;
+        for (int p2 = 0; p2 < d.ln_np / 2; ++p2) {
+          const f32x4 v = ps[p2];
+          msum += v[0] + v[2];
+          m2 += v[1] + v[3];
+          q += v[0] * v[0] + v[2] * v[2];
+        }
+        mean = msum / (float)d.ln_np;
+        const float cnt = (float)K / (float)d.ln_np;
+        m2 += cnt * fmaxf(q - (float)d.ln_np * mean * mean, 0.f);
+        rstd = rsqrtf(m2 / (float)K + d.ln_eps);
+      }
+      ln_rows[2 * r] = mean;
+      ln_rows[2 * r + 1] = rstd;
+    }
+  }
+
   for (int i = 0; i < nkt; ++i) {
     const int younger = min(NST - 2, nkt - 1 - i);
     if (NST >= 4 && younger >= 2)
@@ -136,6 +159,15 @@
   for (int tm = 0; tm < MTW; ++tm) {
     if (tm >= mtw) continue;
     const int row = row0 + tm * 16 + r16;
+    if (d.ln_stats) {
+      const float mu = ln_rows[2 * row], rs = ln_rows[2 * row + 1];
+#pragma unroll
+      for (int tn = 0; tn < 3; ++tn) {
+        const int col = wn * 48 + tn * 16 + nq;
+        const f32x4 cs = *reinterpret_cast<const f32x4*>(d.ln_colsum + (long)(col >> 6) * d.D + head * 64 + (col & 63));
+        acc[tn][tm] = (acc[tn][tm] - cs * mu) * rs;
+      }
+    }
     if (d.bias) {
 #pragma unroll
       for (int tn = 0; tn < 3; ++tn) {
@@ -308,7 +340,7 @@
   if (dsn_first_use_on_device(attr))
     (void)hipFuncSetAttribute(reinterpret_cast<const void*>(qkv_attention_kernel<F16, NST, NKT, TM>),
                               hipFuncAttributeMaxDynamicSharedMemorySize, 160 * 1024);
-  const size_t smem = (size_t)(NST * (TM + QA_TN) * QA_BK + 8 * QA_BK) * sizeof(op16_t);
+  const size_t smem = (size_t)(NST * (TM + QA_TN) * QA_BK + 8 * QA_BK) * sizeof(op16_t) + (d.ln_stats ? TM * 2 * sizeof(float) : 0);
   hipLaunchKernelGGL((qkv_attention_kernel<F16, NST, NKT, TM>), dim3(d.panels * d.H), dim3(512), smem, stream, d, zp);
   return hipGetLastError();
 }
@@ -324,6 +356,7 @@
       d.M <= 0 || d.M % d.S != 0 || !d.A || !d.W || (!d.out && !d.out8) || (d.out8 && !d.out8_scale) || !d.rope_cos ||
       !d.rope_sin || d.A == d.out)
     return hipErrorInvalidValue;
+  if (d.ln_stats && (!d.ln_colsum || d.ln_np <= 0 || (d.ln_np & 1) || d.D % d.ln_np != 0)) return hipErrorInvalidValue;
   d.panels = cdiv(d.M / d.S, d.ipp);
   const op16_t* zp = qa_zero_page();
   if (!zp) return hipErrorOutOfMemory;
diff --git a/ditsep_amd/native.py b/ditsep_amd/native.py
--- a/ditsep_amd/native.py
+++ b/ditsep_amd/native.py
@@ -25,7 +25,7 @@
     "dsn_encode", "dsn_decode_chunked", "dsn_encode_chunked",
     "dsn_latent_frames", "dsn_hop_length", "dsn_separate", "dsn_enable_graphs",
     "dsn_workspace_bytes", "dsn_profile_begin", "dsn_profile_end", "dsn_profile_hbm", "dsn_profile_rows", "dsn_test_igemm",
-    "dsn_test_gemm", "dsn_bench_igemm", "dsn_debug_read", "dsn_si_sdr_pit", "dsn_si_bss_eval",
+    "dsn_test_gemm", "dsn_test_residual_norm", "dsn_test_qkv_attention", "dsn_bench_igemm", "dsn_debug_read", "dsn_si_sdr_pit", "dsn_si_bss_eval",
     "dsn_stoi", "dsn_ode_sample", "dsn_score_loss",
 ]
 
@@ -116,6 +116,7 @@
         ("sc_Cin", C.c_int), ("sc_row_elems", C.c_int),
         ("out_f32", C.c_void_p), ("out_planes", C.c_void_p), ("out_ps", C.c_int64),
         ("slabs", C.c_void_p), ("slab_stride", C.c_int64),
+        ("stat_out", C.c_void_p), ("kr_count", C.c_void_p),
     ]
 
 
@@ -171,6 +172,8 @@
                                      C.POINTER(C.c_double), C.POINTER(C.c_int64)]
     lib.dsn_test_igemm.argtypes = [vp, vp, vp, vp, ci, ci, ci, ci, ci, ci, ci, ci, ci, ci, ci, vp]
     lib.dsn_test_gemm.argtypes = [vp, C.POINTER(DsnTestGemm), vp]
+    lib.dsn_test_residual_norm.argtypes = [vp, vp, vp, C.c_int, C.c_int64, vp, vp, vp, vp, C.c_int, C.c_int, C.c_int, vp]
+    lib.dsn_test_qkv_attention.argtypes = [vp, vp, vp, vp, vp, vp, C.c_int, C.c_int, C.c_int, C.c_int, C.c_int, C.c_int, vp]
     lib.dsn_si_sdr_pit.argtypes = [vp, vp, vp, ci, ci, ci, fp, C.POINTER(ci), vp]
     lib.dsn_si_bss_eval.argtypes = [vp, vp, vp, ci, ci, ci, ci, cf, fp, fp, fp, C.POINTER(ci), vp]
     lib.dsn_stoi.argtypes = [vp, vp, vp, ci, ci, ci, ci, ci, C.POINTER(ci), fp, C.POINTER(ci), vp]
@@ -573,7 +576,7 @@
         for k, v in kw.items():
             if isinstance(v, torch.Tensor):
                 assert v.is_cuda and v.is_contiguous(), k
-                assert v.dtype == (torch.int16 if k == "out_planes" else torch.float32), k
+                assert v.dtype == {"out_planes": torch.int16, "kr_count": torch.int32}.get(k, torch.float32), k
                 keep.append(v)
                 setattr(t, k, v.data_ptr())
                 if k == "sc_a":
@@ -584,6 +587,27 @@
                 setattr(t, k, v)
         self._check(self.lib.dsn_test_gemm(self.ctx, C.byref(t), self._stream()), f"dsn_test_gemm({kernel})")
 
+    def test_residual_norm(self, x, out_planes, *, slabs=None, nslab=0, slab_stride=0, bias=None, gamma=None, beta=None,
+                           do_norm=True):
+        rows, D = x.shape
+        ptr = lambda v: None if v is None else v.data_ptr()
+        for v in (x, slabs, bias, gamma, beta):
+            assert v is None or (v.is_cuda and v.is_contiguous() and v.dtype == torch.float32)
+        assert out_planes.is_cuda and out_planes.is_contiguous() and out_planes.dtype == torch.int16
+        self._check(self.lib.dsn_test_residual_norm(self.ctx, ptr(x), ptr(slabs), nslab, slab_stride, ptr(bias), ptr(gamma),
+                                                    ptr(beta), ptr(out_planes), rows, D, int(do_norm), self._stream()),
+                    "dsn_test_residual_norm")
+
+    def test_qkv_attention(self, x, wqkv, gamma, beta, *, H, S, ipp, fold):
+        M, D = x.shape
+        for v in (x, wqkv, gamma, beta):
+            assert v is None or (v.is_cuda and v.is_contiguous() and v.dtype == torch.float32)
+        out = torch.zeros((M, D), dtype=torch.int16, device=x.device)
+        self._check(self.lib.dsn_test_qkv_attention(self.ctx, x.data_ptr(), wqkv.data_ptr(), gamma.data_ptr(),
+                                                    None if beta is None else beta.data_ptr(), out.data_ptr(), M, D, H, S,
+                                                    ipp, int(fold), self._stream()), "dsn_test_qkv_attention")
+        return out
+
     def decode_planes(self, raw):
         P, f16 = self._PLANES[self.cfg.precision]
         raw = raw.reshape(P, -1)
diff --git a/include/ditsep_hip.h b/include/ditsep_hip.h
--- a/include/ditsep_hip.h
+++ b/include/ditsep_hip.h
@@ -215,8 +215,15 @@
   int64_t out_ps;
   float* slabs;
   int64_t slab_stride;
+  float* stat_out;
+  int32_t* kr_count;
 } DsnTestGemm;
 int dsn_test_gemm(dsn_ctx* ctx, const DsnTestGemm* t, void* stream);
+int dsn_test_residual_norm(dsn_ctx* ctx, float* x, const float* slabs, int nslab, int64_t slab_stride, const float* bias,
+                           const float* gamma, const float* beta, int16_t* out_planes, int rows, int D, int do_norm,
+                           void* stream);
+int dsn_test_qkv_attention(dsn_ctx* ctx, const float* x, const float* wqkv, const float* gamma, const float* beta,
+                           int16_t* out, int M, int D, int H, int S, int ipp, int fold, void* stream);
 
 int dsn_debug_read(dsn_ctx* ctx, const char* name, float* host, int64_t count);
 int dsn_bench_igemm(dsn_ctx* ctx, int B, int Lin, int Cin, int N, int taps, int tap_dil, int in_pad, int ksplit,
```

Result: slower. 252.1 (-12.4%).
